# addtt/ladder-vae-pytorch

Hardware: AMD Instinct MI355X
Metric: training images/sec (ELBO step: fwd+bwd+Adamax) (higher is better)
Workload: dtype f32; 1 GPU; CIFAR10-shaped 15-layer LVAE (BASELINE configs[2]): 32x32x3, zdims 32x15, 4 blocks/layer, 64 filters, gated+skip, DMoL-10, dropout 0.2, free bits 1.0; batch_per_gpu=256, global_batch=256, parallelism=dp1, hip_graph=True

## Files before the change

include/lvae_hip.h:

```cpp
#ifndef LVAE_HIP_H
#define LVAE_HIP_H

#include <stddef.h>
#include <stdint.h>

#ifdef __cplusplus
extern "C" {
#endif

#define LVAE_ABI_VERSION 17

#define LVAE_EINVAL (-1)
#define LVAE_EALIGN (-2)
#define LVAE_EWORKSPACE (-3)

enum { LVAE_STATS_BN_FWD = 0, LVAE_STATS_BN_BWD = 1 };
enum { LVAE_PREC_F32 = 0, LVAE_PREC_BF16 = 1 };
enum { LVAE_DT_F32 = 0, LVAE_DT_BF16 = 1 };
enum {
  LVAE_FORM_AUTO = 0,
  LVAE_FORM_F32_MFMA = 1,
  LVAE_FORM_SIX_PRODUCT = 2,
  LVAE_FORM_SIX_PRODUCT_DIRECT = 3
};
enum { LVAE_ACT_NONE = 0, LVAE_ACT_ELU = 1, LVAE_ACT_RELU = 2, LVAE_ACT_LEAKYRELU = 3, LVAE_ACT_SELU = 4 };

enum {
  LVAE_GATHER_CONV = 0,
  LVAE_GATHER_TRANSPOSED = 1
};

int lvae_abi_version(void);
const char* lvae_last_error(void);

typedef struct lvae_bn_fold {
  const float* parts;
  int32_t rows;
  int64_t M;
  const float* gamma;
  const float* beta;
  float eps, momentum;
  float* running_mean;
  float* running_var;
  float* coef_out;
} lvae_bn_fold;

typedef struct lvae_conv_desc {
  const float* x;
  const float* x2;
  int32_t C1, C2;
  const float* w;
  int64_t w_stap, w_sk, w_sn;
  const float* bias;
  const float* in_scale;
  const float* in_shift;
  int32_t in_act;
  const float* out_scale;
  int32_t out_act;
  float* y;
  int32_t N, H, W, OH, OW, Cout;
  int32_t KH, KW, stride, pad;
  int32_t gather;
  int32_t precision;
  void* workspace;
  int64_t workspace_bytes;
  int32_t workspace_ready;
  float* stats_out;
  const float* stats_pivot;
  int32_t stats_mode;
  int32_t stats_act;
  const float* stats_x;
  const struct lvae_bn_fold* in_fold;
  int32_t form;
  uint8_t x_dtype;
  uint8_t y_dtype;
  uint8_t stats_x_dtype;
  uint8_t reserved_;
} lvae_conv_desc;

size_t lvae_conv2d_workspace(const lvae_conv_desc* d);
int lvae_conv2d_f32(const lvae_conv_desc* d, void* stream);
int lvae_conv1x1_dgrad_cat_f32(const lvae_conv_desc* d, float* dx2, int32_t split, void* stream);
int32_t lvae_conv1x1_dgrad_cat_ok(const lvae_conv_desc* d, int32_t split);
enum {
  LVAE_VARIANT_DIRECT = 0,
  LVAE_VARIANT_POS = 2,
  LVAE_VARIANT_WINO_F32 = 3,
  LVAE_VARIANT_WINO_SIX = 4,
  LVAE_VARIANT_BF16_DIRECT = 5,
  LVAE_VARIANT_SIX_DIRECT = 6
};
int32_t lvae_conv2d_variant(const lvae_conv_desc* d);
int32_t lvae_conv2d_position_major(const lvae_conv_desc* d);
int32_t lvae_resblock_bf16_storage(const lvae_conv_desc* d);
int lvae_conv2d_bf16(const lvae_conv_desc* d, void* stream);
int32_t lvae_conv2d_stats_rows(const lvae_conv_desc* d);
int32_t lvae_conv2d_folds_bn_finalize(const lvae_conv_desc* d);
int32_t lvae_conv2d_stats_buffer_rows(const lvae_conv_desc* d);

size_t lvae_conv2d_prepare_entry_bytes(void);
int lvae_conv2d_prepare_entry(const lvae_conv_desc* d, void* entry);
int lvae_conv2d_prepare_weights(const void* entries, int32_t n, int32_t max_cout, void* stream);

int lvae_conv1x1_gate_f32(const lvae_conv_desc* d, const float* res, int32_t act, float* out, void* stream);
int32_t lvae_conv1x1_gate_stats_rows(const lvae_conv_desc* d);
enum {
  LVAE_GATE_PERSISTENT = 1,
  LVAE_GATE_SINGLE_SHOT = 2
};
int32_t lvae_conv1x1_gate_variant(const lvae_conv_desc* d);
int lvae_conv1x1_gate_bwd_f32(const lvae_conv_desc* d, const float* dout, const float* ab, int32_t act, float* dab,
                              void* stream);
int32_t lvae_conv1x1_gate_bwd_ok(const lvae_conv_desc* d);

typedef struct lvae_bn_apply {
  const float* parts;
  int32_t rows;
  int32_t act;
  int64_t M;
  const float* coef;
  const float* dh;
  const float* x;
  const float* add;
  float* dgamma;
  float* dbeta;
  float* out;
  int32_t dh_bf16;
  int32_t reserved_;
  const float* drop;
} lvae_bn_apply;
size_t lvae_conv1x1_gate_bwd_wgrad_workspace(const lvae_conv_desc* d);
int32_t lvae_conv1x1_gate_bwd_wgrad_apply_ok(const lvae_conv_desc* d);
int lvae_conv1x1_gate_bwd_wgrad_f32(const lvae_conv_desc* d, const float* dout, const float* ab, const float* y, int32_t act,
                                    float* dw, int64_t dw_sk, int64_t dw_sn, float* db, void* workspace, size_t workspace_bytes,
                                    const lvae_bn_apply* ap, void* stream);
int32_t lvae_conv1x1_gate_bwd_wgrad_recompute_ok(const lvae_conv_desc* d);
int lvae_conv1x1_gate_bwd_wgrad_recompute_f32(const lvae_conv_desc* d, const float* dout, const float* y, int32_t act, void* gate_ws,
                                              int64_t gate_ws_bytes, int32_t gate_ws_ready, const float* gate_w, int64_t gate_w_sk,
                                              int64_t gate_w_sn, const float* gate_bias, float* dw, int64_t dw_sk, int64_t dw_sn,
                                              float* db, void* workspace, size_t workspace_bytes, const lvae_bn_apply* ap, void* stream);

enum { LVAE_RB_PRO_AFFINE = 0, LVAE_RB_PRO_BN_APPLY = 1, LVAE_RB_PRO_GATE_BWD = 2 };
enum { LVAE_RB_EPI_PLAIN = 0, LVAE_RB_EPI_GATE = 1 };
typedef struct lvae_rb_ext {
  int32_t prologue, epilogue;
  const float* gate_w;
  int64_t gate_w_sk, gate_w_sn;
  void* gate_ws;
  int64_t gate_ws_bytes;
  int32_t gate_ws_ready;
  const float* gate_bias;
  int32_t act;
  const float* res;
  float* ab;
  float* out;
  float* out_stats;
  const float* out_stats_pivot;
  const float* dout;
  const float* ab_in;
  float* dab;
  const float* bwd_parts;
  int32_t bwd_rows;
  int32_t bwd_act;
  int64_t bwd_M;
  const float* bwd_coef;
  const float* bwd_x;
  float* dgamma;
  float* dbeta;
  const float* pro_drop;
  float* xt_out;
  const void* pf_ptr[2];
  int64_t pf_bytes[2];
  const float* ap_parts;
  int32_t ap_rows;
  int32_t ap_act;
  int64_t ap_M;
  const float* ap_coef;
  const float* ap_dh;
  const float* ap_x;
  const float* ap_add;
  float* ap_dgamma;
  float* ap_dbeta;
  float* ap_out;
} lvae_rb_ext;
size_t lvae_resblock_gate_workspace(const lvae_conv_desc* g);
int lvae_resblock_gate_prepare_entry(const lvae_conv_desc* g, void* entry);
int32_t lvae_resblock_conv_rows(const lvae_conv_desc* d);
int32_t lvae_resblock_conv_gate_rows(const lvae_conv_desc* d);
size_t lvae_resblock_conv_workspace(const lvae_conv_desc* d);
int lvae_resblock_conv_prepare_entry(const lvae_conv_desc* d, void* entry);
int lvae_resblock_conv_f32(const lvae_conv_desc* d, const lvae_rb_ext* ext, void* stream);

size_t lvae_conv2d_wgrad_workspace(const lvae_conv_desc* d);
int lvae_conv2d_wgrad_f32(const lvae_conv_desc* d, const float* dy, float* dw, float* db, void* workspace,
                          size_t workspace_bytes, void* stream);
int lvae_conv2d_wgrad_bf16(const lvae_conv_desc* d, const float* dy, float* dw, float* db, void* workspace, size_t workspace_bytes,
                           void* stream);
int32_t lvae_conv2d_wgrad_apply_ok(const lvae_conv_desc* d);
int lvae_conv2d_wgrad_apply_f32(const lvae_conv_desc* d, const lvae_bn_apply* ap, float* dw, float* db, void* workspace,
                                size_t workspace_bytes, void* stream);
int32_t lvae_conv2d_wgrad_pair_ok(const lvae_conv_desc* a, const lvae_conv_desc* b);
size_t lvae_conv2d_wgrad_pair_workspace(const lvae_conv_desc* a, const lvae_conv_desc* b);
int32_t lvae_conv2d_wgrad_pair_schedule(const lvae_conv_desc* a, const lvae_conv_desc* b, int32_t* sched);
int lvae_conv2d_wgrad_pair_f32(const lvae_conv_desc* a, const lvae_bn_apply* ap, const lvae_conv_desc* b, const float* dy_b, float* dw_a,
                               float* db_a, float* dw_b, float* db_b, void* workspace, size_t workspace_bytes, void* stream);
enum {
  LVAE_WGRAD_VARIANT_GENERIC = 0,
  LVAE_WGRAD_VARIANT_IMG = 1,
  LVAE_WGRAD_VARIANT_BF16 = 2,
  LVAE_WGRAD_VARIANT_WINO = 3,
  LVAE_WGRAD_VARIANT_DIRECT_1X1 = 4,
  LVAE_WGRAD_VARIANT_TILE = 5,
  LVAE_WGRAD_VARIANT_THIN = 6
};
int32_t lvae_conv2d_wgrad_variant(const lvae_conv_desc* d);
size_t lvae_conv2d_wgrad_grouped_workspace(const lvae_conv_desc* descs, int32_t n);
int lvae_conv2d_wgrad_grouped_f32(const lvae_conv_desc* descs, const float* const* dy, float* const* dw, float* const* db,
                                  int32_t n, void* workspace, size_t workspace_bytes, void* stream);
int32_t lvae_conv2d_wgrad_grouped_schedule(const lvae_conv_desc* descs, int32_t n, int32_t* launch_of);

size_t lvae_bn_stats_workspace(int64_t M, int32_t C);
int lvae_bn_stats_f32(const float* x, int64_t M, int32_t C, const float* gamma, const float* beta, float eps,
                      float momentum, float* running_mean, float* running_var, float* scale, float* shift,
                      float* mean, float* rstd, void* workspace, size_t workspace_bytes, void* stream);
int lvae_bn_finalize_parts_f32(const float* parts, int32_t rows, int64_t M, int32_t C, const float* pivot, const float* gamma,
                               const float* beta, float eps, float momentum, float* running_mean, float* running_var,
                               float* scale, float* shift, float* mean, float* rstd, void* stream);
int lvae_bn_eval_coeffs_f32(int32_t C, const float* gamma, const float* beta, const float* running_mean,
                            const float* running_var, float eps, float* scale, float* shift, void* stream);

int lvae_affine_act_f32(const float* x, int64_t M, int32_t C, const float* scale, const float* shift, int32_t act,
                        const float* row_scale, int64_t rows_per_n, float* y, void* stream);

int lvae_affine_act_bwd_f32(const float* dh, const float* x, int64_t M, int32_t C, const float* scale,
                            const float* shift, int32_t act, int32_t bn_train, const float* mean, const float* rstd,
                            float* dgamma, float* dbeta, const float* drop, int64_t rows_per_n, const float* add,
                            float* dx, void* workspace, size_t workspace_bytes, void* stream);
int lvae_affine_act_bwd_parts_f32(const float* parts, int32_t rows, const float* dh, const float* x, int64_t M, int32_t C,
                                  const float* scale, const float* shift, int32_t act, const float* mean, const float* rstd,
                                  float* dgamma, float* dbeta, const float* drop, int64_t rows_per_n, const float* add,
                                  float* dx, void* workspace, size_t workspace_bytes, int32_t dtypes, void* stream);

int lvae_gate_fwd_f32(const float* ab, const float* res, int64_t M, int32_t C, int32_t act, float* out, void* stream);
int lvae_gate_bwd_f32(const float* dout, const float* ab, int64_t M, int32_t C, int32_t act, float* dab, void* stream);

int lvae_act_bwd_from_out_f32(const float* dy, const float* y, int64_t n, int32_t act, float* dx, void* stream);
int lvae_add_f32(const float* a, const float* b, int64_t n, float* out, void* stream);
int lvae_add3_f32(const float* a, const float* b, const float* c, int64_t n, float* out, void* stream);
int lvae_sum_of_row_means_f32(const float* x, int32_t L, int32_t N, float* out, void* stream);
int lvae_scale_rows_add_f32(const float* a, const float* row_scale, int64_t rows_per_n, int32_t C, const float* b,
                            int64_t M, float* out, void* stream);
int lvae_colsum_f32(const float* x, int64_t R, int64_t P, float* out, int32_t accumulate, void* stream);

int lvae_normal_stochastic_fwd_f32(const float* p, int32_t p_bcast, const float* q, const float* eps, int32_t N,
                                   int32_t HW, int32_t Z, int32_t mode, int32_t analytical_kl, float* z,
                                   float* logprob_p, float* logprob_q, float* kl_samplewise, float* kl_spatial,
                                   void* stream);
int lvae_normal_stochastic_bwd_f32(const float* p, int32_t p_bcast, const float* q, const float* eps, const float* z,
                                   const float* dz, const float* g_lp, const float* g_lq, const float* g_kl,
                                   const float* g_ks, int32_t N, int32_t HW, int32_t Z, int32_t mode,
                                   int32_t analytical_kl, float* dp, float* dq, void* stream);

typedef struct lvae_stoch_block {
  lvae_conv_desc conv_p, conv_q, conv_out;
  const float* p_given;
  int32_t p_bcast;
  int32_t mode, analytical_kl;
  const float* eps;
  float *logprob_p, *logprob_q, *kl_samplewise, *kl_spatial;
} lvae_stoch_block;
int32_t lvae_stoch_block_ok(const lvae_stoch_block* b);
size_t lvae_stoch_block_workspace(const lvae_conv_desc* d);
int lvae_stoch_block_prepare_entry(const lvae_conv_desc* d, void* entry);
int lvae_stoch_block_fwd_f32(const lvae_stoch_block* b, void* stream);
typedef struct lvae_stoch_block_bwd {
  lvae_conv_desc dgrad_out, dgrad_q, dgrad_p;
  const float* p;
  int32_t p_bcast;
  int32_t mode, analytical_kl;
  const float *q, *z, *eps, *dz, *g_lp, *g_lq, *g_kl, *g_ks;
} lvae_stoch_block_bwd;
int32_t lvae_stoch_block_bwd_ok(const lvae_stoch_block_bwd* b);
int lvae_stoch_block_bwd_f32(const lvae_stoch_block_bwd* b, void* stream);

int lvae_normal_prior_sample_f32(const float* p, int32_t p_bcast, const float* eps, float temperature,
                                 const float* row_temperature, int32_t N, int32_t HW, int32_t Z, float* z, float* logprob_p,
                                 void* stream);

size_t lvae_latent_interp_workspace(int32_t B, int32_t T);
int lvae_latent_interp_f32(const float* za, const float* zb, const float* t, int32_t B, int64_t n, int32_t T, int32_t mode, float* out,
                           void* workspace, size_t workspace_bytes, void* stream);

int lvae_kl_elementwise_fwd_f32(const float* p, int32_t p_bcast, const float* q, int32_t q_bcast, const float* z, int32_t N,
                                int32_t HW, int32_t Z, int32_t analytical_kl, float* out, void* stream);
int lvae_kl_elementwise_bwd_f32(const float* p, int32_t p_bcast, const float* q, int32_t q_bcast, const float* z, const float* g,
                                int32_t N, int32_t HW, int32_t Z, int32_t analytical_kl, float* dp, float* dq, float* dz,
                                void* stream);

int lvae_bernoulli_fwd_f32(const float* logits, const float* x, const float* u, int32_t N, int64_t P, float* mean,
                           float* mode, float* sample, float* ll, float* dll_dlogits, void* stream);
size_t lvae_dmol_workspace(int32_t N, int32_t HW);
int lvae_dmol_ll_fwd_f32(const float* l, const float* x, int32_t N, int32_t HW, int32_t nmix, float* ll, float* dll_dl,
                         void* workspace, size_t workspace_bytes, void* stream);
int lvae_dmol_sample_f32(const float* l, const float* u_mix, const float* u_log, int32_t N, int32_t HW, int32_t nmix,
                         float* sample, void* stream);
int lvae_gaussian_fwd_f32(const float* params, const float* x, const float* eps, int32_t N, int64_t P, int32_t C,
                          float* sample, float* ll, float* dll_dparams, void* stream);
int lvae_discr_logistic_fwd_f32(const float* raw, const float* x, const float* u, int32_t N, int64_t P, int32_t C, float* mean,
                                float* logscale, float* sample, float* ll, float* dll_draw, void* stream);
int lvae_bernoulli_masked_fwd_f32(const float* logits, const float* x, const float* u, int32_t N, int64_t P, int32_t C, float* mean,
                                  float* mode, float* sample, float* ll, float* dll_dlogits, const uint8_t* mask, float* filled,
                                  void* stream);
int lvae_dmol_ll_masked_fwd_f32(const float* l, const float* x, int32_t N, int32_t HW, int32_t nmix, float* ll, float* dll_dl,
                                void* workspace, size_t workspace_bytes, const uint8_t* mask, const float* sample, float* filled,
                                void* stream);
int lvae_gaussian_masked_fwd_f32(const float* params, const float* x, const float* eps, int32_t N, int64_t P, int32_t C, float* sample,
                                 float* ll, float* dll_dparams, const uint8_t* mask, float* filled, void* stream);
int lvae_discr_logistic_masked_fwd_f32(const float* raw, const float* x, const float* u, int32_t N, int64_t P, int32_t C, float* mean,
                                       float* logscale, float* sample, float* ll, float* dll_draw, const uint8_t* mask, float* filled,
                                       void* stream);
int lvae_mask_select_f32(const float* a, const float* b, float b_value, const uint8_t* mask, int32_t N, int32_t C, int64_t HW,
                         int32_t nchw, float* out, void* stream);
int lvae_scale_per_sample_f32(const float* a, const float* g, int32_t N, int64_t P, float* out, void* stream);

int lvae_upsample2x_fwd_f32(const float* x, int32_t N, int32_t H, int32_t W, int32_t C, float* y, void* stream);
int lvae_upsample2x_bwd_f32(const float* dy, int32_t N, int32_t H, int32_t W, int32_t C, float* dx, void* stream);
int lvae_pad_crop_f32(const float* x, int32_t N, int32_t C, int32_t H, int32_t W, int32_t src_nchw, float* y, int32_t OH,
                      int32_t OW, int32_t dst_nchw, void* stream);

int lvae_kl_bookkeeping_fwd_f32(const float* kl, int32_t L, int32_t N, float free_bits, float* kl_sep,
                                float* kl_avg_layerwise, float* scalars, void* stream);
int lvae_kl_bookkeeping_bwd_f32(const float* kl, int32_t L, int32_t N, float free_bits, const float* g_sep,
                                const float* g_avg, const float* g_scalars, float* dkl, void* stream);
int lvae_elbo_loss_fwd_f32(const float* ll, const float* kl_sep, const float* kl_loss, float beta, int32_t N,
                           float* elbo_sep, float* scalars, void* stream);
int lvae_elbo_loss_bwd_f32(const float* g_loss, float beta, int32_t N, float* d_ll, float* d_kl_loss, void* stream);
int lvae_elbo_loss_fwd_anneal_f32(const float* ll, const float* kl_sep, const float* kl_loss, const int64_t* step, int64_t anneal_steps,
                                  int32_t N, float* elbo_sep, float* scalars, void* stream);
int lvae_elbo_loss_bwd_anneal_f32(const float* g_loss, const int64_t* step, int64_t anneal_steps, int32_t N, float* d_ll,
                                  float* d_kl_loss, void* stream);

int lvae_iw_loss_fwd_f32(const float* ll, const float* kl_sep, float beta, int32_t K, int32_t B, float* elbo_sep, float* w, float* bound,
                         float* scalars, void* stream);
int lvae_iw_loss_bwd_f32(const float* g_loss, const float* w, float beta, int32_t K, int32_t B, float* d_ll, float* d_kl_sep,
                         void* stream);
int lvae_iw_loss_fwd_anneal_f32(const float* ll, const float* kl_sep, const int64_t* step, int64_t anneal_steps, int32_t K, int32_t B,
                                float* elbo_sep, float* w, float* bound, float* scalars, void* stream);
int lvae_iw_loss_bwd_anneal_f32(const float* g_loss, const float* w, const int64_t* step, int64_t anneal_steps, int32_t K, int32_t B,
                                float* d_ll, float* d_kl_sep, void* stream);
int lvae_repeat_samples_fwd_f32(const float* in, int64_t n, int32_t K, float* out, void* stream);
int lvae_repeat_samples_bwd_f32(const float* dout, int64_t n, int32_t K, float* din, void* stream);

int lvae_iw_logmeanexp_f32(const float* elbo, int32_t S, int32_t N, float* out, void* stream);
int lvae_iw_online_f32(const float* elbo, float* state, int32_t N, int32_t mode, int32_t S, float* iw, float* mean, void* stream);
int lvae_eval_online_f32(const float* elbo_sep, const float* ll, const float* kl_sep, const float* kl_avg_layerwise, double* state,
                         int32_t N, int32_t L, int32_t mode, void* stream);
int lvae_eval_totals_f64(const double* state, int32_t N, int32_t L, int32_t S, double* totals, void* stream);
size_t lvae_latent_stats_workspace(int32_t N, int32_t HW, int32_t Z);
int lvae_latent_stats_fold_f32(const float* p, int32_t p_bcast, const float* q, int32_t N, int32_t HW, int32_t Z, double* sums,
                               void* workspace, size_t workspace_bytes, void* stream);
int lvae_latent_stats_finalize_f64(const double* sums, int64_t U, int64_t n_images, double kl_threshold, double var_threshold,
                                   double* unit_out, double* layer_out, void* stream);
int lvae_summary_fold_f64(const float* loss, const float* elbo, const float* recons, const float* kl, const float* l2,
                          const float* grad_norm, const float* gscale, const float* kl_layers, int32_t L, double* acc, void* stream);
int lvae_summary_take_f64(double* acc, int32_t n, double* out, void* stream);

int lvae_image_border_count_f32(const float* a, int32_t a_nhwc, const float* b, int32_t b_nhwc, int32_t N, int32_t C, int32_t H,
                                int32_t W, float threshold, int32_t* count, void* stream);
int lvae_image_grid_u8(const float* a, int32_t a_nhwc, const float* b, int32_t b_nhwc, int32_t N, int32_t C, int32_t H, int32_t W,
                       int32_t nrow, const int32_t* border_count, float pad_value, uint8_t* grid, int64_t grid_bytes, void* stream);

#define LVAE_FEED_U8 0
#define LVAE_FEED_F32 1
int lvae_batch_gather_f32(const void* src, int32_t src_kind, int32_t src_hwc, int32_t N, int32_t C, int32_t H, int32_t W,
                          const int32_t* index, const int64_t* cursor, int32_t steps_per_epoch, int32_t B_global, int32_t lo,
                          int64_t base, int32_t n_rows, float* out, void* stream);

size_t lvae_nn_l2_workspace(int32_t Q, int64_t N, int32_t k);
int lvae_nn_l2_f32(const float* queries, int32_t Q, const void* table, int32_t table_kind, int64_t N, int64_t D, const int32_t* exclude,
                   int32_t k, int32_t* index_out, float* dist_out, void* workspace, size_t workspace_bytes, void* stream);

int lvae_adamax_step_f32(float* p, const float* g, float* exp_avg, float* exp_inf, const float* mask, int64_t n,
                         float lr, float beta1, float beta2, float eps, float weight_decay, const float* gscale,
                         const uint64_t* step_count, void* stream);
int lvae_adamax_ema_step_f32(float* p, const float* g, float* exp_avg, float* exp_inf, const float* mask, int64_t n,
                             float lr, float beta1, float beta2, float eps, float weight_decay, const float* gscale,
                             const uint64_t* step_count, float* ema, float decay, void* stream);
enum { LVAE_LR_CONSTANT = 0, LVAE_LR_COSINE = 1, LVAE_LR_LINEAR = 2, LVAE_LR_STEP = 3, LVAE_LR_EXP = 4 };
typedef struct lvae_lr_schedule {
  float base_lr;
  float min_lr;
  float gamma;
  int32_t kind;
  int64_t warmup_steps;
  int64_t decay_steps;
} lvae_lr_schedule;
int lvae_lr_schedule_at(const lvae_lr_schedule* schedule, uint64_t n, float* lr);
int lvae_adamax_sched_step_f32(float* p, const float* g, float* exp_avg, float* exp_inf, const float* mask, int64_t n,
                               const lvae_lr_schedule* schedule, float beta1, float beta2, float eps, float weight_decay,
                               const float* gscale, const uint64_t* step_count, float* ema, float decay, float* lr_out, void* stream);
typedef struct lvae_grad_guard_state {
  float norm;
  float scale;
  int32_t skip;
  int32_t reserved_;
  uint64_t clipped;
  uint64_t skipped;
} lvae_grad_guard_state;
int lvae_grad_guard_f32(const float* g, int64_t n, const float* gscale_in, float max_norm, float skip_threshold,
                        lvae_grad_guard_state* state, void* workspace, size_t workspace_bytes, void* stream);
int lvae_adamax_guarded_step_f32(float* p, const float* g, float* exp_avg, float* exp_inf, const float* mask, int64_t n, float lr,
                                 const lvae_lr_schedule* schedule, float beta1, float beta2, float eps, float weight_decay,
                                 const uint64_t* step_count, float* ema, float decay, float* lr_out,
                                 const lvae_grad_guard_state* guard, void* stream);
int lvae_adam_step_f32(float* p, const float* g, float* exp_avg, float* exp_avg_sq, const float* mask, int64_t n, float lr,
                       const lvae_lr_schedule* schedule , double beta1, double beta2, float eps, float weight_decay,
                       int32_t decoupled, const float* gscale , const uint64_t* step_count, float* ema ,
                       float decay, float* lr_out , const lvae_grad_guard_state* guard , void* stream);
typedef struct lvae_copy_entry {
  float* dst;
  const float* src;
  int64_t n;
} lvae_copy_entry;
int lvae_multi_copy_f32(const lvae_copy_entry* table, int32_t n_entries, const int32_t* flag, int32_t want, void* stream);
int lvae_swap_f32(float* a, float* b, int64_t n, void* stream);
size_t lvae_sumsq_workspace(int64_t n);
int lvae_l2norm_f32(const float* x, int64_t n, float* out, void* workspace, size_t workspace_bytes, void* stream);

int lvae_rng_fill_f32(float* out, int64_t n, int32_t kind, float lo, float hi, uint64_t seed, const uint64_t* offset,
                      uint64_t stream_id, void* stream);
int lvae_counter_advance(uint64_t* counter, uint64_t by, void* stream);
int lvae_counter_advance_unless(uint64_t* counter, uint64_t by, const int32_t* flag, void* stream);
int lvae_fill_f32(float* out, int64_t n, float value, void* stream);

int lvae_allreduce_unique_id(const char* librccl_path, void* id128);
int lvae_allreduce_init(const char* librccl_path, const void* id128, int32_t world, int32_t rank, void** handle);
int lvae_allreduce_enqueue(void* handle, float* buf, int64_t n, float* scratch, void* launch_stream, void* side_stream);
int lvae_allreduce_wait(void* handle, void* launch_stream, void* side_stream);
int lvae_allreduce_destroy(void* handle);

#ifdef __cplusplus
}
#endif
#endif
```

ladder-vae-pytorch_amd/_C.py:

```python
import ctypes as C
import os

import torch

_HERE = os.path.dirname(os.path.abspath(__file__))
LIB_PATH = os.path.join(_HERE, 'liblvae_hip.so')

ACT = {None: 0, 'none': 0, 'elu': 1, 'relu': 2, 'leakyrelu': 3, 'selu': 4}
GATHER_CONV, GATHER_TRANSPOSED = 0, 1
PREC_F32, PREC_BF16 = 0, 1
DT_F32, DT_BF16 = 0, 1
VARIANT_DIRECT, VARIANT_POS, VARIANT_WINO_F32, VARIANT_WINO_SIX, VARIANT_BF16_DIRECT, VARIANT_SIX_DIRECT = 0, 2, 3, 4, 5, 6
GATE_PERSISTENT, GATE_SINGLE_SHOT = 1, 2
WGRAD_VARIANT_GENERIC, WGRAD_VARIANT_IMG, WGRAD_VARIANT_BF16, WGRAD_VARIANT_WINO, WGRAD_VARIANT_DIRECT_1X1, WGRAD_VARIANT_TILE, WGRAD_VARIANT_THIN = range(7)
FEED_U8, FEED_F32 = 0, 1
FORM_AUTO, FORM_F32_MFMA, FORM_SIX_PRODUCT, FORM_SIX_PRODUCT_DIRECT = 0, 1, 2, 3


class LvaeHipError(RuntimeError):
    pass


class ConvDesc(C.Structure):
    _fields_ = [
        ('x', C.c_void_p), ('x2', C.c_void_p), ('C1', C.c_int32), ('C2', C.c_int32),
        ('w', C.c_void_p), ('w_stap', C.c_int64), ('w_sk', C.c_int64), ('w_sn', C.c_int64),
        ('bias', C.c_void_p), ('in_scale', C.c_void_p), ('in_shift', C.c_void_p), ('in_act', C.c_int32),
        ('out_scale', C.c_void_p), ('out_act', C.c_int32), ('y', C.c_void_p),
        ('N', C.c_int32), ('H', C.c_int32), ('W', C.c_int32), ('OH', C.c_int32), ('OW', C.c_int32),
        ('Cout', C.c_int32), ('KH', C.c_int32), ('KW', C.c_int32), ('stride', C.c_int32), ('pad', C.c_int32),
        ('gather', C.c_int32), ('precision', C.c_int32), ('workspace', C.c_void_p), ('workspace_bytes', C.c_int64), ('workspace_ready', C.c_int32), ('stats_out', C.c_void_p), ('stats_pivot', C.c_void_p), ('stats_mode', C.c_int32), ('stats_act', C.c_int32),
        ('stats_x', C.c_void_p),
        ('in_fold', C.c_void_p),
        ('form', C.c_int32), ('x_dtype', C.c_uint8), ('y_dtype', C.c_uint8), ('stats_x_dtype', C.c_uint8), ('reserved_', C.c_uint8),
    ]


class BnFold(C.Structure):
    _fields_ = [('parts', C.c_void_p), ('rows', C.c_int32), ('M', C.c_int64), ('gamma', C.c_void_p), ('beta', C.c_void_p),
                ('eps', C.c_float), ('momentum', C.c_float), ('running_mean', C.c_void_p), ('running_var', C.c_void_p),
                ('coef_out', C.c_void_p)]


class BnApply(C.Structure):
    _fields_ = [('parts', C.c_void_p), ('rows', C.c_int32), ('act', C.c_int32), ('M', C.c_int64), ('coef', C.c_void_p), ('dh', C.c_void_p),
                ('x', C.c_void_p), ('add', C.c_void_p), ('dgamma', C.c_void_p), ('dbeta', C.c_void_p), ('out', C.c_void_p),
                ('dh_bf16', C.c_int32), ('reserved_', C.c_int32), ('drop', C.c_void_p)]


class RbExt(C.Structure):
    _fields_ = [('prologue', C.c_int32), ('epilogue', C.c_int32), ('gate_w', C.c_void_p), ('gate_w_sk', C.c_int64), ('gate_w_sn', C.c_int64),
                ('gate_ws', C.c_void_p), ('gate_ws_bytes', C.c_int64), ('gate_ws_ready', C.c_int32), ('gate_bias', C.c_void_p), ('act', C.c_int32), ('res', C.c_void_p), ('ab', C.c_void_p), ('out', C.c_void_p),
                ('out_stats', C.c_void_p), ('out_stats_pivot', C.c_void_p), ('dout', C.c_void_p), ('ab_in', C.c_void_p), ('dab', C.c_void_p),
                ('bwd_parts', C.c_void_p), ('bwd_rows', C.c_int32), ('bwd_act', C.c_int32), ('bwd_M', C.c_int64), ('bwd_coef', C.c_void_p),
                ('bwd_x', C.c_void_p), ('dgamma', C.c_void_p), ('dbeta', C.c_void_p), ('pro_drop', C.c_void_p), ('xt_out', C.c_void_p),
                ('pf_ptr', C.c_void_p * 2), ('pf_bytes', C.c_int64 * 2),
                ('ap_parts', C.c_void_p), ('ap_rows', C.c_int32), ('ap_act', C.c_int32), ('ap_M', C.c_int64), ('ap_coef', C.c_void_p),
                ('ap_dh', C.c_void_p), ('ap_x', C.c_void_p), ('ap_add', C.c_void_p), ('ap_dgamma', C.c_void_p), ('ap_dbeta', C.c_void_p),
                ('ap_out', C.c_void_p)]


class StochBlock(C.Structure):
    _fields_ = [('conv_p', ConvDesc), ('conv_q', ConvDesc), ('conv_out', ConvDesc), ('p_given', C.c_void_p), ('p_bcast', C.c_int32),
                ('mode', C.c_int32), ('analytical_kl', C.c_int32), ('eps', C.c_void_p), ('logprob_p', C.c_void_p), ('logprob_q', C.c_void_p),
                ('kl_samplewise', C.c_void_p), ('kl_spatial', C.c_void_p)]


class StochBlockBwd(C.Structure):
    _fields_ = [('dgrad_out', ConvDesc), ('dgrad_q', ConvDesc), ('dgrad_p', ConvDesc), ('p', C.c_void_p), ('p_bcast', C.c_int32),
                ('mode', C.c_int32), ('analytical_kl', C.c_int32), ('q', C.c_void_p), ('z', C.c_void_p), ('eps', C.c_void_p), ('dz', C.c_void_p),
                ('g_lp', C.c_void_p), ('g_lq', C.c_void_p), ('g_kl', C.c_void_p), ('g_ks', C.c_void_p)]


class LrScheduleStruct(C.Structure):
    _fields_ = [('base_lr', C.c_float), ('min_lr', C.c_float), ('gamma', C.c_float), ('kind', C.c_int32),
                ('warmup_steps', C.c_int64), ('decay_steps', C.c_int64)]


class GradGuardState(C.Structure):
    _fields_ = [('norm', C.c_float), ('scale', C.c_float), ('skip', C.c_int32), ('reserved_', C.c_int32), ('clipped', C.c_uint64),
                ('skipped', C.c_uint64)]


class CopyEntry(C.Structure):
    _fields_ = [('dst', C.c_void_p), ('src', C.c_void_p), ('n', C.c_int64)]


LR_KINDS = {'constant': 0, 'cosine': 1, 'linear': 2, 'step': 3, 'exp': 4}

RB_PRO_AFFINE, RB_PRO_BN_APPLY, RB_PRO_GATE_BWD = 0, 1, 2
RB_EPI_PLAIN, RB_EPI_GATE = 0, 1

ABI_VERSION = 17

_P, _I, _L, _F, _Z, _U = C.c_void_p, C.c_int32, C.c_int64, C.c_float, C.c_size_t, C.c_uint64

SIGNATURES = {
    'lvae_abi_version': (C.c_int, []),
    'lvae_last_error': (C.c_char_p, []),
    'lvae_conv2d_workspace': (_Z, [C.POINTER(ConvDesc)]),
    'lvae_conv2d_f32': (C.c_int, [C.POINTER(ConvDesc), _P]),
    'lvae_conv2d_bf16': (C.c_int, [C.POINTER(ConvDesc), _P]),
    'lvae_conv1x1_dgrad_cat_f32': (C.c_int, [C.POINTER(ConvDesc), _P, _I, _P]),
    'lvae_conv1x1_dgrad_cat_ok': (_I, [C.POINTER(ConvDesc), _I]),
    'lvae_conv2d_stats_rows': (_I, [C.POINTER(ConvDesc)]),
    'lvae_conv2d_variant': (_I, [C.POINTER(ConvDesc)]),
    'lvae_conv2d_position_major': (_I, [C.POINTER(ConvDesc)]),
    'lvae_resblock_bf16_storage': (_I, [C.POINTER(ConvDesc)]),
    'lvae_conv2d_folds_bn_finalize': (_I, [C.POINTER(ConvDesc)]),
    'lvae_conv2d_stats_buffer_rows': (_I, [C.POINTER(ConvDesc)]),
    'lvae_conv2d_prepare_entry_bytes': (_Z, []),
    'lvae_conv2d_prepare_entry': (C.c_int, [C.POINTER(ConvDesc), _P]),
    'lvae_conv2d_prepare_weights': (C.c_int, [_P, _I, _I, _P]),
    'lvae_conv1x1_gate_f32': (C.c_int, [C.POINTER(ConvDesc), _P, _I, _P, _P]),
    'lvae_conv1x1_gate_stats_rows': (_I, [C.POINTER(ConvDesc)]),
    'lvae_conv1x1_gate_variant': (_I, [C.POINTER(ConvDesc)]),
    'lvae_conv1x1_gate_bwd_f32': (C.c_int, [C.POINTER(ConvDesc), _P, _P, _I, _P, _P]),
    'lvae_conv1x1_gate_bwd_ok': (_I, [C.POINTER(ConvDesc)]),
    'lvae_conv1x1_gate_bwd_wgrad_workspace': (_Z, [C.POINTER(ConvDesc)]),
    'lvae_conv1x1_gate_bwd_wgrad_apply_ok': (_I, [C.POINTER(ConvDesc)]),
    'lvae_conv1x1_gate_bwd_wgrad_f32': (C.c_int, [C.POINTER(ConvDesc), _P, _P, _P, _I, _P, _L, _L, _P, _P, _Z, C.POINTER(BnApply), _P]),
    'lvae_conv1x1_gate_bwd_wgrad_recompute_ok': (_I, [C.POINTER(ConvDesc)]),
    'lvae_conv1x1_gate_bwd_wgrad_recompute_f32': (C.c_int, [C.POINTER(ConvDesc), _P, _P, _I, _P, _L, _I, _P, _L, _L, _P, _P, _L, _L, _P, _P, _Z,
                                                            C.POINTER(BnApply), _P]),
    'lvae_resblock_gate_workspace': (_Z, [C.POINTER(ConvDesc)]),
    'lvae_resblock_gate_prepare_entry': (C.c_int, [C.POINTER(ConvDesc), _P]),
    'lvae_resblock_conv_rows': (_I, [C.POINTER(ConvDesc)]),
    'lvae_resblock_conv_gate_rows': (_I, [C.POINTER(ConvDesc)]),
    'lvae_resblock_conv_workspace': (_Z, [C.POINTER(ConvDesc)]),
    'lvae_resblock_conv_prepare_entry': (C.c_int, [C.POINTER(ConvDesc), _P]),
    'lvae_resblock_conv_f32': (C.c_int, [C.POINTER(ConvDesc), C.POINTER(RbExt), _P]),
    'lvae_conv2d_wgrad_workspace': (_Z, [C.POINTER(ConvDesc)]),
    'lvae_conv2d_wgrad_f32': (C.c_int, [C.POINTER(ConvDesc), _P, _P, _P, _P, _Z, _P]),
    'lvae_conv2d_wgrad_bf16': (C.c_int, [C.POINTER(ConvDesc), _P, _P, _P, _P, _Z, _P]),
    'lvae_conv2d_wgrad_variant': (_I, [C.POINTER(ConvDesc)]),
    'lvae_conv2d_wgrad_apply_ok': (_I, [C.POINTER(ConvDesc)]),
    'lvae_conv2d_wgrad_apply_f32': (C.c_int, [C.POINTER(ConvDesc), C.POINTER(BnApply), _P, _P, _P, _Z, _P]),
    'lvae_conv2d_wgrad_pair_ok': (_I, [C.POINTER(ConvDesc), C.POINTER(ConvDesc)]),
    'lvae_conv2d_wgrad_pair_workspace': (_Z, [C.POINTER(ConvDesc), C.POINTER(ConvDesc)]),
    'lvae_conv2d_wgrad_pair_schedule': (_I, [C.POINTER(ConvDesc), C.POINTER(ConvDesc), C.POINTER(_I)]),
    'lvae_conv2d_wgrad_pair_f32': (C.c_int, [C.POINTER(ConvDesc), C.POINTER(BnApply), C.POINTER(ConvDesc), _P, _P, _P, _P, _P, _P, _Z, _P]),
    'lvae_conv2d_wgrad_grouped_workspace': (_Z, [C.POINTER(ConvDesc), _I]),
    'lvae_conv2d_wgrad_grouped_f32': (C.c_int, [C.POINTER(ConvDesc), _P, _P, _P, _I, _P, _Z, _P]),
    'lvae_conv2d_wgrad_grouped_schedule': (_I, [C.POINTER(ConvDesc), _I, C.POINTER(_I)]),
    'lvae_bn_stats_workspace': (_Z, [_L, _I]),
    'lvae_bn_stats_f32': (C.c_int, [_P, _L, _I, _P, _P, _F, _F, _P, _P, _P, _P, _P, _P, _P, _Z, _P]),
    'lvae_bn_finalize_parts_f32': (C.c_int, [_P, _I, _L, _I, _P, _P, _P, _F, _F, _P, _P, _P, _P, _P, _P, _P]),
    'lvae_bn_eval_coeffs_f32': (C.c_int, [_I, _P, _P, _P, _P, _F, _P, _P, _P]),
    'lvae_affine_act_f32': (C.c_int, [_P, _L, _I, _P, _P, _I, _P, _L, _P, _P]),
    'lvae_affine_act_bwd_f32': (C.c_int, [_P, _P, _L, _I, _P, _P, _I, _I, _P, _P, _P, _P, _P, _L, _P, _P, _P, _Z, _P]),
    'lvae_affine_act_bwd_parts_f32': (C.c_int, [_P, _I, _P, _P, _L, _I, _P, _P, _I, _P, _P, _P, _P, _P, _L, _P, _P, _P, _Z, _I, _P]),
    'lvae_gate_fwd_f32': (C.c_int, [_P, _P, _L, _I, _I, _P, _P]),
    'lvae_gate_bwd_f32': (C.c_int, [_P, _P, _L, _I, _I, _P, _P]),
    'lvae_act_bwd_from_out_f32': (C.c_int, [_P, _P, _L, _I, _P, _P]),
    'lvae_add_f32': (C.c_int, [_P, _P, _L, _P, _P]),
    'lvae_add3_f32': (C.c_int, [_P, _P, _P, _L, _P, _P]),
    'lvae_sum_of_row_means_f32': (C.c_int, [_P, _I, _I, _P, _P]),
    'lvae_scale_rows_add_f32': (C.c_int, [_P, _P, _L, _I, _P, _L, _P, _P]),
    'lvae_colsum_f32': (C.c_int, [_P, _L, _L, _P, _I, _P]),
    'lvae_normal_stochastic_fwd_f32': (C.c_int, [_P, _I, _P, _P, _I, _I, _I, _I, _I, _P, _P, _P, _P, _P, _P]),
    'lvae_normal_stochastic_bwd_f32': (C.c_int, [_P, _I, _P, _P, _P, _P, _P, _P, _P, _P, _I, _I, _I, _I, _I, _P, _P, _P]),
    'lvae_stoch_block_ok': (_I, [C.POINTER(StochBlock)]),
    'lvae_stoch_block_workspace': (_Z, [C.POINTER(ConvDesc)]),
    'lvae_stoch_block_prepare_entry': (C.c_int, [C.POINTER(ConvDesc), _P]),
    'lvae_stoch_block_fwd_f32': (C.c_int, [C.POINTER(StochBlock), _P]),
    'lvae_stoch_block_bwd_ok': (_I, [C.POINTER(StochBlockBwd)]),
    'lvae_stoch_block_bwd_f32': (C.c_int, [C.POINTER(StochBlockBwd), _P]),
    'lvae_normal_prior_sample_f32': (C.c_int, [_P, _I, _P, _F, _P, _I, _I, _I, _P, _P, _P]),
    'lvae_latent_interp_workspace': (_Z, [_I, _I]),
    'lvae_latent_interp_f32': (C.c_int, [_P, _P, _P, _I, _L, _I, _I, _P, _P, _Z, _P]),
    'lvae_kl_elementwise_fwd_f32': (C.c_int, [_P, _I, _P, _I, _P, _I, _I, _I, _I, _P, _P]),
    'lvae_kl_elementwise_bwd_f32': (C.c_int, [_P, _I, _P, _I, _P, _P, _I, _I, _I, _I, _P, _P, _P, _P]),
    'lvae_bernoulli_fwd_f32': (C.c_int, [_P, _P, _P, _I, _L, _P, _P, _P, _P, _P, _P]),
    'lvae_dmol_workspace': (_Z, [_I, _I]),
    'lvae_dmol_ll_fwd_f32': (C.c_int, [_P, _P, _I, _I, _I, _P, _P, _P, _Z, _P]),
    'lvae_dmol_sample_f32': (C.c_int, [_P, _P, _P, _I, _I, _I, _P, _P]),
    'lvae_gaussian_fwd_f32': (C.c_int, [_P, _P, _P, _I, _L, _I, _P, _P, _P, _P]),
    'lvae_discr_logistic_fwd_f32': (C.c_int, [_P, _P, _P, _I, _L, _I, _P, _P, _P, _P, _P, _P]),
    'lvae_bernoulli_masked_fwd_f32': (C.c_int, [_P, _P, _P, _I, _L, _I, _P, _P, _P, _P, _P, _P, _P, _P]),
    'lvae_dmol_ll_masked_fwd_f32': (C.c_int, [_P, _P, _I, _I, _I, _P, _P, _P, _Z, _P, _P, _P, _P]),
    'lvae_gaussian_masked_fwd_f32': (C.c_int, [_P, _P, _P, _I, _L, _I, _P, _P, _P, _P, _P, _P]),
    'lvae_discr_logistic_masked_fwd_f32': (C.c_int, [_P, _P, _P, _I, _L, _I, _P, _P, _P, _P, _P, _P, _P, _P]),
    'lvae_mask_select_f32': (C.c_int, [_P, _P, _F, _P, _I, _I, _L, _I, _P, _P]),
    'lvae_scale_per_sample_f32': (C.c_int, [_P, _P, _I, _L, _P, _P]),
    'lvae_upsample2x_fwd_f32': (C.c_int, [_P, _I, _I, _I, _I, _P, _P]),
    'lvae_upsample2x_bwd_f32': (C.c_int, [_P, _I, _I, _I, _I, _P, _P]),
    'lvae_pad_crop_f32': (C.c_int, [_P, _I, _I, _I, _I, _I, _P, _I, _I, _I, _P]),
    'lvae_kl_bookkeeping_fwd_f32': (C.c_int, [_P, _I, _I, _F, _P, _P, _P, _P]),
    'lvae_kl_bookkeeping_bwd_f32': (C.c_int, [_P, _I, _I, _F, _P, _P, _P, _P, _P]),
    'lvae_elbo_loss_fwd_f32': (C.c_int, [_P, _P, _P, _F, _I, _P, _P, _P]),
    'lvae_elbo_loss_bwd_f32': (C.c_int, [_P, _F, _I, _P, _P, _P]),
    'lvae_elbo_loss_fwd_anneal_f32': (C.c_int, [_P, _P, _P, _P, _L, _I, _P, _P, _P]),
    'lvae_elbo_loss_bwd_anneal_f32': (C.c_int, [_P, _P, _L, _I, _P, _P, _P]),
    'lvae_iw_loss_fwd_f32': (C.c_int, [_P, _P, _F, _I, _I, _P, _P, _P, _P, _P]),
    'lvae_iw_loss_bwd_f32': (C.c_int, [_P, _P, _F, _I, _I, _P, _P, _P]),
    'lvae_iw_loss_fwd_anneal_f32': (C.c_int, [_P, _P, _P, _L, _I, _I, _P, _P, _P, _P, _P]),
    'lvae_iw_loss_bwd_anneal_f32': (C.c_int, [_P, _P, _P, _L, _I, _I, _P, _P, _P]),
    'lvae_repeat_samples_fwd_f32': (C.c_int, [_P, _L, _I, _P, _P]),
    'lvae_repeat_samples_bwd_f32': (C.c_int, [_P, _L, _I, _P, _P]),
    'lvae_iw_online_f32': (C.c_int, [_P, _P, _I, _I, _I, _P, _P, _P]),
    'lvae_eval_online_f32': (C.c_int, [_P, _P, _P, _P, _P, _I, _I, _I, _P]),
    'lvae_eval_totals_f64': (C.c_int, [_P, _I, _I, _I, _P, _P]),
    'lvae_latent_stats_workspace': (_Z, [_I, _I, _I]),
    'lvae_latent_stats_fold_f32': (C.c_int, [_P, _I, _P, _I, _I, _I, _P, _P, _Z, _P]),
    'lvae_latent_stats_finalize_f64': (C.c_int, [_P, _L, _L, C.c_double, C.c_double, _P, _P, _P]),
    'lvae_summary_fold_f64': (C.c_int, [_P, _P, _P, _P, _P, _P, _P, _P, _I, _P, _P]),
    'lvae_summary_take_f64': (C.c_int, [_P, _I, _P, _P]),
    'lvae_image_border_count_f32': (C.c_int, [_P, _I, _P, _I, _I, _I, _I, _I, _F, _P, _P]),
    'lvae_image_grid_u8': (C.c_int, [_P, _I, _P, _I, _I, _I, _I, _I, _I, _P, _F, _P, _L, _P]),
    'lvae_batch_gather_f32': (C.c_int, [_P, _I, _I, _I, _I, _I, _I, _P, _P, _I, _I, _I, _L, _I, _P, _P]),
    'lvae_nn_l2_workspace': (_Z, [_I, _L, _I]),
    'lvae_nn_l2_f32': (C.c_int, [_P, _I, _P, _I, _L, _L, _P, _I, _P, _P, _P, _Z, _P]),
    'lvae_iw_logmeanexp_f32': (C.c_int, [_P, _I, _I, _P, _P]),
    'lvae_adamax_step_f32': (C.c_int, [_P, _P, _P, _P, _P, _L, _F, _F, _F, _F, _F, _P, _P, _P]),
    'lvae_adamax_ema_step_f32': (C.c_int, [_P, _P, _P, _P, _P, _L, _F, _F, _F, _F, _F, _P, _P, _P, _F, _P]),
    'lvae_lr_schedule_at': (C.c_int, [C.POINTER(LrScheduleStruct), _U, C.POINTER(C.c_float)]),
    'lvae_adamax_sched_step_f32': (C.c_int, [_P, _P, _P, _P, _P, _L, C.POINTER(LrScheduleStruct), _F, _F, _F, _F, _P, _P, _P, _F, _P, _P]),
    'lvae_grad_guard_f32': (C.c_int, [_P, _L, _P, _F, _F, _P, _P, _Z, _P]),
    'lvae_adamax_guarded_step_f32': (C.c_int, [_P, _P, _P, _P, _P, _L, _F, C.POINTER(LrScheduleStruct), _F, _F, _F, _F, _P, _P, _F, _P, _P, _P]),
    'lvae_adam_step_f32': (C.c_int, [_P, _P, _P, _P, _P, _L, _F, C.POINTER(LrScheduleStruct), C.c_double, C.c_double, _F, _F, _I, _P, _P, _P,
                                     _F, _P, _P, _P]),
    'lvae_multi_copy_f32': (C.c_int, [_P, _I, _P, _I, _P]),
    'lvae_swap_f32': (C.c_int, [_P, _P, _L, _P]),
    'lvae_sumsq_workspace': (_Z, [_L]),
    'lvae_l2norm_f32': (C.c_int, [_P, _L, _P, _P, _Z, _P]),
    'lvae_rng_fill_f32': (C.c_int, [_P, _L, _I, _F, _F, _U, _P, _U, _P]),
    'lvae_counter_advance': (C.c_int, [_P, _U, _P]),
    'lvae_counter_advance_unless': (C.c_int, [_P, _U, _P, _P]),
    'lvae_fill_f32': (C.c_int, [_P, _L, _F, _P]),
    'lvae_allreduce_unique_id': (C.c_int, [C.c_char_p, _P]),
    'lvae_allreduce_init': (C.c_int, [C.c_char_p, _P, _I, _I, C.POINTER(C.c_void_p)]),
    'lvae_allreduce_enqueue': (C.c_int, [_P, _P, _L, _P, _P, _P]),
    'lvae_allreduce_wait': (C.c_int, [_P, _P, _P]),
    'lvae_allreduce_destroy': (C.c_int, [_P]),
}

_lib = None


def load():
    global _lib
    if _lib is not None:
        return _lib
    if not os.path.exists(LIB_PATH):
        raise LvaeHipError("%s is missing: build it with `python -c 'import __graft_entry__ as g; g.build()'` or "
                           "`make -C ladder-vae-pytorch_amd/csrc`. There is no CPU / PyTorch fallback." % LIB_PATH)
    lib = C.CDLL(LIB_PATH)
    for name, (res, args) in SIGNATURES.items():
        fn = getattr(lib, name)
        fn.restype, fn.argtypes = res, args
    if lib.lvae_abi_version() != ABI_VERSION:
        raise LvaeHipError("liblvae_hip.so ABI version %d, expected %d" % (lib.lvae_abi_version(), ABI_VERSION))
    _lib = lib
    return lib


def stream_ptr():
    return torch.cuda.current_stream().cuda_stream


def ptr(t, dtypes=(torch.float32, torch.int64, torch.uint8)):
    if t is None:
        return None
    if not t.is_cuda:
        raise LvaeHipError("lvae_hip kernels need CUDA/HIP tensors; got a %s tensor (no CPU fallback exists)" % t.device)
    if t.dtype not in dtypes:
        raise LvaeHipError("unexpected dtype %s for this entry point (it has no storage-type argument for this tensor)" % t.dtype)
    return t.data_ptr()


def ptr_dt(t):
    return ptr(t, (torch.float32, torch.bfloat16))


def check(rc, name):
    if rc != 0:
        raise LvaeHipError("%s failed (%d): %s" % (name, rc, load().lvae_last_error().decode()))


def call(name, *args):
    check(getattr(load(), name)(*args), name)
```

ladder-vae-pytorch_amd/csrc/conv3x3_wgrad_wino.hip:

```cpp
#include <stdlib.h>

#include <algorithm>
#include <type_traits>

#include "bn_stats.h"
#include "lvae_host.h"

namespace lvae {

struct WgWinoArgs {
  lvae_conv_desc d;
  const float* dy;
  float* slab_w;
  float* slab_b;
  int nranges, ncog, cpr, total_chunks, cpi;
  uint32_t m_cpi;
};

constexpr int WG_XS = 48;
constexpr int WG_DS = 80;

template <int TPR>
__global__ __launch_bounds__(512, 2) void conv_wgrad_wino_kernel(WgWinoArgs a) {
  kernarg_warmup<sizeof(WgWinoArgs)>();
  const int nwg_ = gridDim.x, bid_ = blockIdx.x;
  constexpr bool AP = false;
  const lvae_bn_apply ap = lvae_bn_apply{};
#include "conv3x3_wgrad_wino_body.inc"
}

struct WgWinoApArgs {
  WgWinoArgs w;
  lvae_bn_apply ap;
};
template <int TPR>
__global__ __launch_bounds__(512, 2) void conv_wgrad_wino_ap_kernel(WgWinoApArgs g) {
  kernarg_warmup<sizeof(WgWinoApArgs)>();
  const WgWinoArgs& a = g.w;
  const lvae_bn_apply& ap = g.ap;
  const int nwg_ = gridDim.x, bid_ = blockIdx.x;
  constexpr bool AP = true;
#include "conv3x3_wgrad_wino_body.inc"
}

struct WgWinoGroup {
  WgWinoArgs p[kWgradWinoGroup];
};
static_assert(sizeof(WgWinoGroup) <= 4096, "kernel argument block");

template <int TPR>
__global__ __launch_bounds__(512, 2) void conv_wgrad_wino_grouped_kernel(WgWinoGroup g) {
  kernarg_warmup<(sizeof(WgWinoGroup) < 1024 ? sizeof(WgWinoGroup) : 1024)>();
  const WgWinoArgs& a = g.p[blockIdx.y];
  const int nwg_ = a.nranges * a.ncog * 2;
  if ((int)blockIdx.x >= nwg_) return;
  const int bid_ = blockIdx.x;
  constexpr bool AP = false;
  const lvae_bn_apply ap = lvae_bn_apply{};
#include "conv3x3_wgrad_wino_body.inc"
}

struct WgWinoPairArgs {
  WgWinoArgs a, b;
  lvae_bn_apply ap;
  int nwg_a, pad_;
};
static_assert(sizeof(WgWinoPairArgs) <= 4096, "kernel argument block");

template <int TPR>
__global__ __launch_bounds__(512, 2) void conv_wgrad_wino_pair_kernel(WgWinoPairArgs g) {
  kernarg_warmup<(sizeof(WgWinoPairArgs) < 1024 ? sizeof(WgWinoPairArgs) : 1024)>();
  if ((int)blockIdx.x < g.nwg_a) {
    const WgWinoArgs& a = g.a;
    const lvae_bn_apply& ap = g.ap;
    const int nwg_ = g.nwg_a, bid_ = blockIdx.x;
    constexpr bool AP = true;
#include "conv3x3_wgrad_wino_body.inc"
  } else {
    const WgWinoArgs& a = g.b;
    const lvae_bn_apply ap = lvae_bn_apply{};
    const int nwg_ = (int)gridDim.x - g.nwg_a, bid_ = (int)blockIdx.x - g.nwg_a;
    constexpr bool AP = false;
#include "conv3x3_wgrad_wino_body.inc"
  }
}

struct WinoReduceArgs {
  const float* slab_w;
  const float* slab_b;
  int nranges, ncog, Cout, pad_;
  int64_t stap, sk, sn;
  float* dw;
  float* db;
};
struct WinoReduceGroup {
  WinoReduceArgs p[kWgradWinoGroup];
};
struct WinoReducePair {
  WinoReduceArgs p[2];
};

template <bool HALF>
__device__ __forceinline__ void wino_reduce_body(const WinoReduceArgs& a, int bx, float* red, float (*red_b)[64]) {
  constexpr int CW = HALF ? 32 : 64;
  const int ncog = a.ncog, nranges = a.nranges;
  const int half = HALF ? (bx & 1) : 0, cc = HALF ? (bx >> 1) : bx, ci = cc / ncog, cog = cc % ncog;
  const int t = threadIdx.x;
  const int q = HALF ? (t & 7) : (t & 15), p = HALF ? ((t >> 3) & 15) : ((t >> 4) & 15), rs = HALF ? (t >> 7) : (t >> 8);
  const float* src = a.slab_w + ((((size_t)(ci >> 5) * ncog + cog) * 32 + (ci & 31)) * 16 + p) * 64 + half * 32 + q * 4;
  const size_t rstride = (size_t)2 * ncog * 32 * 16 * 64;
  f32x4 s = {0.f, 0.f, 0.f, 0.f};
  if ((p & 3) != 3) {
    if (HALF) {
#pragma unroll 8
      for (int r = rs; r < nranges; r += 8) s += *reinterpret_cast<const f32x4*>(src + r * rstride);
      *reinterpret_cast<f32x4*>(red + (rs * 16 + p) * CW + q * 4) = s;
    } else {
      f32x4 s1 = {0.f, 0.f, 0.f, 0.f};
#pragma unroll 4
      for (int r = rs; r < nranges; r += 8) {
        s += *reinterpret_cast<const f32x4*>(src + r * rstride);
        if (r + 4 < nranges) s1 += *reinterpret_cast<const f32x4*>(src + (r + 4) * rstride);
      }
      *reinterpret_cast<f32x4*>(red + (rs * 16 + p) * CW + q * 4) = s;
      *reinterpret_cast<f32x4*>(red + ((rs + 4) * 16 + p) * CW + q * 4) = s1;
    }
  }
  const bool do_b = a.db != nullptr && ci == 0 && half == 0;
  if (do_b) {
    const int co = t & 63, slice = t >> 6;
    float v = 0.f;
#pragma unroll 4
    for (int r = slice; r < nranges; r += 16) v += a.slab_b[(size_t)(r * ncog + cog) * 64 + co];
    red_b[slice][co] = v;
  }
  __syncthreads();
  if (t < 3 * CW && cog * 64 + half * 32 + (t % CW) < a.Cout) {
    const int co = t % CW, ga = t / CW;
    float u[4][3];
#pragma unroll
    for (int i = 0; i < 4; ++i)
#pragma unroll
      for (int b = 0; b < 3; ++b) {
        const float* rp = red + (i * 4 + b) * CW + co;
        u[i][b] = ((rp[0] + rp[16 * CW]) + (rp[32 * CW] + rp[48 * CW])) + ((rp[64 * CW] + rp[80 * CW]) + (rp[96 * CW] + rp[112 * CW]));
      }
    float* o = a.dw + (int64_t)ci * a.sk + (int64_t)(cog * 64 + half * 32 + co) * a.sn + (int64_t)(ga * 3) * a.stap;
#pragma unroll
    for (int b = 0; b < 3; ++b)
      o[b * a.stap] += ga == 0 ? u[0][b] + 0.5f * (u[1][b] + u[2][b]) : (ga == 1 ? 0.5f * (u[1][b] - u[2][b]) : 0.5f * (u[1][b] + u[2][b]) + u[3][b]);
  }
  if (do_b && t >= 256 && t < 320 && cog * 64 + t - 256 < a.Cout) {
    const int co = t - 256;
    float v = 0.f;
#pragma unroll
    for (int k = 0; k < 16; ++k) v += red_b[k][co];
    a.db[cog * 64 + co] += v;
  }
}

__global__ __launch_bounds__(1024) void conv_wgrad_wino_reduce_kernel(WinoReduceArgs a) {
  kernarg_warmup<sizeof(WinoReduceArgs)>();
  __shared__ __attribute__((aligned(16))) float red[8 * 16 * 32];
  __shared__ float red_b[16][64];
  wino_reduce_body<true>(a, blockIdx.x, red, red_b);
}

__global__ __launch_bounds__(1024) void conv_wgrad_wino_reduce_pair_kernel(WinoReducePair g) {
  kernarg_warmup<sizeof(WinoReducePair)>();
  __shared__ __attribute__((aligned(16))) float red[8 * 16 * 32];
  __shared__ float red_b[16][64];
  wino_reduce_body<true>(g.p[blockIdx.y], blockIdx.x, red, red_b);
}

__global__ __launch_bounds__(1024) void conv_wgrad_wino_reduce_grouped_kernel(WinoReduceGroup g) {
  kernarg_warmup<(sizeof(WinoReduceGroup) < 1024 ? sizeof(WinoReduceGroup) : 1024)>();
  const WinoReduceArgs& a = g.p[blockIdx.y];
  if ((int)blockIdx.x >= 64 * a.ncog) return;
  __shared__ __attribute__((aligned(16))) float red[8 * 16 * 64];
  __shared__ float red_b[16][64];
  wino_reduce_body<false>(a, blockIdx.x, red, red_b);
}

static bool wg_wino_plan(const lvae_conv_desc* d, WgWinoArgs& a, int budget = 128) {
  static const bool off = tune("LVAE_DISABLE_WINO_WGRAD", 0) != 0 || tune("LVAE_DISABLE_WINO", 0) != 0;
  if (off) return false;
  if (d->KH != 3 || d->KW != 3 || d->stride != 1 || d->pad != 1 || d->gather != LVAE_GATHER_CONV) return false;
  if (d->C1 != 64 || d->C2 != 0 || d->x2 != nullptr || d->Cout % 4 != 0 || d->Cout > 256) return false;
  if (d->OH != d->H || d->OW != d->W || (d->H & 1)) return false;
  if (d->W != 8 && d->W != 16 && d->W != 32) return false;
  const int tpr = d->W / 2, tr = 16 / tpr;
  if ((d->H / 2) % tr != 0) return false;
  if (!al16_or_null(d->x) || !al16_or_null(d->in_scale) || !al16_or_null(d->in_shift)) return false;
  const int64_t M = (int64_t)d->N * d->H * d->W;
  static const int64_t min_m = tune("LVAE_WINO_WGRAD_MIN_M", 256 * 64);
  if (M < min_m || M * 256 >= ((int64_t)1 << 31)) return false;
  a.ncog = (d->Cout + 63) / 64;
  a.cpi = (d->H / 2) / tr;
  a.total_chunks = d->N * a.cpi;
  int nranges = budget / a.ncog;
  if (nranges < 1) nranges = 1;
  static const int min_cpr = (int)tune("LVAE_WINO_WGRAD_MIN_CPR", 4);
  if (nranges > a.total_chunks / min_cpr) nranges = a.total_chunks / min_cpr;
  if (nranges < 1) nranges = 1;
  a.cpr = (a.total_chunks + nranges - 1) / nranges;
  a.nranges = (a.total_chunks + a.cpr - 1) / a.cpr;
  a.m_cpi = fastdiv_magic(a.cpi);
  return true;
}

bool conv_wgrad_wino_plan(const lvae_conv_desc* d, WgradPlan& p) {
  static const int64_t group_max_m = tune("LVAE_WINO_GROUP_MAX_M", 65536);
  WgWinoArgs a;
  if (!wg_wino_plan(d, a)) return false;
  p.group = (int64_t)d->N * d->H * d->W < group_max_m ? d->W : -1;
  p.set_slabs(a.nranges, (size_t)a.ncog * 2 * 16 * 32 * 64, (size_t)a.ncog * 64);
  p.apply_ok = d->precision == LVAE_PREC_F32 && d->Cout == 64 && (d->W == 16 || d->W == 32) && d->x_dtype == LVAE_DT_F32 && d->y_dtype == LVAE_DT_F32;
  return true;
}

constexpr int kWgWinoPairRangesA = 74;
static int wg_wino_pair_ranges_a() {
  static const int v = (int)std::min<int64_t>(127, std::max<int64_t>(1, tune("LVAE_WINO_PAIR_RANGES_A", kWgWinoPairRangesA)));
  return v;
}

static bool wg_wino_pair_split(const lvae_conv_desc* da, const lvae_conv_desc* db, WgWinoArgs& a, WgWinoArgs& b) {
  if (!wg_wino_plan(da, a, wg_wino_pair_ranges_a()) || a.ncog != 1 || a.nranges >= 128) return false;
  if (!wg_wino_plan(db, b, 128 - a.nranges) || b.ncog != 1) return false;
  return wg_wino_plan(da, a, 128 - b.nranges);
}

bool conv_wgrad_wino_pair_plan(const lvae_conv_desc* da, const lvae_conv_desc* db, WgradPlan& pa, WgradPlan& pb, int32_t* sched) {
  WgWinoArgs a, b;
  if (!wg_wino_pair_split(da, db, a, b)) return false;
  pa.set_slabs(a.nranges, (size_t)2 * 16 * 32 * 64, 64);
  pb.set_slabs(b.nranges, (size_t)2 * 16 * 32 * 64, 64);
  if (sched) {
    const int32_t v[6] = {a.nranges, a.cpr, a.nranges * 2, b.nranges, b.cpr, b.nranges * 2};
    std::copy(v, v + 6, sched);
  }
  return true;
}

template <typename F>
static int with_tpr(int W, F f) {
  if (W == 8) return f(std::integral_constant<int, 4>{});
  if (W == 16) return f(std::integral_constant<int, 8>{});
  return f(std::integral_constant<int, 16>{});
}

static size_t wg_wino_lds(int W) {
  const int tpr = W / 2, hp = (2 * (16 / tpr) + 2) * (W + 2);
  return std::max((size_t)2 * (hp * WG_XS + 64 * WG_DS), (size_t)(4 * 4 * 2 * 16 * 64 + 128)) * sizeof(float);
}

static int wino_fill_planned(const WgradOp& o, WgWinoArgs& a, WinoReduceArgs& r) {
  a.d = *o.d;
  a.dy = o.dy;
  a.slab_w = o.slab_w();
  a.slab_b = o.slab_b();
  r = WinoReduceArgs{a.slab_w, a.slab_b, a.nranges, a.ncog, o.d->Cout, 0, o.d->w_stap, o.d->w_sk, o.d->w_sn, o.dw, o.db};
  return a.nranges * a.ncog * 2;
}
static int wino_fill(const WgradOp& o, WgWinoArgs& a, WinoReduceArgs& r) {
  wg_wino_plan(o.d, a);
  return wino_fill_planned(o, a, r);
}

int conv_wgrad_wino_apply_launch(const WgradOp& o, const lvae_bn_apply* ap, hipStream_t s) {
  WgWinoApArgs g;
  WinoReduceArgs r;
  const int wgs = wino_fill(o, g.w, r);
  g.ap = *ap;
  auto launch = [&](auto tpr) {
    return launch_lds<conv_wgrad_wino_ap_kernel<decltype(tpr)::value>>("conv_wgrad_wino_ap", dim3(wgs), dim3(512), wg_wino_lds(o.d->W),
                                                                       160 * 1024, s, g);
  };
  const int rc = o.d->W == 16 ? launch(std::integral_constant<int, 8>{}) : launch(std::integral_constant<int, 16>{});
  if (rc) return rc;
  hipLaunchKernelGGL(conv_wgrad_wino_reduce_kernel, dim3(128 * r.ncog), dim3(1024), 0, s, r);
  LVAE_LAUNCH_CHECK("conv_wgrad_wino_reduce");
  return 0;
}

int conv_wgrad_wino_pair_launch(const WgradOp& a, const lvae_bn_apply* ap, const WgradOp& b, hipStream_t s) {
  WgWinoPairArgs g;
  WinoReducePair rg;
  wg_wino_pair_split(a.d, b.d, g.a, g.b);
  g.nwg_a = wino_fill_planned(a, g.a, rg.p[0]);
  const int nwg_b = wino_fill_planned(b, g.b, rg.p[1]);
  g.ap = *ap;
  g.pad_ = 0;
  auto launch = [&](auto tpr) {
    return launch_lds<conv_wgrad_wino_pair_kernel<decltype(tpr)::value>>("conv_wgrad_wino_pair", dim3(g.nwg_a + nwg_b), dim3(512), wg_wino_lds(a.d->W),
                                                                         160 * 1024, s, g);
  };
  const int rc = a.d->W == 16 ? launch(std::integral_constant<int, 8>{}) : launch(std::integral_constant<int, 16>{});
  if (rc) return rc;
  hipLaunchKernelGGL(conv_wgrad_wino_reduce_pair_kernel, dim3(128, 2), dim3(1024), 0, s, rg);
  LVAE_LAUNCH_CHECK("conv_wgrad_wino_reduce_pair");
  return 0;
}

int conv_wgrad_wino_launch(const WgradOp* o, int n, hipStream_t s) {
  WgWinoGroup g;
  WinoReduceGroup rg;
  int max_wgs = 0, max_ncog = 0;
  for (int i = 0; i < n; ++i) {
    max_wgs = std::max(max_wgs, wino_fill(o[i], g.p[i], rg.p[i]));
    max_ncog = std::max(max_ncog, g.p[i].ncog);
  }
  for (int i = n; i < kWgradWinoGroup; ++i) {
    g.p[i] = g.p[0];
    rg.p[i] = rg.p[0];
  }
  const size_t lds = wg_wino_lds(o->d->W);
  const int rc = with_tpr(o->d->W, [&](auto tpr) {
    constexpr int T = decltype(tpr)::value;
    if (n == 1) return launch_lds<conv_wgrad_wino_kernel<T>>("conv_wgrad_wino", dim3(max_wgs), dim3(512), lds, 160 * 1024, s, g.p[0]);
    return launch_lds<conv_wgrad_wino_grouped_kernel<T>>("conv_wgrad_wino_grouped", dim3(max_wgs, n), dim3(512), lds, 160 * 1024, s, g);
  });
  if (rc) return rc;
  if (n == 1) hipLaunchKernelGGL(conv_wgrad_wino_reduce_kernel, dim3(128 * max_ncog), dim3(1024), 0, s, rg.p[0]);
  else hipLaunchKernelGGL(conv_wgrad_wino_reduce_grouped_kernel, dim3(64 * max_ncog, n), dim3(1024), 0, s, rg);
  LVAE_LAUNCH_CHECK(n == 1 ? "conv_wgrad_wino_reduce" : "conv_wgrad_wino_reduce_grouped");
  return 0;
}

}
```

ladder-vae-pytorch_amd/csrc/conv3x3_wgrad_wino_body.inc:

```
  extern __shared__ __attribute__((aligned(16))) float smem[];
  constexpr int W = 2 * TPR, HW2 = W + 2, TR = 16 / TPR, HROWS = 2 * TR + 2;
  constexpr int HP = HROWS * HW2;
  constexpr int XSLOTS = (HP * 8 + 511) / 512;
  constexpr int BUF = HP * WG_XS + 64 * WG_DS;
  const lvae_conv_desc& d = a.d;
  const int t = threadIdx.x, lane = t & 63, wave = t >> 6;
  const int li = lane & 31, lh = lane >> 5, pi = wave & 3, kg = wave >> 2;
  int bid = bid_;
  {
    const int nwg = nwg_, xcd = bid & 7, q = nwg >> 3, r = nwg & 7;
    bid = (xcd < r ? xcd * (q + 1) : r * (q + 1) + (xcd - r) * q) + (bid >> 3);
  }
  const int cib = bid & 1, cog = (bid >> 1) % a.ncog, range = (bid >> 1) / a.ncog;
  const int c_begin = range * a.cpr;
  const int c_end = min(a.total_chunks, c_begin + a.cpr);
  const f32x4 zero4 = {0.f, 0.f, 0.f, 0.f};
#ifdef LVAE_WGW_DBG
  constexpr int dbg = LVAE_WGW_DBG;
#else
  constexpr int dbg = 0;
#endif

  const int xc4 = (t & 7) * 4;
  int xrel[AP ? 1 : XSLOTS], xhy[AP ? 1 : XSLOTS];
  bool xcol_ok[AP ? 1 : XSLOTS], xin[AP ? 1 : XSLOTS];
  auto slot = [&](int u, int& hy, bool& col_ok, bool& in, int& rel) {
    const int px = (t >> 3) + 64 * u;
    hy = px / HW2;
    const int hx = px - hy * HW2;
    in = px < HP;
    col_ok = (hx >= 1) & (hx <= W);
    rel = (hy * W + hx) * 64 + cib * 32 + xc4;
  };
  if (!AP) {
#pragma unroll
    for (int u = 0; u < XSLOTS; ++u) slot(u, xhy[u], xcol_ok[u], xin[u], xrel[u]);
  }
  const int dpx = t >> 4, dc4 = (t & 15) * 4;
  const int drel = dpx * d.Cout + cog * 64 + dc4;
  const bool dy_ok = cog * 64 + dc4 < d.Cout;
  f32x4 sc = {1.f, 1.f, 1.f, 1.f}, sh = zero4;
  if (d.in_scale && !AP) {
    sc = *reinterpret_cast<const f32x4*>(d.in_scale + cib * 32 + xc4);
    sh = *reinterpret_cast<const f32x4*>(d.in_shift + cib * 32 + xc4);
  }
  f32x4 xreg[XSLOTS], dreg[2];
  f32x4 yreg[AP ? 2 : 1], dmask = {1.f, 1.f, 1.f, 1.f};
  float* Cf = smem + 2 * BUF;
  if (AP) {
    const int q = t & 31, rg = t >> 5, rows = ap.rows;
    f32x4 accp = zero4;
    for (int r = rg; r < rows; r += 16 * 8) {
      f32x4 v[8];
#pragma unroll
      for (int u = 0; u < 8; ++u) {
        const int rr = r + 16 * u;
        v[u] = *reinterpret_cast<const f32x4*>(ap.parts + (size_t)(rr < rows ? rr : 0) * 128 + q * 4);
      }
#pragma unroll
      for (int u = 0; u < 8; ++u)
        if (r + 16 * u < rows) accp += v[u];
    }
    *reinterpret_cast<f32x4*>(smem + rg * 128 + q * 4) = accp;
    if (t < 256) Cf[t] = ap.coef[t];
    if (t < 64) {
      Cf[384 + t] = d.in_scale ? d.in_scale[t] : 1.f;
      Cf[448 + t] = d.in_scale ? d.in_shift[t] : 0.f;
    }
    __syncthreads();
    if (t < 64) {
      double sa = 0.0, sb = 0.0;
#pragma unroll
      for (int g2 = 0; g2 < 16; ++g2) {
        sa += (double)smem[g2 * 128 + t];
        sb += (double)smem[g2 * 128 + 64 + t];
      }
      const BnBwdChannel r = bn_bwd_finish(sa, sb, ap.M);
      Cf[256 + t] = r.c1;
      Cf[320 + t] = r.c2;
      if (bid_ == 0) {
        if (ap.dbeta) ap.dbeta[t] += r.dbeta;
        if (ap.dgamma) ap.dgamma[t] += r.dgamma;
      }
    }
    __syncthreads();
  }
  const float* dysrc = AP ? ap.dh : a.dy;
  unsigned xok = 0;
  auto load_chunk = [&](int c) {
    const int n = fastdiv(c, a.m_cpi), cr = c - n * a.cpi;
    const int oh0 = cr * (2 * TR);
    const float* xb = d.x + ((int64_t)(n * d.H + oh0 - 1) * W - 1) * 64;
    xok = 0;
#pragma unroll
    for (int u = 0; u < XSLOTS; ++u) {
      int s_hy, s_rel;
      bool s_col, s_in;
      if (AP) slot(u, s_hy, s_col, s_in, s_rel);
      else { s_hy = xhy[u]; s_col = xcol_ok[u]; s_in = xin[u]; s_rel = xrel[u]; }
      const int ih = oh0 - 1 + s_hy;
      const bool ok = s_in & s_col & ((unsigned)ih < (unsigned)d.H);
      const float* p = ok ? xb + s_rel : d.x;
      if (dbg & 1) xreg[u] = zero4;
      else xreg[u] = *reinterpret_cast<const f32x4*>(p);
      xok |= ok ? (1u << u) : 0u;
    }
    const int64_t doff0 = (int64_t)(n * d.H + oh0) * W * d.Cout + drel;
    const float* dyb = dy_ok ? dysrc + doff0 : dysrc;
    if (dbg & 1) {
      dreg[0] = dreg[1] = zero4;
    } else {
      dreg[0] = *reinterpret_cast<const f32x4*>(dyb);
      dreg[1] = *reinterpret_cast<const f32x4*>(dy_ok ? dyb + 32 * d.Cout : dyb);
    }
    if (AP) {
      const float* yb = dy_ok ? ap.x + doff0 : ap.x;
      yreg[0] = *reinterpret_cast<const f32x4*>(yb);
      yreg[AP ? 1 : 0] = *reinterpret_cast<const f32x4*>(dy_ok ? yb + 32 * d.Cout : yb);
      if (ap.drop) dmask = *reinterpret_cast<const f32x4*>(ap.drop + (size_t)n * d.Cout + (dy_ok ? cog * 64 + dc4 : 0));
    }
    if (!dy_ok) dreg[0] = dreg[1] = zero4;
  };
  auto store_chunk = [&](float* buf, int c) {
    if (AP) {
      const int n = fastdiv(c, a.m_cpi), cr = c - n * a.cpi;
      const int64_t doff0 = (int64_t)(n * d.H + cr * (2 * TR)) * W * d.Cout + drel;
      const f32x4 ap_sc = *reinterpret_cast<const f32x4*>(Cf + dc4), ap_sh = *reinterpret_cast<const f32x4*>(Cf + 64 + dc4);
      const f32x4 ap_mu = *reinterpret_cast<const f32x4*>(Cf + 128 + dc4), ap_rs = *reinterpret_cast<const f32x4*>(Cf + 192 + dc4);
      const f32x4 ap_c1 = *reinterpret_cast<const f32x4*>(Cf + 256 + dc4), ap_c2 = *reinterpret_cast<const f32x4*>(Cf + 320 + dc4);
#pragma unroll
      for (int k = 0; k < 2; ++k) {
        const f32x4 xv = yreg[AP ? k : 0];
        const f32x4 gq = dreg[k] * act_grad4(xv * ap_sc + ap_sh, ap.act);
        f32x4 v = bn_bwd_apply(gq, xv, ap_c1, ap_c2, ap_mu, ap_rs, ap_sc) * dmask;
        if (!dy_ok) v = zero4;
        dreg[k] = v;
        if (cib == 0 && dy_ok) store_wt4(ap.out + doff0 + (k ? 32 * d.Cout : 0), v);
      }
    }
    if (AP) {
      sc = *reinterpret_cast<const f32x4*>(Cf + 384 + cib * 32 + xc4);
      sh = *reinterpret_cast<const f32x4*>(Cf + 448 + cib * 32 + xc4);
    }
#pragma unroll
    for (int u = 0; u < XSLOTS; ++u) {
      if (AP ? ((t >> 3) + 64 * u < HP) : xin[u]) {
        f32x4 v = zero4;
        if ((xok >> u) & 1u) {
          v = xreg[u];
          if (d.in_scale && !(dbg & 8)) v = act_fwd4(v * sc + sh, d.in_act);
        }
        *reinterpret_cast<f32x4*>(buf + ((t >> 3) + 64 * u) * WG_XS + xc4) = v;
      }
    }
    *reinterpret_cast<f32x4*>(buf + HP * WG_XS + dpx * WG_DS + dc4) = dreg[0];
    *reinterpret_cast<f32x4*>(buf + HP * WG_XS + (dpx + 32) * WG_DS + dc4) = dreg[1];
  };

  const int ra = pi == 0 ? 0 : (pi == 2 ? 2 : 1);
  const int rb = pi == 0 ? 2 : (pi == 1 ? 2 : (pi == 2 ? 1 : 3));
  const float sgn = pi == 1 ? 1.f : -1.f;
  const float alpha = pi == 3 ? 0.f : 1.f;
  const float beta = pi == 0 ? 0.f : (pi == 1 ? 1.f : -1.f);
  int xbase_px, dbase_px;
  if (TPR == 4) {
    xbase_px = 4 * kg * HW2 + 2 * lh;
    dbase_px = 4 * kg * W + 2 * lh;
  } else if (TPR == 8) {
    xbase_px = 2 * kg * HW2 + 2 * lh;
    dbase_px = 2 * kg * W + 2 * lh;
  } else {
    xbase_px = 16 * kg + 2 * lh;
    dbase_px = 16 * kg + 2 * lh;
  }
  const int xoff_a = (xbase_px + ra * HW2) * WG_XS + li;
  const int xoff_b = (xbase_px + rb * HW2) * WG_XS + li;
  const int doff = HP * WG_XS + dbase_px * WG_DS + li;

  f32x16 acc[4][2];
#pragma unroll
  for (int j = 0; j < 4; ++j)
#pragma unroll
    for (int h = 0; h < 2; ++h)
#pragma unroll
      for (int r = 0; r < 16; ++r) acc[j][h][r] = 0.f;
  float dbacc[2] = {0.f, 0.f};

  if (c_begin < c_end) {
    load_chunk(c_begin);
    store_chunk(smem, c_begin);
    if (c_begin + 1 < c_end) load_chunk(c_begin + 1);
  }
  __syncthreads();
  for (int c = c_begin; c < c_end; ++c) {
    const float* buf = smem + ((c - c_begin) & 1) * BUF;
    const float* pa = buf + xoff_a;
    const float* pb = buf + xoff_b;
    const float* pd = buf + doff;
    float rxa[4], rxb[4], ry[2][4];
    auto read_step = [&](int ss) {
      const int cx = TPR == 4 ? 2 * (ss >> 1) * HW2 + 4 * (ss & 1) : 4 * ss;
      const int cd = TPR == 4 ? 2 * (ss >> 1) * W + 4 * (ss & 1) : 4 * ss;
#pragma unroll
      for (int cc = 0; cc < 4; ++cc) {
        rxa[cc] = pa[(cx + cc) * WG_XS];
        rxb[cc] = pb[(cx + cc) * WG_XS];
      }
#pragma unroll
      for (int h = 0; h < 2; ++h) {
        const float* q = pd + cd * WG_DS + 32 * h;
        ry[h][0] = q[0];
        ry[h][1] = q[WG_DS];
        ry[h][2] = q[W * WG_DS];
        ry[h][3] = q[(W + 1) * WG_DS];
      }
    };
    read_step(0);
#pragma unroll
    for (int ss = 0; ss < 4; ++ss) {
      float tt[4], vv[4];
#pragma unroll
      for (int cc = 0; cc < 4; ++cc) tt[cc] = __builtin_fmaf(sgn, rxb[cc], rxa[cc]);
      vv[0] = tt[0] - tt[2];
      vv[1] = tt[1] + tt[2];
      vv[2] = tt[2] - tt[1];
      vv[3] = tt[1] - tt[3];
      float ww[2][4];
#pragma unroll
      for (int h = 0; h < 2; ++h) {
        const float s0 = __builtin_fmaf(beta, ry[h][2], alpha * ry[h][0]), s1 = __builtin_fmaf(beta, ry[h][3], alpha * ry[h][1]);
        ww[h][0] = s0;
        ww[h][1] = s0 + s1;
        ww[h][2] = s0 - s1;
        ww[h][3] = -s1;
        dbacc[h] += ww[h][1];
      }
      __builtin_amdgcn_sched_barrier(0);
      if (ss + 1 < 4) read_step(ss + 1);
      __builtin_amdgcn_sched_barrier(0);
#pragma unroll
      for (int j = 0; j < 4; ++j)
#pragma unroll
        for (int h = 0; h < 2; ++h) {
          if (dbg & 2) acc[j][h][0] += vv[j] * ww[h][j];
          else acc[j][h] = __builtin_amdgcn_mfma_f32_32x32x2f32(vv[j], ww[h][j], acc[j][h], 0, 0, 0);
        }
      __builtin_amdgcn_sched_barrier(0);
    }
    if (c + 1 < c_end) {
      store_chunk(smem + ((c + 1 - c_begin) & 1) * BUF, c + 1);
      if (c + 2 < c_end) load_chunk(c + 2);
    }
    __syncthreads();
  }

  float* Rs = smem;
  if (dbg & 16) {
    float v = dbacc[0] + dbacc[1];
#pragma unroll
    for (int j = 0; j < 4; ++j)
#pragma unroll
      for (int h = 0; h < 2; ++h)
#pragma unroll
        for (int r = 0; r < 16; ++r) v += acc[j][h][r];
    if (v == 12345.678f) a.slab_w[t] = v;
    return;
  }
  auto hand_over = [&](auto hsel) {
    constexpr int h = decltype(hsel)::value;
#pragma unroll
    for (int j = 0; j < 4; ++j)
#pragma unroll
      for (int r = 0; r < 16; ++r) Rs[(((pi * 4 + j) * 2 + h) * 16 + r) * 64 + lane] = acc[j][h][r];
  };
  if (kg == 0) hand_over(std::integral_constant<int, 1>{});
  else hand_over(std::integral_constant<int, 0>{});
  if (kg == 1 && pi == 1) {
    Rs[4 * 4 * 2 * 16 * 64 + lane] = dbacc[0];
    Rs[4 * 4 * 2 * 16 * 64 + 64 + lane] = dbacc[1];
  }
  __syncthreads();
  float* slab = a.slab_w + (size_t)((range * 2 + cib) * a.ncog + cog) * 32 * 16 * 64 + 4 * pi * 64;
  auto finish = [&](auto hsel) {
    constexpr int h = decltype(hsel)::value;
#pragma unroll
    for (int r = 0; r < 16; ++r) {
      const int ci = (r & 3) + 8 * (r >> 2) + 4 * lh;
      float u[4];
#pragma unroll
      for (int j = 0; j < 4; ++j) u[j] = acc[j][h][r] + Rs[(((pi * 4 + j) * 2 + h) * 16 + r) * 64 + lane];
      const float g[3] = {u[0] + 0.5f * (u[1] + u[2]), 0.5f * (u[1] - u[2]), 0.5f * (u[1] + u[2]) + u[3]};
#pragma unroll
      for (int b = 0; b < 3; ++b)
        if (!(dbg & 4) || g[b] == 12345.678f) slab[((size_t)ci * 16 + b) * 64 + 32 * h + li] = g[b];
    }
  };
  if (kg == 0) finish(std::integral_constant<int, 0>{});
  else finish(std::integral_constant<int, 1>{});
  if (kg == 0) {
    if (pi == 1 && cib == 0 && a.slab_b) {
#pragma unroll
      for (int h = 0; h < 2; ++h) {
        float v = dbacc[h] + Rs[4 * 4 * 2 * 16 * 64 + 64 * h + lane];
        v += __shfl_xor(v, 32, 64);
        if (lh == 0) a.slab_b[(size_t)(range * a.ncog + cog) * 64 + 32 * h + li] = v;
      }
    }
  }
```

ladder-vae-pytorch_amd/csrc/conv_wgrad.hip:

```cpp
#include <stdlib.h>

#include <algorithm>
#include <map>
#include <vector>

#include "lvae_host.h"

namespace lvae {

constexpr int KP = 32;
constexpr int CT = 64;

struct WgradArgs {
  lvae_conv_desc d;
  const float* dy;
  float* slab_w;
  float* slab_b;
  int M, ohw, Cin, ntaps, ncit, ncot, ksplit, px_per_split;
};

__device__ __forceinline__ bool tap_coord_w(int o, int k, int stride, int pad, int limit, int gather, int& i) {
  if (gather == LVAE_GATHER_CONV) {
    i = o * stride - pad + k;
    return i >= 0 && i < limit;
// ... 332 lines not shown
  for (int i = 0; i < n; ++i) {
    g.p[i] = r[i];
    const int tot = r[i].ntaps * r[i].Cin * r[i].Cout + (r[i].db ? r[i].Cout : 0);
    if (tot > max_tot) max_tot = tot;
  }
  for (int i = n; i < kMaxReduceGroup; ++i) g.p[i] = g.p[0];
  hipLaunchKernelGGL(wgrad_reduce_grouped_kernel, dim3((max_tot / 4 + 15) / 16, n), dim3(256), 0, s, g);
}

struct ThinWgradArgs {
  lvae_conv_desc d;
  const float* dy;
  float* slab_w;
  float* slab_b;
  int K, PH, PW;
};

__global__ __launch_bounds__(256) void conv_wgrad_thin_kernel(ThinWgradArgs a) {
  kernarg_warmup<(sizeof(ThinWgradArgs) < 1024 ? sizeof(ThinWgradArgs) : 1024)>();
  extern __shared__ __attribute__((aligned(16))) float smem[];
  const lvae_conv_desc& d = a.d;
  const int t = threadIdx.x, n = blockIdx.x;
  const int Cin = d.C1, npx = d.OH * d.OW;
  float* xs = smem;
  float* ys = smem + ((a.PH * a.PW * Cin + 3) & ~3);
  for (int i = t; i < a.PH * a.PW * Cin; i += 256) {
    const int ci = i % Cin, r = i / Cin, pw = r % a.PW, ph = r / a.PW;
    const int ih = ph - d.pad, iw = pw - d.pad;
    xs[i] = ((unsigned)ih < (unsigned)d.H && (unsigned)iw < (unsigned)d.W) ? d.x[((size_t)(n * d.H + ih) * d.W + iw) * Cin + ci] : 0.f;
  }
  for (int i = t; i < npx * 64; i += 256) {
    const int co = i & 63, px = i >> 6;
    ys[i] = co < d.Cout ? a.dy[((size_t)n * npx + px) * d.Cout + co] : 0.f;
  }
  __syncthreads();
  const int co = t & 63, kg = t >> 6;
  int koff[19];
#pragma unroll
  for (int kk = 0; kk < 19; ++kk) {
    int k = kg * 19 + kk;
    if (k >= a.K) k = 0;
    const int ci = k % Cin, tap = k / Cin, kw = tap % d.KW, kh = tap / d.KW;
    koff[kk] = (kh * a.PW + kw) * Cin + ci;
  }
  float acc[19];
#pragma unroll
  for (int kk = 0; kk < 19; ++kk) acc[kk] = 0.f;
  float bsum = 0.f;
  for (int oh = 0; oh < d.OH; ++oh) {
    for (int ow = 0; ow < d.OW; ++ow) {
      const float g = ys[(oh * d.OW + ow) * 64 + co];
      const float* xb = xs + ((oh * d.stride) * a.PW + ow * d.stride) * Cin;
      bsum += g;
#pragma unroll
      for (int kk = 0; kk < 19; ++kk) acc[kk] += xb[koff[kk]] * g;
    }
  }
  if (co < d.Cout) {
    float* slab = a.slab_w + (size_t)n * a.K * d.Cout;
#pragma unroll
    for (int kk = 0; kk < 19; ++kk) {
      const int k = kg * 19 + kk;
      if (k < a.K) slab[(size_t)k * d.Cout + co] = acc[kk];
    }
    if (a.slab_b && kg == 0) a.slab_b[(size_t)n * d.Cout + co] = bsum;
  }
}

static size_t thin_lds(const lvae_conv_desc* d) {
  return ((size_t)((d->H + 2 * d->pad) * (d->W + 2 * d->pad) * d->C1 + 3) / 4 * 4 + (size_t)d->OH * d->OW * 64) * sizeof(float);
}

static bool thin_wgrad_plan(const lvae_conv_desc* d, WgradPlan& p) {
  const int K = d->KH * d->KW * d->C1;
  if (d->gather != LVAE_GATHER_CONV || d->x2 != nullptr || d->C2 != 0 || d->in_scale != nullptr) return false;
  if (K > 76 || d->Cout > 64 || d->OH * d->OW > 1024 || d->N < 32 || d->N > 65535) return false;
  if (thin_lds(d) > 160 * 1024) return false;
  p.set_slabs(d->N, (size_t)K * d->Cout, d->Cout);
  return true;
}

static int thin_wgrad_launch(const WgradOp& o, hipStream_t s) {
  const lvae_conv_desc* d = o.d;
  ThinWgradArgs ta;
  ta.d = *d;
  ta.dy = o.dy;
  ta.K = d->KH * d->KW * d->C1;
  ta.PH = d->H + 2 * d->pad;
  ta.PW = d->W + 2 * d->pad;
  ta.slab_w = o.slab_w();
  ta.slab_b = o.slab_b();
  const int rc = launch_lds<conv_wgrad_thin_kernel>("conv_wgrad_thin", dim3(d->N), dim3(256), thin_lds(d), 160 * 1024, s, ta);
  return rc ? rc : wgrad_op_reduce(o, s);
}

static void wgrad_plan(const lvae_conv_desc* d, int& ksplit, int& px_per_split, int& ncit, int& ncot) {
  const int Cin = d->C1 + d->C2, M = d->N * d->OH * d->OW, ntaps = d->KH * d->KW;
  ncit = (Cin + CT - 1) / CT;
  ncot = (d->Cout + CT - 1) / CT;
  const int tiles = ntaps * ncit * ncot;
  int want = (512 + tiles - 1) / tiles;
  if (want > 64) want = 64;
  int maxsplit = (M + 255) / 256;
  ksplit = want < 1 ? 1 : want;
  if (ksplit > maxsplit) ksplit = maxsplit;
  if (ksplit < 1) ksplit = 1;
  px_per_split = (M + ksplit - 1) / ksplit;
  px_per_split = (px_per_split + KP - 1) / KP * KP;
  ksplit = (M + px_per_split - 1) / px_per_split;
}

static bool generic_wgrad_plan(const lvae_conv_desc* d, WgradPlan& p) {
  int ksplit, pps, ncit, ncot;
  wgrad_plan(d, ksplit, pps, ncit, ncot);
  p.set_slabs(ksplit, (size_t)d->KH * d->KW * (d->C1 + d->C2) * d->Cout, d->Cout);
  return true;
}

static int generic_wgrad_launch(const WgradOp& o, hipStream_t s) {
  const lvae_conv_desc* d = o.d;
  WgradArgs a;
  a.d = *d;
  a.dy = o.dy;
  a.M = d->N * d->OH * d->OW;
  a.ohw = d->OH * d->OW;
  a.Cin = d->C1 + d->C2;
  a.ntaps = d->KH * d->KW;
  wgrad_plan(d, a.ksplit, a.px_per_split, a.ncit, a.ncot);
  a.slab_w = o.slab_w();
  a.slab_b = o.slab_b();
  const bool xv = (d->C1 % 4 == 0) && (d->C2 % 4 == 0) && al16(d->x) && (!d->x2 || al16(d->x2)) &&
                  (!d->in_scale || (al16(d->in_scale) && al16(d->in_shift)));
  const bool yv = (d->Cout % 4 == 0) && al16(o.dy);
  const int grid = a.ksplit * a.ncot * a.ncit * a.ntaps;
  if (xv && yv) hipLaunchKernelGGL((conv_wgrad_kernel<true, true>), dim3(grid), dim3(256), 0, s, a);
  else if (xv) hipLaunchKernelGGL((conv_wgrad_kernel<true, false>), dim3(grid), dim3(256), 0, s, a);
  else if (yv) hipLaunchKernelGGL((conv_wgrad_kernel<false, true>), dim3(grid), dim3(256), 0, s, a);
  else hipLaunchKernelGGL((conv_wgrad_kernel<false, false>), dim3(grid), dim3(256), 0, s, a);
  LVAE_LAUNCH_CHECK("conv2d_wgrad");
  return wgrad_op_reduce(o, s);
}

struct WgradFamily {
  int32_t variant;
  bool (*plan)(const lvae_conv_desc*, WgradPlan&);
  bool dy16, ws16;
};
static const WgradFamily kWgradFamilies[] = {
    {LVAE_WGRAD_VARIANT_IMG, [](auto d, auto& p) { return conv_wgrad_img_plan(d, p); }, true, true},
    {LVAE_WGRAD_VARIANT_BF16, [](auto d, auto& p) { return conv3x3_wgrad_bf16_plan(d, p); }, true, true},
    {LVAE_WGRAD_VARIANT_WINO, [](auto d, auto& p) { return conv_wgrad_wino_plan(d, p); }, true, true},
    {LVAE_WGRAD_VARIANT_DIRECT_1X1, [](auto d, auto& p) { return conv1x1_wgrad_plan(d, p); }, false, false},
    {LVAE_WGRAD_VARIANT_TILE, [](auto d, auto& p) { return conv_wgrad_tile_plan(d, p); }, true, false},
    {LVAE_WGRAD_VARIANT_THIN, thin_wgrad_plan, false, false},
    {LVAE_WGRAD_VARIANT_GENERIC, generic_wgrad_plan, false, false},
};

static WgradPlan wgrad_route(const lvae_conv_desc* d, bool dy16, bool ws16) {
  static const bool halo_off = tune("LVAE_DISABLE_HALO", 0) != 0;
  for (const WgradFamily& f : kWgradFamilies) {
    WgradPlan p;
    p.variant = f.variant;
    if ((f.dy16 && !dy16) || (f.ws16 && !ws16) || (halo_off && f.variant != LVAE_WGRAD_VARIANT_GENERIC)) continue;
    if (f.plan(d, p)) return p;
  }
  return WgradPlan{};
}

static int wgrad_launch(const WgradOp* o, int n, hipStream_t s) {
  switch (o->plan.variant) {
    case LVAE_WGRAD_VARIANT_IMG: return conv_wgrad_img_grouped(o, n, s);
    case LVAE_WGRAD_VARIANT_BF16: return conv3x3_wgrad_bf16_launch(*o, s);
    case LVAE_WGRAD_VARIANT_WINO: return conv_wgrad_wino_launch(o, n, s);
    case LVAE_WGRAD_VARIANT_DIRECT_1X1: return conv1x1_wgrad_launch(*o, s);
    case LVAE_WGRAD_VARIANT_TILE: return conv_wgrad_tile_launch(o, n, s);
    case LVAE_WGRAD_VARIANT_THIN: return thin_wgrad_launch(*o, s);
    default: return generic_wgrad_launch(*o, s);
  }
}

static const std::pair<int32_t, int> kWgradGroupings[] = {
    {LVAE_WGRAD_VARIANT_TILE, kWgradTileGroup}, {LVAE_WGRAD_VARIANT_WINO, kWgradWinoGroup}, {LVAE_WGRAD_VARIANT_IMG, kWgradImgGroup}};
constexpr int kWgradMaxGroup = std::max({kWgradTileGroup, kWgradWinoGroup, kWgradImgGroup});

static std::vector<std::vector<int>> wgrad_schedule(const WgradOp* ops, int n) {
  std::vector<std::vector<int>> launches;
  std::vector<char> grouped(n, 0);
  for (const auto& [variant, cap] : kWgradGroupings) {
    std::map<int32_t, std::vector<int>> members;
    for (int i = 0; i < n; ++i)
      if (ops[i].plan.variant == variant && ops[i].plan.group >= 0) members[ops[i].plan.group].push_back(i);
    for (const auto& km : members)
      for (size_t m0 = 0; m0 < km.second.size(); m0 += cap) {
        const size_t m1 = std::min(km.second.size(), m0 + cap);
        if (m1 - m0 == 1 && variant != LVAE_WGRAD_VARIANT_IMG) continue;
        launches.emplace_back(km.second.begin() + m0, km.second.begin() + m1);
        for (const int i : launches.back()) grouped[i] = 1;
      }
  }
  for (int i = 0; i < n; ++i)
    if (!grouped[i]) launches.push_back({i});
  return launches;
}

static int wgrad_op_check(const WgradOp& o, size_t have, const char* who) {
  LVAE_REQUIRE(have >= o.plan.workspace, LVAE_EWORKSPACE,
               "%s: workspace %zu < %zu (the kernel taken for this dy / workspace alignment; lvae_conv2d_wgrad_workspace assumes 16-byte "
               "aligned ones)", who, have, o.plan.workspace);
  LVAE_REQUIRE((o.d->x_dtype == LVAE_DT_F32 && o.d->y_dtype == LVAE_DT_F32) || o.plan.takes_bf16_storage, LVAE_EINVAL,
               "%s: bf16-stored x / dy need the bf16 weight-gradient kernel, which does not take this shape (lvae_resblock_bf16_storage(d) == 0)", who);
  return 0;
}

}

using namespace lvae;

extern "C" size_t lvae_conv2d_wgrad_workspace(const lvae_conv_desc* d) { return d ? wgrad_route(d, true, true).workspace : 0; }

extern "C" int32_t lvae_conv2d_wgrad_variant(const lvae_conv_desc* d) {
  return d ? wgrad_route(d, true, true).variant : LVAE_WGRAD_VARIANT_GENERIC;
}

extern "C" int32_t lvae_conv2d_wgrad_apply_ok(const lvae_conv_desc* d) { return d && wgrad_route(d, true, true).apply_ok ? 1 : 0; }

extern "C" int lvae_conv2d_wgrad_f32(const lvae_conv_desc* d, const float* dy, float* dw, float* db, void* workspace,
                                     size_t workspace_bytes, void* stream) {
  int rc = conv_desc_check(d, "lvae_conv2d_wgrad_f32");
  if (rc) return rc;
  LVAE_REQUIRE(dy && dw && workspace, LVAE_EINVAL, "lvae_conv2d_wgrad_f32: null dy/dw/workspace");
  const WgradOp o{d, wgrad_route(d, al16(dy), al16(workspace)), dy, dw, db, workspace};
  rc = wgrad_op_check(o, workspace_bytes, "lvae_conv2d_wgrad_f32");
  return rc ? rc : wgrad_launch(&o, 1, (hipStream_t)stream);
}

extern "C" int lvae_conv2d_wgrad_apply_f32(const lvae_conv_desc* d, const lvae_bn_apply* ap, float* dw, float* db, void* workspace,
                                           size_t workspace_bytes, void* stream) {
  const char* who = "lvae_conv2d_wgrad_apply_f32";
  int rc = conv_desc_check(d, who);
  if (rc) return rc;
  const WgradOp o{d, wgrad_route(d, true, true), nullptr, dw, db, workspace};
  LVAE_REQUIRE(o.plan.apply_ok, LVAE_EINVAL,
               "%s: shape not supported (the Winograd-domain fp32 weight gradient of a 64 -> 64 layer, W = 16 or 32): "
               "use lvae_affine_act_bwd_parts_f32 + lvae_conv2d_wgrad_f32", who);
  LVAE_REQUIRE(ap && ap->parts && ap->rows > 0 && ap->M == (int64_t)d->N * d->H * d->W && ap->coef && ap->dh && ap->x && ap->out && ap->add == nullptr &&
                   ap->dh_bf16 == 0 && dw && workspace,
               LVAE_EINVAL, "%s: needs parts / rows, M = N*H*W, the coefficient block, fp32 dh, x and out, no add", who);
  LVAE_REQUIRE(workspace_bytes >= o.plan.workspace, LVAE_EWORKSPACE, "%s: workspace %zu < %zu", who, workspace_bytes, o.plan.workspace);
  const void* const operand[] = {workspace, ap->parts, ap->coef, ap->dh, ap->x, ap->out, ap->drop};
  const char* const name[] = {"workspace", "ap->parts", "ap->coef", "ap->dh", "ap->x", "ap->out", "ap->drop"};
  for (int i = 0; i < 7; ++i) LVAE_REQUIRE(al16_or_null(operand[i]), LVAE_EALIGN, "%s: %s must be 16-byte aligned", who, name[i]);
  return conv_wgrad_wino_apply_launch(o, ap, (hipStream_t)stream);
}

static bool wgrad_pair_route(const lvae_conv_desc* a, const lvae_conv_desc* b, WgradPlan& pa, WgradPlan& pb, int32_t* sched) {
  if (!a || !b) return false;
  pa = wgrad_route(a, true, true);
  pb = wgrad_route(b, true, true);
  if (pa.variant != LVAE_WGRAD_VARIANT_WINO || pb.variant != LVAE_WGRAD_VARIANT_WINO || !pa.apply_ok) return false;
  const bool same = a->N == b->N && a->H == b->H && a->W == b->W && a->OH == b->OH && a->OW == b->OW && a->C1 == b->C1 && a->C2 == b->C2 &&
                    a->KH == b->KH && a->KW == b->KW && a->stride == b->stride && a->pad == b->pad && a->gather == b->gather;
  const auto f32 = [](const lvae_conv_desc* d) { return d->precision == LVAE_PREC_F32 && d->x_dtype == LVAE_DT_F32 && d->y_dtype == LVAE_DT_F32; };
  if (!same || a->Cout != 64 || b->Cout != 64 || !f32(a) || !f32(b)) return false;
  return conv_wgrad_wino_pair_plan(a, b, pa, pb, sched);
}
static size_t wgrad_piece(const WgradPlan& aligned) { return (aligned.workspace + 255) / 256 * 256; }

extern "C" int32_t lvae_conv2d_wgrad_pair_ok(const lvae_conv_desc* a, const lvae_conv_desc* b) {
  WgradPlan pa, pb;
  return wgrad_pair_route(a, b, pa, pb, nullptr) ? 1 : 0;
}

extern "C" size_t lvae_conv2d_wgrad_pair_workspace(const lvae_conv_desc* a, const lvae_conv_desc* b) {
  WgradPlan pa, pb;
  return wgrad_pair_route(a, b, pa, pb, nullptr) ? wgrad_piece(pa) + wgrad_piece(pb) : 0;
}

extern "C" int32_t lvae_conv2d_wgrad_pair_schedule(const lvae_conv_desc* a, const lvae_conv_desc* b, int32_t* sched) {
  WgradPlan pa, pb;
  return sched && wgrad_pair_route(a, b, pa, pb, sched) ? 1 : 0;
}

extern "C" int lvae_conv2d_wgrad_pair_f32(const lvae_conv_desc* a, const lvae_bn_apply* ap, const lvae_conv_desc* b, const float* dy_b,
                                          float* dw_a, float* db_a, float* dw_b, float* db_b, void* workspace, size_t workspace_bytes,
                                          void* stream) {
  const char* who = "lvae_conv2d_wgrad_pair_f32";
  int rc = conv_desc_check(a, who);
  if (!rc) rc = conv_desc_check(b, who);
  if (rc) return rc;
  WgradPlan pa, pb;
  LVAE_REQUIRE(wgrad_pair_route(a, b, pa, pb, nullptr), LVAE_EINVAL,
               "%s: not a pair (two Winograd-domain fp32 weight gradients of 64 -> 64 layers of one geometry, W = 16 or 32, fp32 storage; "
               "lvae_conv2d_wgrad_pair_ok): use lvae_conv2d_wgrad_apply_f32 + lvae_conv2d_wgrad_f32", who);
  LVAE_REQUIRE(ap && ap->parts && ap->rows > 0 && ap->M == (int64_t)a->N * a->H * a->W && ap->coef && ap->dh && ap->x && ap->out && ap->add == nullptr &&
                   ap->dh_bf16 == 0 && dy_b && dw_a && dw_b && workspace,
               LVAE_EINVAL, "%s: needs parts / rows, M = N*H*W, the coefficient block, fp32 dh, x and out, no add; dy of B, both dw, workspace", who);
  const size_t piece_a = wgrad_piece(pa), need = piece_a + wgrad_piece(pb);
  LVAE_REQUIRE(workspace_bytes >= need, LVAE_EWORKSPACE, "%s: workspace %zu < %zu", who, workspace_bytes, need);
  const void* const operand[] = {workspace, ap->parts, ap->coef, ap->dh, ap->x, ap->out, ap->drop, dy_b};
  const char* const name[] = {"workspace", "ap->parts", "ap->coef", "ap->dh", "ap->x", "ap->out", "ap->drop", "dy_b"};
  for (int i = 0; i < 8; ++i) LVAE_REQUIRE(al16_or_null(operand[i]), LVAE_EALIGN, "%s: %s must be 16-byte aligned", who, name[i]);
  const WgradOp oa{a, pa, nullptr, dw_a, db_a, workspace}, ob{b, pb, dy_b, dw_b, db_b, static_cast<char*>(workspace) + piece_a};
  return conv_wgrad_wino_pair_launch(oa, ap, ob, (hipStream_t)stream);
}

extern "C" int lvae_conv2d_wgrad_bf16(const lvae_conv_desc* d, const float* dy, float* dw, float* db, void* workspace,
                                      size_t workspace_bytes, void* stream) {
  LVAE_REQUIRE(d != nullptr, LVAE_EINVAL, "lvae_conv2d_wgrad_bf16: null descriptor");
  lvae_conv_desc dd = *d;
  dd.precision = LVAE_PREC_BF16;
  return lvae_conv2d_wgrad_f32(&dd, dy, dw, db, workspace, workspace_bytes, stream);
}


extern "C" size_t lvae_conv2d_wgrad_grouped_workspace(const lvae_conv_desc* descs, int32_t n) {
  size_t tot = 0;
  for (int i = 0; descs && i < n; ++i) tot += wgrad_piece(wgrad_route(&descs[i], true, true));
  return tot;
}

extern "C" int32_t lvae_conv2d_wgrad_grouped_schedule(const lvae_conv_desc* descs, int32_t n, int32_t* launch_of) {
  if (!descs || !launch_of || n <= 0) return 0;
  std::vector<WgradOp> ops(n);
  for (int i = 0; i < n; ++i) ops[i].plan = wgrad_route(&descs[i], true, true);
  const std::vector<std::vector<int>> launches = wgrad_schedule(ops.data(), n);
  for (size_t l = 0; l < launches.size(); ++l)
    for (const int i : launches[l]) launch_of[i] = (int32_t)l;
  return (int32_t)launches.size();
}

extern "C" int lvae_conv2d_wgrad_grouped_f32(const lvae_conv_desc* descs, const float* const* dy, float* const* dw,
                                             float* const* db, int32_t n, void* workspace, size_t workspace_bytes,
                                             void* stream) {
  const char* who = "lvae_conv2d_wgrad_grouped_f32";
  LVAE_REQUIRE(descs && dy && dw && db && n > 0 && n <= 4096 && workspace, LVAE_EINVAL, "%s: bad arguments", who);
  std::vector<WgradOp> ops(n);
  char* ws = static_cast<char*>(workspace);
  for (int i = 0; i < n; ++i) {
    const lvae_conv_desc* d = &descs[i];
    int rc = conv_desc_check(d, who);
    if (rc) return rc;
    LVAE_REQUIRE(dy[i] && dw[i], LVAE_EINVAL, "%s: null dy/dw at %d", who, i);
    WgradPlan p = wgrad_route(d, true, true);
    const size_t piece = wgrad_piece(p);
    LVAE_REQUIRE((size_t)(ws - static_cast<char*>(workspace)) + piece <= workspace_bytes, LVAE_EWORKSPACE, "%s: workspace %zu < %zu", who,
                 workspace_bytes, lvae_conv2d_wgrad_grouped_workspace(descs, n));
    if (!al16(dy[i]) || !al16(ws)) p = wgrad_route(d, al16(dy[i]), al16(ws));
    ops[i] = WgradOp{d, p, dy[i], dw[i], db[i], ws};
    char entry[64];
    snprintf(entry, sizeof entry, "%s: entry %d", who, i);
    rc = wgrad_op_check(ops[i], piece, entry);
    if (rc) return rc;
    ws += piece;
  }
  WgradOp group[kWgradMaxGroup];
  for (const std::vector<int>& l : wgrad_schedule(ops.data(), n)) {
    for (size_t j = 0; j < l.size(); ++j) group[j] = ops[l[j]];
    const int rc = wgrad_launch(group, (int)l.size(), (hipStream_t)stream);
    if (rc) return rc;
  }
  return 0;
}
```

ladder-vae-pytorch_amd/csrc/lvae_host.h:

```cpp
#pragma once
#include "lvae_common.h"

namespace lvae {

struct ConvPlan {
  int32_t variant = LVAE_VARIANT_DIRECT;
  int32_t rows = 0;
  bool folds = false;
  size_t workspace = 0;
};

struct ReduceArgs {
  const float* slab_w;
  const float* slab_b;
  int ksplit, ntaps, Cin, Cout;
  int64_t stap, sk, sn;
  float* dw;
  float* db;
};
constexpr int kMaxReduceGroup = 12;

struct WgradPlan {
  int32_t variant = LVAE_WGRAD_VARIANT_GENERIC;
  int32_t group = -1;
  int32_t slabs = 0;
  size_t w_floats = 0, b_floats = 0;
  size_t workspace = 0;
  bool takes_bf16_storage = false, apply_ok = false;
  void set_slabs(int n, size_t w, size_t b) { slabs = n, w_floats = w, b_floats = b, workspace = (size_t)n * (w + b) * sizeof(float); }
};

struct WgradOp {
  const lvae_conv_desc* d;
  WgradPlan plan;
  const float* dy;
  float *dw, *db;
  void* workspace;
  float* slab_w() const { return static_cast<float*>(workspace); }
  float* slab_b() const { return db ? slab_w() + (size_t)plan.slabs * plan.w_floats : nullptr; }
};
constexpr int kWgradTileGroup = 12, kWgradWinoGroup = 12, kWgradImgGroup = 32;

int conv_desc_check(const lvae_conv_desc* d, const char* who);

bool conv3x3_halo_plan(const lvae_conv_desc* d, ConvPlan& p);
int conv3x3_halo_launch(const lvae_conv_desc* d, hipStream_t s);

bool conv3x3_pos_plan(const lvae_conv_desc* d, ConvPlan& p);
int conv3x3_pos_launch(const lvae_conv_desc* d, hipStream_t s);

bool conv3x3_resample_plan(const lvae_conv_desc* d, ConvPlan& p);
int conv3x3_resample_launch(const lvae_conv_desc* d, hipStream_t s);

bool conv3x3_wino_plan(const lvae_conv_desc* d, bool assume_ws, ConvPlan& p);
int conv3x3_wino_launch(const lvae_conv_desc* d, hipStream_t s);
int conv3x3_wino2_gate_rows(const lvae_conv_desc* d);
int conv3x3_wino2_gate_launch(const lvae_conv_desc* d, const lvae_rb_ext* gate, hipStream_t s);

int conv3x3_bf16_form(const lvae_conv_desc* d);
bool conv3x3_bf16_plan(const lvae_conv_desc* d, bool assume_ws, ConvPlan& p);
int conv3x3_bf16_launch(const lvae_conv_desc* d, const ConvPlan& p, hipStream_t s);
size_t conv3x3_bf16_workspace(const lvae_conv_desc* d, int split);
void conv3x3_bf16_prep_entry(const lvae_conv_desc* d, int split, void* entry);
int conv3x3_bf16_prepare_single(const lvae_conv_desc* d, int split, hipStream_t s);
int conv3x3_bf16_prepare_batched(const void* entries, int n, int npad, hipStream_t s);
size_t resblock_gate_ws_bytes(const lvae_conv_desc* d, int planes);
void resblock_gate_prep_entry(const lvae_conv_desc* d, int planes, void* entry);
int resblock_gate_prepare_single(const lvae_conv_desc* d, int planes, hipStream_t s);
bool conv3x3_wgrad_bf16_plan(const lvae_conv_desc* d, WgradPlan& p);
int conv3x3_wgrad_bf16_launch(const WgradOp& o, hipStream_t s);

enum { PW_PLAIN, PW_GATE_FWD, PW_GATE_BWD, PW_DGRAD_CAT };
struct PwForm {
  int kind = PW_PLAIN;
  int act = 0;
  const float* res = nullptr;
  float* out = nullptr;
  const float* dout = nullptr;
  const float* ab = nullptr;
  float* dab = nullptr;
  float* y2 = nullptr;
  int split = 0;
};
bool conv1x1_plan(const lvae_conv_desc* d, const PwForm& f, ConvPlan& p);
int conv1x1_launch(const lvae_conv_desc* d, const PwForm& f, hipStream_t s);

bool conv1x1_gate_fwd_plan(const lvae_conv_desc* d, ConvPlan& p);
int conv1x1_gate_fwd_launch(const lvae_conv_desc* d, const ConvPlan& p, const float* res, float* out, int act, hipStream_t s);

bool conv1x1_gate_bwd_fused_plan(const lvae_conv_desc* d, bool with_apply, ConvPlan& p);

void wgrad_reduce_launch(const float* slab_w, const float* slab_b, int ksplit, int ntaps, int Cin, int Cout, int64_t stap,
                         int64_t sk, int64_t sn, float* dw, float* db, hipStream_t s);
void wgrad_reduce_grouped_launch(const ReduceArgs* r, int n, hipStream_t s);
int wgrad_op_reduce(const WgradOp& o, hipStream_t s);

bool conv_wgrad_img_plan(const lvae_conv_desc* d, WgradPlan& p);
int conv_wgrad_img_grouped(const WgradOp* o, int n, hipStream_t s);

bool conv_wgrad_tile_plan(const lvae_conv_desc* d, WgradPlan& p);
int conv_wgrad_tile_launch(const WgradOp* o, int n, hipStream_t s);

bool conv_wgrad_wino_plan(const lvae_conv_desc* d, WgradPlan& p);
int conv_wgrad_wino_launch(const WgradOp* o, int n, hipStream_t s);
int conv_wgrad_wino_apply_launch(const WgradOp& o, const lvae_bn_apply* ap, hipStream_t s);
bool conv_wgrad_wino_pair_plan(const lvae_conv_desc* da, const lvae_conv_desc* db, WgradPlan& pa, WgradPlan& pb, int32_t* sched);
int conv_wgrad_wino_pair_launch(const WgradOp& a, const lvae_bn_apply* ap, const WgradOp& b, hipStream_t s);

bool conv1x1_wgrad_plan(const lvae_conv_desc* d, WgradPlan& p);
int conv1x1_wgrad_launch(const WgradOp& o, hipStream_t s);

template <auto Kern, typename Args>
int launch_lds(const char* name, dim3 grid, dim3 block, size_t lds, int max_lds, hipStream_t s, const Args& a) {
  static std::atomic<bool> attr_set{false};
  if (!attr_set) {
    hipError_t e = hipFuncSetAttribute(reinterpret_cast<const void*>(Kern), hipFuncAttributeMaxDynamicSharedMemorySize, max_lds);
    if (e != hipSuccess) {
      set_error("%s: hipFuncSetAttribute failed: %s", name, hipGetErrorString(e));
      return (int)e;
    }
    attr_set = true;
  }
  hipLaunchKernelGGL(Kern, grid, block, lds, s, a);
  LVAE_LAUNCH_CHECK(name);
  return 0;
}

}
```

ladder-vae-pytorch_amd/kernels.py:

```python
import ctypes as C
import weakref

import torch

from . import _C
from ._C import ACT, BnFold, ConvDesc, RbExt, GATHER_CONV, GATHER_TRANSPOSED, PREC_BF16, PREC_F32, call, ptr, ptr_dt, stream_ptr

_ws_cache = {}

precision = PREC_F32


form = _C.FORM_AUTO


class use_form:
    def __init__(self, f):
        self.f = f

    def __enter__(self):
        global form
        self.prev, form = form, self.f

    def __exit__(self, *exc):
# ... 392 lines not shown
    return int(_C.load().lvae_resblock_conv_rows(C.byref(d))) if d is not None else 0


def _rb_query_desc(x, weight, g):
    if _ddi is not None or x.dtype != torch.float32 or x.dim() != 4 or g.transposed or g.KH != 3 or g.stride != 1 or g.pad != 1:
        return None
    N, H, W, _ = x.shape
    return _desc(g, weight, x, None, N, H, W, H, W, g.Cout, g.s_ci, g.s_co, GATHER_CONV)


def _in_bn(d, in_bn, x, can_fold=True, coef=None):
    if in_bn is None:
        d.in_scale, d.in_shift = ptr(coef[0]), ptr(coef[1])
        return coef, None
    sp, pivot, bn = in_bn
    N, H, W, C1 = x.shape
    M = N * H * W
    if sp.has_pivot and can_fold:
        coef = torch.empty((4, C1), dtype=torch.float32, device=x.device)
        fold = BnFold(ptr(sp.buf), sp.rows, M, ptr(bn.weight), ptr(bn.bias), bn.eps, bn.momentum, ptr(bn.running_mean),
                      ptr(bn.running_var), ptr(coef))
        d.in_fold = C.addressof(fold)
        return (coef[0], coef[1], coef[2], coef[3]), fold
    coef = bn_finalize_parts(sp.rows_view(), M, pivot, bn.weight, bn.bias, bn.running_mean, bn.running_var, bn.eps, bn.momentum)
    d.in_scale, d.in_shift = ptr(coef[0]), ptr(coef[1])
    return coef, None


def rb_weight_ranges(x_like, weight, g, dgrad, gate=None, gate_bwd=False):
    d, need = _rb_desc(x_like, weight, g, dgrad)
    out = [(int(d.workspace), int(need), d._ws_tensor)] if need else []
    if gate is not None:
        e = RbExt()
        _rb_gate_ws(e, gate[0], gate[1], x_like.device, gate_bwd)
        out.append((int(e.gate_ws), int(e.gate_ws_bytes), e._ws_tensor))
    return out


def _rb_prefetch(e, prefetch):
    for i, rng in enumerate((prefetch or [])[:2]):
        e.pf_ptr[i], e.pf_bytes[i] = rng[0], rng[1]


def rb_conv(x, weight, g, bias, in_act, out_scale, in_bn=None, coef=None, stats_pivot=None, prefetch=None):
    N, H, W, _ = x.shape
    y = torch.empty((N, H, W, g.Cout), dtype=torch.float32, device=x.device)
    d, _ = _rb_desc(x, weight, g, False, y, bias, None, None, in_act, out_scale)
    coef, keep = _in_bn(d, in_bn, x, coef=coef)
    parts = None
    if stats_pivot is not None:
        rows = _C.load().lvae_resblock_conv_rows(C.byref(d))
        buf = torch.empty((rows + 1, 2, g.Cout), dtype=torch.float32, device=x.device)
        parts = StatParts(buf, rows, True)
        d.stats_out, d.stats_pivot = ptr(buf), ptr(stats_pivot)
    e = RbExt()
    e.prologue, e.epilogue = _C.RB_PRO_AFFINE, _C.RB_EPI_PLAIN
    _rb_prefetch(e, prefetch)
    call('lvae_resblock_conv_f32', C.byref(d), C.byref(e), stream_ptr())
    del keep
    return y, parts, coef


def rb_gate_rows(x, weight, g, whole_image=True):
    d = _rb_query_desc(x, weight, g)
    if d is None:
        return 0
    rows = int(_C.load().lvae_resblock_conv_rows(C.byref(d)))
    if rows > 0:
        return rows if whole_image else 0
    _conv_ws(d, weight, x.device)
    return int(_C.load().lvae_resblock_conv_gate_rows(C.byref(d)))


def rb_conv_gate(x, weight, g, bias, in_act, out_scale, gate_w, gate_g, gate_bias, res, act, in_bn=None, coef=None, stats_pivot=None,
                 prefetch=None, want_ab=True):
    N, H, W, _ = x.shape
    dev = x.device
    y = torch.empty((N, H, W, g.Cout), dtype=torch.float32, device=dev)
    out = torch.empty((N, H, W, gate_g.Cout // 2), dtype=torch.float32, device=dev)
    d, need = _rb_desc(x, weight, g, False, y, bias, None, None, in_act, out_scale)
    if need and not want_ab:
        raise _C.LvaeHipError("rb_conv_gate: the whole-image kernels always store ab")
    ab = torch.empty((N, H, W, gate_g.Cout), dtype=torch.float32, device=dev) if want_ab else None
    can_fold = True
    if not need:
        _conv_ws(d, weight, dev)
        can_fold = bool(_C.load().lvae_conv2d_folds_bn_finalize(C.byref(d)))
    coef, keep = _in_bn(d, in_bn, x, can_fold, coef)
    e = RbExt()
    e.prologue, e.epilogue = _C.RB_PRO_AFFINE, _C.RB_EPI_GATE
    _rb_gate_ws(e, gate_w, gate_g, dev, False)
    e.gate_bias, e.act = ptr(gate_bias), ACT[act]
    e.res, e.ab, e.out = ptr(res), ptr(ab), ptr(out)
    parts = None
    if stats_pivot is not None:
        rows = _C.load().lvae_resblock_conv_gate_rows(C.byref(d))
        buf = torch.empty((rows + 1, 2, g.Cout), dtype=torch.float32, device=dev)
        parts = StatParts(buf, rows, True)
        e.out_stats, e.out_stats_pivot = ptr(buf), ptr(stats_pivot)
    _rb_prefetch(e, prefetch)
    call('lvae_resblock_conv_f32', C.byref(d), C.byref(e), stream_ptr())
    del keep
    return y, ab, out, parts, coef


def _rb_bn_bwd(d, bn_bwd, dx):
    xb, coef0, act = bn_bwd
    rows = _C.load().lvae_resblock_conv_rows(C.byref(d))
    parts = torch.empty((rows, 2, dx.shape[3]), dtype=torch.float32, device=dx.device)
    d.stats_out, d.stats_pivot, d.stats_x = ptr(parts), ptr(coef0), ptr(xb)
    d.stats_mode, d.stats_act = 1, ACT[act]
    return parts


class PendingApply:
    __slots__ = ('parts', 'dh', 'x', 'coef0', 'act', 'dgamma', 'dbeta', 'add', 'out')

    def __init__(self, parts, dh, x, coef0, act, dgamma, dbeta, add, out):
        self.parts, self.dh, self.x, self.coef0, self.act, self.dgamma, self.dbeta, self.add, self.out = parts, dh, x, coef0, act, dgamma, dbeta, add, out


def rb_gate_dgrad(dout, ab, gate_w, gate_g, act, drop, weight, g, bn_bwd, prefetch=None, apply=None):
    N, H, W, Cn = dout.shape
    dev = dout.device
    dab = torch.empty_like(ab)
    dy2 = torch.empty((N, H, W, Cn), dtype=torch.float32, device=dev)
    dh = torch.empty((N, H, W, g.Cin), dtype=torch.float32, device=dev)
    d, _ = _rb_desc(dout, weight, g, True, dh)
    e = RbExt()
    e.prologue, e.epilogue = _C.RB_PRO_GATE_BWD, _C.RB_EPI_PLAIN
    _rb_gate_ws(e, gate_w, gate_g, dev, True)
    e.act = ACT[act]
    e.dout, e.ab_in, e.dab, e.pro_drop, e.xt_out = ptr(dout), ptr(ab), ptr(dab), ptr(drop), ptr(dy2)
    if apply is not None:
        e.ap_parts, e.ap_rows, e.ap_act, e.ap_M = ptr(apply.parts), apply.parts.shape[0], ACT[apply.act], N * H * W
        e.ap_coef, e.ap_dh, e.ap_x, e.ap_add = ptr(apply.coef0), ptr(apply.dh), ptr(apply.x), ptr(apply.add)
        e.ap_dgamma, e.ap_dbeta, e.ap_out = ptr(apply.dgamma), ptr(apply.dbeta), ptr(apply.out)
    parts = _rb_bn_bwd(d, bn_bwd, dh)
    _rb_prefetch(e, prefetch)
    call('lvae_resblock_conv_f32', C.byref(d), C.byref(e), stream_ptr())
    return dab, dy2, dh, parts


def rb_apply_dgrad(parts_in, dh_in, x_bn, coef0, act, dgamma, dbeta, drop, weight, g, bn_bwd, prefetch=None):
    N, H, W, Cn = dh_in.shape
    dev = dh_in.device
    dy1 = torch.empty((N, H, W, Cn), dtype=torch.float32, device=dev)
    dh = torch.empty((N, H, W, g.Cin), dtype=torch.float32, device=dev)
    d, _ = _rb_desc(dh_in, weight, g, True, dh)
    e = RbExt()
    e.prologue, e.epilogue = _C.RB_PRO_BN_APPLY, _C.RB_EPI_PLAIN
    e.bwd_parts, e.bwd_rows, e.bwd_act, e.bwd_M = ptr(parts_in), parts_in.shape[0], ACT[act], N * H * W
    e.bwd_coef, e.bwd_x, e.dgamma, e.dbeta, e.pro_drop, e.xt_out = ptr(coef0), ptr(x_bn), ptr(dgamma), ptr(dbeta), ptr(drop), ptr(dy1)
    parts = _rb_bn_bwd(d, bn_bwd, dh)
    _rb_prefetch(e, prefetch)
    call('lvae_resblock_conv_f32', C.byref(d), C.byref(e), stream_ptr())
    return dy1, dh, parts


def bn_coef_block(scale, shift, mean, rstd):
    if scale is None or shift is None or mean is None or rstd is None:
        return False
    n = 4 * scale.numel()
    p0 = scale.data_ptr()
    return shift.data_ptr() == p0 + n and mean.data_ptr() == p0 + 2 * n and rstd.data_ptr() == p0 + 3 * n


def affine_act_bwd_parts(parts, dh, x, scale, shift, act, mean, rstd, dgamma, dbeta, drop=None, add=None, out_bf16=False, out=None):
    Cn = x.shape[-1]
    M = x.numel() // Cn
    dx = out if out is not None else torch.empty(x.shape, dtype=torch.bfloat16 if out_bf16 else torch.float32, device=x.device)
    ws = workspace(8 * Cn, x.device)
    rows_per_n = M // x.shape[0]
    dtypes = _dt(dh) | (_dt(x) << 1) | (_dt(dx) << 2)
    call('lvae_affine_act_bwd_parts_f32', ptr(parts), parts.shape[0], ptr_dt(dh), ptr_dt(x), M, Cn, ptr(scale), ptr(shift), ACT[act],
         ptr(mean), ptr(rstd), ptr(dgamma), ptr(dbeta), ptr(drop), rows_per_n, ptr(add), ptr_dt(dx), ws.data_ptr(), ws.numel(),
         dtypes, stream_ptr())
    return dx


def conv2d_dgrad(dy, weight, g, in_hw, out_scale=None, ci_range=None, bn_bwd=None, out_bf16=False):
    _chk_nhwc(dy, 'dy')
    N, OH, OW, Co = dy.shape
    H, W = in_hw
    a, b = ci_range if ci_range is not None else (0, g.Cin)
    dx = torch.empty((N, H, W, b - a), dtype=torch.bfloat16 if out_bf16 else torch.float32, device=dy.device)
    d = _desc(g, weight, dy, None, N, OH, OW, H, W, b - a, g.s_co, g.s_ci,
              GATHER_CONV if g.transposed else GATHER_TRANSPOSED, out_scale=out_scale, y=dx)
    d.w = ptr(weight) + 4 * a * g.s_ci
    _conv_ws(d, weight, dy.device)
    if bn_bwd is None:
        call('lvae_conv2d_f32', C.byref(d), stream_ptr())
        return dx
    xb, coef, act = bn_bwd
    parts = None
    rows = _C.load().lvae_conv2d_stats_rows(C.byref(d))
    if rows > 0 and out_scale is None and ci_range is None and tuple(xb.shape) == tuple(dx.shape):
        parts = torch.empty((rows, 2, b - a), dtype=torch.float32, device=dy.device)
        d.stats_out, d.stats_pivot, d.stats_x = ptr(parts), ptr(coef), ptr_dt(xb)
        d.stats_mode, d.stats_act, d.stats_x_dtype = 1, ACT[act], _dt(xb)
    call('lvae_conv2d_f32', C.byref(d), stream_ptr())
    return dx, parts


def conv2d_wgrad_apply_ok(x, weight, g):
    if precision != PREC_F32 or x.dtype != torch.float32 or x.dim() != 4 or g.transposed or _ddi is not None:
        return False
    N, H, W, _ = x.shape
    d = _desc(g, weight, x, None, N, H, W, H, W, g.Cout, g.s_ci, g.s_co, GATHER_CONV)
    return bool(_C.load().lvae_conv2d_wgrad_apply_ok(C.byref(d)))


def conv2d_wgrad_apply(x, weight, g, dweight, dbias, parts, dh, xbn, coef0, act, dgamma, dbeta, drop=None, in_scale=None, in_shift=None, in_act=None):
    _chk_nhwc(x, 'x')
    N, H, W, _ = x.shape
    if tuple(dweight.stride()) != tuple(weight.stride()):
        raise _C.LvaeHipError("conv2d_wgrad_apply: gradient strides differ from weight strides")
    d = _desc(g, weight, x, None, N, H, W, H, W, g.Cout, g.s_ci, g.s_co, GATHER_CONV, None, in_scale, in_shift, in_act)
    need = _C.load().lvae_conv2d_wgrad_workspace(C.byref(d))
    ws = workspace(need, x.device)
    dy = torch.empty((N, H, W, g.Cout), dtype=torch.float32, device=x.device)
    ap = _C.BnApply(ptr(parts), parts.shape[0], ACT[act], N * H * W, ptr(coef0), ptr(dh), ptr(xbn), None, ptr(dgamma), ptr(dbeta), ptr(dy), 0, 0, ptr(drop))
    call('lvae_conv2d_wgrad_apply_f32', C.byref(d), C.byref(ap), ptr(dweight), ptr(dbias), ws.data_ptr(), ws.numel(), stream_ptr())
    return dy


def _wgrad_pair_descs(x_a, w_a, g_a, x_b, w_b, g_b, in_a=(None, None, None), in_b=(None, None, None)):
    if precision != PREC_F32 or _ddi is not None or g_a.transposed or g_b.transposed:
        return None
    if x_a.dim() != 4 or x_b.dim() != 4:
        return None
    N, H, W, _ = x_a.shape
    d_a = _desc(g_a, w_a, x_a, None, N, H, W, H, W, g_a.Cout, g_a.s_ci, g_a.s_co, GATHER_CONV, None, *in_a)
    N, H, W, _ = x_b.shape
    d_b = _desc(g_b, w_b, x_b, None, N, H, W, H, W, g_b.Cout, g_b.s_ci, g_b.s_co, GATHER_CONV, None, *in_b)
    return d_a, d_b


def conv2d_wgrad_pair_ok(x_a, w_a, g_a, x_b, w_b, g_b):
    ds = _wgrad_pair_descs(x_a, w_a, g_a, x_b, w_b, g_b)
    return ds is not None and bool(_C.load().lvae_conv2d_wgrad_pair_ok(C.byref(ds[0]), C.byref(ds[1])))


def conv2d_wgrad_pair_schedule(x_a, w_a, g_a, x_b, w_b, g_b):
    ds = _wgrad_pair_descs(x_a, w_a, g_a, x_b, w_b, g_b)
    out = (C.c_int32 * 6)()
    if ds is None or not _C.load().lvae_conv2d_wgrad_pair_schedule(C.byref(ds[0]), C.byref(ds[1]), out):
        return None
    return tuple(out[:3]), tuple(out[3:])


def conv2d_wgrad_pair(x, weight, g, dweight, dbias, parts, dh, xbn, coef0, act, dgamma, dbeta, dy_b, weight_b, g_b, dweight_b, dbias_b,
                      drop=None, in_scale=None, in_shift=None, in_act=None, in_scale_b=None, in_shift_b=None, in_act_b=None, out=None):
    _chk_nhwc(x, 'x')
    _chk_nhwc(xbn, 'xbn')
    _chk_nhwc(dy_b, 'dy_b')
    N, H, W, _ = x.shape
    if tuple(dweight.stride()) != tuple(weight.stride()) or tuple(dweight_b.stride()) != tuple(weight_b.stride()):
        raise _C.LvaeHipError("conv2d_wgrad_pair: gradient strides differ from weight strides")
    ds = _wgrad_pair_descs(x, weight, g, xbn, weight_b, g_b, (in_scale, in_shift, in_act), (in_scale_b, in_shift_b, in_act_b))
    if ds is None:
        raise _C.LvaeHipError("conv2d_wgrad_pair: not a pair (fp32 precision, plain convolutions)")
    d_a, d_b = ds
    d_b.y_dtype = _dt(dy_b)
    need = _C.load().lvae_conv2d_wgrad_pair_workspace(C.byref(d_a), C.byref(d_b))
    ws = workspace(need, x.device)
    dy = out if out is not None else torch.empty((N, H, W, g.Cout), dtype=torch.float32, device=x.device)
    ap = _C.BnApply(ptr(parts), parts.shape[0], ACT[act], N * H * W, ptr(coef0), ptr(dh), ptr(xbn), None, ptr(dgamma), ptr(dbeta), ptr(dy), 0, 0, ptr(drop))
    call('lvae_conv2d_wgrad_pair_f32', C.byref(d_a), C.byref(ap), C.byref(d_b), ptr_dt(dy_b), ptr(dweight), ptr(dbias), ptr(dweight_b), ptr(dbias_b),
         ws.data_ptr(), ws.numel(), stream_ptr())
    return dy


def conv1x1_dgrad_cat(dy, weight, g, C1):
    _chk_nhwc(dy, 'dy')
    N, H, W, _ = dy.shape
    if not 0 < C1 < g.Cin:
        return None
    dx = torch.empty((N, H, W, C1), dtype=torch.float32, device=dy.device)
    dx2 = torch.empty((N, H, W, g.Cin - C1), dtype=torch.float32, device=dy.device)
    d = _desc(g, weight, dy, None, N, H, W, H, W, g.Cin, g.s_co, g.s_ci, GATHER_TRANSPOSED, y=dx)
    if not _C.load().lvae_conv1x1_dgrad_cat_ok(C.byref(d), C1):
        return None
    call('lvae_conv1x1_dgrad_cat_f32', C.byref(d), ptr(dx2), C1, stream_ptr())
    return dx, dx2


def conv2d_wgrad(x, dy, weight, g, dweight, dbias=None, x2=None, in_scale=None, in_shift=None, in_act=None):
    _chk_nhwc(x, 'x')
    _chk_nhwc(dy, 'dy')
    N, H, W, _ = x.shape
    OH, OW = dy.shape[1], dy.shape[2]
    if tuple(dweight.stride()) != tuple(weight.stride()):
        raise _C.LvaeHipError("conv2d_wgrad: gradient strides %s differ from weight strides %s" %
                              (tuple(dweight.stride()), tuple(weight.stride())))
    d = _desc(g, weight, x, x2, N, H, W, OH, OW, g.Cout, g.s_ci, g.s_co,
              GATHER_TRANSPOSED if g.transposed else GATHER_CONV, None, in_scale, in_shift, in_act)
    d.y_dtype = _dt(dy)
    need = _C.load().lvae_conv2d_wgrad_workspace(C.byref(d))
    ws = workspace(need, x.device)
    call('lvae_conv2d_wgrad_f32', C.byref(d), ptr_dt(dy), ptr(dweight), ptr(dbias), ws.data_ptr(), ws.numel(), stream_ptr())


def conv2d_wgrad_grouped(items):
    n = len(items)
    descs = (ConvDesc * n)()
    dys, dws, dbs = (C.c_void_p * n)(), (C.c_void_p * n)(), (C.c_void_p * n)()
    for i, (x, dy, weight, g, dweight, dbias, kw) in enumerate(items):
        _chk_nhwc(x, 'x')
        _chk_nhwc(dy, 'dy')
        if tuple(dweight.stride()) != tuple(weight.stride()):
            raise _C.LvaeHipError("conv2d_wgrad_grouped: gradient strides %s differ from weight strides %s" %
                                  (tuple(dweight.stride()), tuple(weight.stride())))
        N, H, W, _ = x.shape
        d = _desc(g, weight, x, kw.get('x2'), N, H, W, dy.shape[1], dy.shape[2], g.Cout, g.s_ci, g.s_co,
                  GATHER_TRANSPOSED if g.transposed else GATHER_CONV, None, kw.get('in_scale'), kw.get('in_shift'), kw.get('in_act'))
        d.y_dtype = _dt(dy)
        C.memmove(C.byref(descs, i * C.sizeof(ConvDesc)), C.byref(d), C.sizeof(ConvDesc))
        dys[i], dws[i], dbs[i] = ptr_dt(dy), ptr(dweight), ptr(dbias)
    need = _C.load().lvae_conv2d_wgrad_grouped_workspace(descs, n)
    ws = workspace(need, items[0][0].device)
    call('lvae_conv2d_wgrad_grouped_f32', descs, C.cast(dys, C.c_void_p), C.cast(dws, C.c_void_p), C.cast(dbs, C.c_void_p), n,
         ws.data_ptr(), ws.numel(), stream_ptr())


def bn_stats(x, gamma, beta, running_mean, running_var, eps=1e-5, momentum=0.1):
    Cn = x.shape[-1]
    M = x.numel() // Cn
    out = torch.empty((4, Cn), dtype=torch.float32, device=x.device)
    need = _C.load().lvae_bn_stats_workspace(M, Cn)
    ws = workspace(need, x.device)
    call('lvae_bn_stats_f32', ptr(x), M, Cn, ptr(gamma), ptr(beta), eps, momentum, ptr(running_mean), ptr(running_var),
         ptr(out[0]), ptr(out[1]), ptr(out[2]), ptr(out[3]), ws.data_ptr(), ws.numel(), stream_ptr())
    return out[0], out[1], out[2], out[3]


def bn_finalize_parts(parts, M, pivot, gamma, beta, running_mean, running_var, eps=1e-5, momentum=0.1):
    rows, _, Cn = parts.shape
    out = torch.empty((4, Cn), dtype=torch.float32, device=parts.device)
    call('lvae_bn_finalize_parts_f32', ptr(parts), rows, M, Cn, ptr(pivot), ptr(gamma), ptr(beta), eps, momentum,
         ptr(running_mean), ptr(running_var), ptr(out[0]), ptr(out[1]), ptr(out[2]), ptr(out[3]), stream_ptr())
    return out[0], out[1], out[2], out[3]


def bn_eval_coeffs(gamma, beta, running_mean, running_var, eps=1e-5):
    Cn = running_mean.numel()
    out = torch.empty((2, Cn), dtype=torch.float32, device=running_mean.device)
    call('lvae_bn_eval_coeffs_f32', Cn, ptr(gamma), ptr(beta), ptr(running_mean), ptr(running_var), eps, ptr(out[0]),
         ptr(out[1]), stream_ptr())
    return out[0], out[1]


def affine_act(x, scale, shift, act, row_scale=None):
    Cn = x.shape[-1]
    M = x.numel() // Cn
    y = torch.empty_like(x)
    rows_per_n = M // x.shape[0]
    call('lvae_affine_act_f32', ptr(x), M, Cn, ptr(scale), ptr(shift), ACT[act], ptr(row_scale), rows_per_n, ptr(y),
         stream_ptr())
    return y


def affine_act_bwd(dh, x, scale, shift, act, bn_train, mean=None, rstd=None, dgamma=None, dbeta=None, drop=None, add=None):
    Cn = x.shape[-1]
    M = x.numel() // Cn
    dx = torch.empty_like(x)
    need = _C.load().lvae_bn_stats_workspace(M, Cn)
    ws = workspace(need, x.device)
    rows_per_n = M // x.shape[0]
    call('lvae_affine_act_bwd_f32', ptr(dh), ptr(x), M, Cn, ptr(scale), ptr(shift), ACT[act], int(bool(bn_train)),
         ptr(mean), ptr(rstd), ptr(dgamma), ptr(dbeta), ptr(drop), rows_per_n, ptr(add), ptr(dx), ws.data_ptr(),
         ws.numel(), stream_ptr())
    return dx


def gate_fwd(ab, res, act):
    Cn = ab.shape[-1] // 2
    M = ab.numel() // (2 * Cn)
    out = torch.empty(ab.shape[:-1] + (Cn,), dtype=torch.float32, device=ab.device)
    call('lvae_gate_fwd_f32', ptr(ab), ptr(res), M, Cn, ACT[act], ptr(out), stream_ptr())
    return out


def gate_bwd(dout, ab, act):
    Cn = ab.shape[-1] // 2
    M = ab.numel() // (2 * Cn)
    dab = torch.empty_like(ab)
    call('lvae_gate_bwd_f32', ptr(dout), ptr(ab), M, Cn, ACT[act], ptr(dab), stream_ptr())
    return dab


def act_bwd_from_out(dy, y, act):
    dx = torch.empty_like(y)
    call('lvae_act_bwd_from_out_f32', ptr(dy), ptr(y), y.numel(), ACT[act], ptr(dx), stream_ptr())
    return dx


def add(a, b):
    out = torch.empty_like(a)
    call('lvae_add_f32', ptr(a), ptr(b), a.numel(), ptr(out), stream_ptr())
    return out


def fill(t, value=0.0):
    call('lvae_fill_f32', ptr(t), t.numel(), float(value), stream_ptr())
    return t


def fill_zero(t):
    z = _zeros_like_cached(t)
    call('lvae_scale_rows_add_f32', ptr(z), None, 1, 1, None, t.numel(), ptr(t), stream_ptr())
    return t


_zero_cache = {}


def _zeros_like_cached(t):
    key = (t.device, t.numel())
    if key not in _zero_cache:
        _zero_cache[key] = torch.zeros(t.numel(), dtype=torch.float32, device=t.device)
    return _zero_cache[key]


def add3(a, b, c):
    out = torch.empty_like(a)
    call('lvae_add3_f32', ptr(a), ptr(b), ptr(c), a.numel(), ptr(out), stream_ptr())
    return out


def sum_of_row_means(x_ln):
    L, N = x_ln.shape
    out = torch.empty((1,), dtype=torch.float32, device=x_ln.device)
    call('lvae_sum_of_row_means_f32', ptr(x_ln), L, N, ptr(out), stream_ptr())
    return out


def scale_rows_add(a, row_scale, b, out=None):
    Cn = a.shape[-1]
    M = a.numel() // Cn
    if out is None:
        out = torch.empty_like(a)
    call('lvae_scale_rows_add_f32', ptr(a), ptr(row_scale), M // a.shape[0], Cn, ptr(b), M, ptr(out), stream_ptr())
    return out


def colsum(x2d, out, accumulate):
    R, P = x2d.shape
    call('lvae_colsum_f32', ptr(x2d), R, P, ptr(out), int(bool(accumulate)), stream_ptr())


def normal_stochastic_fwd(p, q, eps_or_z, mode, analytical_kl, Z, N, rows=None):
    p_bcast = int(p.shape[0] == 1 and N > 1)
    _, H, W, _ = p.shape
    dev = p.device
    z = torch.empty((N, H, W, Z), dtype=torch.float32, device=dev)
    small = torch.empty((3, N), dtype=torch.float32, device=dev)
    if rows is not None:
        small = [rows[0], small[1], rows[1]]
    ks = torch.empty((N, H, W), dtype=torch.float32, device=dev) if q is not None else None
    call('lvae_normal_stochastic_fwd_f32', ptr(p), p_bcast, ptr(q), ptr(eps_or_z), N, H * W, Z, mode, int(bool(analytical_kl)),
         ptr(z), ptr(small[0]), ptr(small[1]) if q is not None else None, ptr(small[2]) if q is not None else None, ptr(ks),
         stream_ptr())
    if q is None:
        return z, small[0], None, None, None
    return z, small[0], small[1], small[2], ks


def _stoch_block_desc(x_p, cv_p, p_given, x_q, cv_q, cv_out, eps_or_z, mode, analytical_kl, N, attach=True):
    if _ddi is not None or x_q is None or x_q.dim() != 4 or x_q.dtype != torch.float32 or not x_q.is_contiguous():
        return None
    _, H, W, _ = x_q.shape
    b = _C.StochBlock()
    keep = []
    for name, cv, x, cin in (('conv_p', cv_p, x_p, None), ('conv_q', cv_q, x_q, None), ('conv_out', cv_out, None, cv_out[1].Cin)):
        if cv is None:
            continue
        w, g, bias = cv
        if g.transposed or (x is not None and (x.dim() != 4 or x.dtype != torch.float32 or not x.is_contiguous() or tuple(x.shape[:3]) != (N, H, W))):
            return None
        d = ConvDesc()
        d.x = ptr(x)
        d.C1 = x.shape[3] if x is not None else cin
        d.w, d.w_stap, d.w_sk, d.w_sn, d.bias = ptr(w), g.s_tap, g.s_ci, g.s_co, ptr(bias)
        d.N, d.H, d.W, d.OH, d.OW, d.Cout = N, H, W, H, W, g.Cout
        d.KH, d.KW, d.stride, d.pad, d.gather, d.precision = g.KH, g.KW, g.stride, g.pad, GATHER_CONV, precision
        if d.C1 != g.Cin:
            return None
        if attach:
            need = _C.load().lvae_stoch_block_workspace(C.byref(d))
            if not need:
                return None
            prepared.attach(d, w, x_q.device, need, 'lvae_stoch_block_prepare_entry')
            keep.append(d._ws_tensor)
        setattr(b, name, d)
    if cv_p is None:
        if p_given is None or p_given.dim() != 4 or p_given.dtype != torch.float32 or not p_given.is_contiguous() or tuple(p_given.shape[1:3]) != (H, W):
            return None
        b.p_given, b.p_bcast = ptr(p_given), int(p_given.shape[0] == 1 and N > 1)
        if p_given.shape[0] not in (1, N) or p_given.shape[3] != cv_q[1].Cout:
            return None
    b.mode, b.analytical_kl, b.eps = mode, int(bool(analytical_kl)), ptr(eps_or_z)
    b._keep = keep
    return b


def stoch_block_ok(x_p, cv_p, p_given, x_q, cv_q, cv_out, mode, N):
    b = _stoch_block_desc(x_p, cv_p, p_given, x_q, cv_q, cv_out, None, mode, False, N, attach=False)
    return b is not None and bool(_C.load().lvae_stoch_block_ok(C.byref(b)))


def stoch_block_fwd(x_p, cv_p, p_given, x_q, cv_q, cv_out, eps_or_z, mode, analytical_kl, N, rows=None):
    b = _stoch_block_desc(x_p, cv_p, p_given, x_q, cv_q, cv_out, eps_or_z, mode, analytical_kl, N)
    if b is None:
        raise _C.LvaeHipError("stoch_block_fwd: not a call of the fused stochastic block (ask stoch_block_ok first)")
    _, H, W, _ = x_q.shape
    dev, Z = x_q.device, cv_out[1].Cin
    q_params = torch.empty((N, H, W, cv_q[1].Cout), dtype=torch.float32, device=dev)
    p_params = torch.empty_like(q_params) if cv_p is not None else p_given
    z = torch.empty((N, H, W, Z), dtype=torch.float32, device=dev)
    out = torch.empty((N, H, W, cv_out[1].Cout), dtype=torch.float32, device=dev)
    small = torch.empty((3, N), dtype=torch.float32, device=dev)
    if rows is not None:
        small = [rows[0], small[1], rows[1]]
    ks = torch.empty((N, H, W), dtype=torch.float32, device=dev)
    if cv_p is not None:
        b.conv_p.y = ptr(p_params)
    b.conv_q.y, b.conv_out.x, b.conv_out.y = ptr(q_params), ptr(z), ptr(out)
    b.logprob_p, b.logprob_q, b.kl_samplewise, b.kl_spatial = ptr(small[0]), ptr(small[1]), ptr(small[2]), ptr(ks)
    call('lvae_stoch_block_fwd_f32', C.byref(b), stream_ptr())
    return out, z, p_params, q_params, small[0], small[1], small[2], ks


def stoch_block_bwd(d_out, cv_p, cv_q, cv_out, p, q, z, eps, dz, g_lp, g_lq, g_kl, g_ks, mode, analytical_kl):
    if _ddi is not None or any(t is None or t.dtype != torch.float32 or not t.is_contiguous() for t in (d_out, p, q, z)):
        return None
    N, H, W, _ = z.shape
    dev = z.device
    b = _C.StochBlockBwd()
    keep = []
    dq = torch.empty_like(q)
    dp = torch.empty_like(q)
    dxq = torch.empty((N, H, W, cv_q[1].Cin), dtype=torch.float32, device=dev)
    dxp = torch.empty((N, H, W, cv_p[1].Cin), dtype=torch.float32, device=dev) if cv_p is not None else None
    for name, cv, x, y in (('dgrad_out', cv_out, d_out, None), ('dgrad_q', cv_q, dq, dxq), ('dgrad_p', cv_p, dp, dxp)):
        d = ConvDesc()
        d.x, d.y = ptr(x), ptr(y)
        if cv is not None:
            w, g, _ = cv
            if g.transposed or tuple(x.shape) != (N, H, W, g.Cout):
                return None
            d.C1, d.Cout = g.Cout, g.Cin
            d.w, d.w_stap, d.w_sk, d.w_sn = ptr(w), g.s_tap, g.s_co, g.s_ci
            d.N, d.H, d.W, d.OH, d.OW = N, H, W, H, W
            d.KH, d.KW, d.stride, d.pad, d.gather, d.precision = g.KH, g.KW, g.stride, g.pad, GATHER_TRANSPOSED, precision
            need = _C.load().lvae_stoch_block_workspace(C.byref(d))
            if not need:
                return None
            prepared.attach(d, w, dev, need, 'lvae_stoch_block_prepare_entry')
            keep.append(d._ws_tensor)
        setattr(b, name, d)
    b.p, b.p_bcast, b.q, b.z, b.eps, b.dz = ptr(p), int(p.shape[0] == 1 and N > 1), ptr(q), ptr(z), ptr(eps), ptr(dz)
    b.g_lp, b.g_lq, b.g_kl, b.g_ks = ptr(g_lp), ptr(g_lq), ptr(g_kl), ptr(g_ks)
    b.mode, b.analytical_kl = mode, int(bool(analytical_kl))
    if not _C.load().lvae_stoch_block_bwd_ok(C.byref(b)):
        return None
    call('lvae_stoch_block_bwd_f32', C.byref(b), stream_ptr())
    del keep
    return dp, dq, dxp, dxq


def normal_prior_sample(p, eps, Z, N, temperature, row_temperature=None, rows=None):
    p_bcast = int(p.shape[0] == 1 and N > 1)
    _, H, W, _ = p.shape
    if row_temperature is not None and (row_temperature.dtype != torch.float32 or tuple(row_temperature.shape) != (N,)):
        raise ValueError("row_temperature must be a float32 tensor of shape (%d,), got %s %s"
                         % (N, row_temperature.dtype, tuple(row_temperature.shape)))
    z = torch.empty((N, H, W, Z), dtype=torch.float32, device=p.device)
    lp = rows[0] if rows is not None else torch.empty((N,), dtype=torch.float32, device=p.device)
    call('lvae_normal_prior_sample_f32', ptr(p), p_bcast, ptr(eps), float(temperature),
         ptr(None if row_temperature is None else row_temperature.contiguous()), N, H * W, Z, ptr(z), ptr(lp), stream_ptr())
    return z, lp


INTERP_MODES = {'lerp': 0, 'slerp': 1}


def latent_interp(za, zb, t, mode='slerp'):
    if mode not in INTERP_MODES:
        raise ValueError("mode must be 'slerp' or 'lerp', got %r" % (mode,))
    if tuple(za.shape) != tuple(zb.shape) or za.dim() < 1:
        raise ValueError("za and zb must have one shape (B, ...), got %s and %s" % (tuple(za.shape), tuple(zb.shape)))
    if t.dim() != 1:
        raise ValueError("t must have shape (T,), got %s" % (tuple(t.shape),))
    pa, pb, pt = ptr(za, (torch.float32,)), ptr(zb, (torch.float32,)), ptr(t, (torch.float32,))
    if not (za.is_contiguous() and zb.is_contiguous() and t.is_contiguous()):
        raise _C.LvaeHipError("latent_interp: za, zb and t must be contiguous, got strides %s, %s, %s" % (za.stride(), zb.stride(), t.stride()))
    B, T = int(za.shape[0]), int(t.shape[0])
    n = za.numel() // B if B > 0 else 0
    out = torch.empty((T * B,) + tuple(za.shape[1:]), dtype=torch.float32, device=za.device)
    ws = workspace(_C.load().lvae_latent_interp_workspace(B, T), za.device)
    call('lvae_latent_interp_f32', pa, pb, pt, B, n, T, INTERP_MODES[mode], ptr(out), ws.data_ptr(), ws.numel(), stream_ptr())
    return out


def normal_stochastic_bwd(p, q, eps, z, dz, g_lp, g_lq, g_kl, g_ks, mode, analytical_kl, Z):
    N, H, W, _ = z.shape
    p_bcast = int(p.shape[0] == 1 and N > 1)
    dp = torch.empty((N, H, W, 2 * Z), dtype=torch.float32, device=z.device)
    dq = torch.empty_like(dp) if q is not None else None
    call('lvae_normal_stochastic_bwd_f32', ptr(p), p_bcast, ptr(q), ptr(eps), ptr(z), ptr(dz), ptr(g_lp), ptr(g_lq),
         ptr(g_kl), ptr(g_ks), N, H * W, Z, mode, int(bool(analytical_kl)), ptr(dp), ptr(dq), stream_ptr())
    return dp, dq


def kl_elementwise_fwd(p, q, z, analytical_kl):
    N, H, W, Z = z.shape
    out = torch.empty_like(z)
    call('lvae_kl_elementwise_fwd_f32', ptr(p), int(p.shape[0] == 1 and N > 1), ptr(q), int(q.shape[0] == 1 and N > 1), ptr(z),
         N, H * W, Z, int(bool(analytical_kl)), ptr(out), stream_ptr())
    return out

# ... 549 lines not shown
```

ladder-vae-pytorch_amd/lib/stochastic.py:

```python
import torch
from torch import nn

from .. import kernels as K
from .. import ops
from .. import resblock as RB
from .nn import Conv2dParams


class NormalStochasticBlock2d(nn.Module):

    def __init__(self, c_in, c_vars, c_out, kernel=3, transform_p_params=True):
        super().__init__()
        assert kernel % 2 == 1
        pad = kernel // 2
        self.transform_p_params = transform_p_params
        self.c_in, self.c_out, self.c_vars = c_in, c_out, c_vars
        if transform_p_params:
            self.conv_in_p = Conv2dParams(c_in, 2 * c_vars, kernel, padding=pad)
        self.conv_in_q = Conv2dParams(c_in, 2 * c_vars, kernel, padding=pad)
        self.conv_out = Conv2dParams(c_vars, c_out, kernel, padding=pad)

    def forward(self, p_params, q_params=None, forced_latent=None, use_mode=False, force_constant_output=False,
                analytical_kl=False, noise=None, n_img=None, need_kl_elementwise=True, rows=None, stats=None, temperature=None):
        assert (forced_latent is None) or (not use_mode)
        tempered = temperature is not None and (torch.is_tensor(temperature) or float(temperature) != 1.0)
        if tempered and (q_params is not None or forced_latent is not None or use_mode):
            raise ValueError("temperature applies to a draw from the prior: it cannot be combined with q_params, forced_latent or use_mode")
        if not self.transform_p_params:
            assert p_params.size(3) == 2 * self.c_vars
        if q_params is not None and not tempered and not need_kl_elementwise and not force_constant_output and RB.switches.stoch_block:
            fused = self._fused(p_params, q_params, forced_latent, use_mode, analytical_kl, noise, n_img, rows, stats)
            if fused is not None:
                return fused
        if self.transform_p_params:
            p_params = self.conv_in_p(p_params)
        if q_params is not None:
            q_params = self.conv_in_q(q_params)
        ref = q_params if q_params is not None else p_params
        N = ref.shape[0] if n_img is None else n_img
        H, W = ref.shape[1], ref.shape[2]
        dev = ref.device
        if tempered:
            return self._tempered(p_params, temperature, force_constant_output, noise, N, H, W, rows)
        if forced_latent is not None:
            mode, src = 2, forced_latent.contiguous()
        elif use_mode:
            mode, src = 1, None
        else:
            mode, src = 0, noise.normal((N, H, W, self.c_vars), dev)
        outs = ops.NormalStochFn.apply(p_params, q_params, src, mode, bool(analytical_kl), self.c_vars, N, rows)
        if stats is not None and q_params is not None:
            with torch.no_grad():
                K.latent_stats_fold(p_params.detach(), q_params.detach(), stats, N)
        z = outs[0]
        if force_constant_output:
            if torch.is_grad_enabled() and z.requires_grad:
                raise RuntimeError("force_constant_output is a sampling-time option; run it under torch.no_grad()")
            z = z[0:1].expand_as(z).contiguous()
            p_params = p_params[0:1].expand(N, -1, -1, -1).contiguous()
        out = self.conv_out(z)
        data = {'z': z, 'p_params': p_params, 'q_params': q_params, 'logprob_p': outs[1], 'logprob_q': None,
                'kl_elementwise': None, 'kl_samplewise': None, 'kl_spatial': None}
        if q_params is not None:
            data['logprob_q'], data['kl_samplewise'], data['kl_spatial'] = outs[2], outs[3], outs[4]
            if need_kl_elementwise:
                data['kl_elementwise'] = ops.KlElementwiseFn.apply(z, p_params, q_params, bool(analytical_kl))
        return out, data

    def _fused(self, p_in, q_in, forced_latent, use_mode, analytical_kl, noise, n_img, rows, stats):
        has_p = self.transform_p_params
        N = q_in.shape[0] if n_img is None else n_img
        cv = lambda m: (m.weight, m.geom(), m.bias)
        mode = 2 if forced_latent is not None else 1 if use_mode else 0
        if not K.stoch_block_ok(p_in if has_p else None, cv(self.conv_in_p) if has_p else None, None if has_p else p_in, q_in,
                                cv(self.conv_in_q), cv(self.conv_out), mode, N):
            return None
        H, W = q_in.shape[1], q_in.shape[2]
        src = forced_latent.contiguous() if mode == 2 else None if mode == 1 else noise.normal((N, H, W, self.c_vars), q_in.device)
        params = [t for m in ((self.conv_in_p,) if has_p else ()) + (self.conv_in_q, self.conv_out) for t in (m.weight, m.bias)]
        outs = ops.StochBlockFn.apply(p_in if has_p else None, None if has_p else p_in, q_in, src, self, mode, bool(analytical_kl), N, rows, *params)
        out, z, q_params, lp, lq, kl, ks = outs[:7]
        p_params = outs[7] if has_p else p_in
        if stats is not None:
            with torch.no_grad():
                K.latent_stats_fold(p_params.detach(), q_params.detach(), stats, N)
        return out, {'z': z, 'p_params': p_params, 'q_params': q_params, 'logprob_p': lp, 'logprob_q': lq, 'kl_elementwise': None,
                     'kl_samplewise': kl, 'kl_spatial': ks}

    def _tempered(self, p_params, temperature, force_constant_output, noise, N, H, W, rows):
        if torch.is_grad_enabled() and p_params.requires_grad:
            raise RuntimeError("a tempered prior draw has no backward; run it under torch.no_grad()")
        p_params = p_params.detach()
        if torch.is_tensor(temperature):
            scalar, row_t = 1.0, temperature
        else:
            scalar, row_t = float(temperature), None
            if not (0.0 <= scalar < float('inf')):
                raise ValueError("temperature must be a finite number >= 0, got %r" % (temperature,))
        eps = None if row_t is None and scalar == 0.0 else noise.normal((N, H, W, self.c_vars), p_params.device)
        z, logprob_p = K.normal_prior_sample(p_params, eps, self.c_vars, N, scalar, row_t, rows=rows)
        if force_constant_output:
            z = z[0:1].expand_as(z).contiguous()
            p_params = p_params[0:1].expand(N, -1, -1, -1).contiguous()
        out = self.conv_out(z)
        return out, {'z': z, 'p_params': p_params, 'q_params': None, 'logprob_p': logprob_p, 'logprob_q': None,
                     'kl_elementwise': None, 'kl_samplewise': None, 'kl_spatial': None}


def kl_normal_mc(z, p_mulv, q_mulv):
    return ops.KlElementwiseFn.apply(z.contiguous(), p_mulv.contiguous(), q_mulv.contiguous(), False)
```

ladder-vae-pytorch_amd/ops.py:

```python
from types import SimpleNamespace

import torch
from torch.autograd import Function

from . import kernels as K
from . import resblock as RB

_const_cache = {}


def _ones_zeros(C, device):
    key = (C, device)
    if key not in _const_cache:
        _const_cache[key] = (torch.ones(C, device=device), torch.zeros(C, device=device))
    return _const_cache[key]


def grad_buf(p):
    if not p.requires_grad:
        return None
    if p.grad is None:
        p.grad = torch.zeros_like(p)
    return p.grad


def _c(t):
    return t if t.is_contiguous() else t.contiguous()


_side = {'stream': None}


def set_wgrad_stream(streams):
    if streams is None:
        _side['stream'] = None
    else:
        _side['stream'] = list(streams) if isinstance(streams, (list, tuple)) else [streams]


def join_wgrad_stream():
    sts = _side['stream']
    if sts is not None:
        for st in sts:
            torch.cuda.current_stream().wait_stream(st)


def set_wgrad_grouping(max_rows, flush_at=None):
    flush_wgrad_group()
    _side['group_rows'] = max_rows
    _side['group_at'] = RB.switches.wgrad_flush if flush_at is None else flush_at


def flush_wgrad_group():
    q, _side['group_q'] = _side.get('group_q') or [], []
    if len(q) == 1:
        x, dy, w, g, dw, db, kw = q[0]
        K.conv2d_wgrad(x, dy, w, g, dw, db, **kw)
    elif q:
        K.conv2d_wgrad_grouped(q)


def drop_wgrad_group():
    _side['group_q'] = []


def wgrad(x, dy, w, g, dw, db, **kw):
    rows = _side.get('group_rows')
    if rows is not None and x.shape[0] * x.shape[1] * x.shape[2] <= rows:
        q = _side.setdefault('group_q', [])
        if any(e[4].data_ptr() == dw.data_ptr() for e in q):
            flush_wgrad_group()
            q = _side['group_q']
        q.append((x, dy, w, g, dw, db, kw))
        if len(q) >= _side.get('group_at', 1024):
            flush_wgrad_group()
        return
    sts = _side['stream']
    if sts is None:
        return K.conv2d_wgrad(x, dy, w, g, dw, db, **kw)
    st = sts[(dw.data_ptr() >> 8) % len(sts)]
    st.wait_stream(torch.cuda.current_stream())
    with torch.cuda.stream(st):
        K.conv2d_wgrad(x, dy, w, g, dw, db, **kw)
    for t in (x, dy, kw.get('x2'), kw.get('in_scale'), kw.get('in_shift')):
        if t is not None:
            t.record_stream(st)


class ConvFn(Function):

    @staticmethod
    def forward(ctx, x, x2, mod, out_act, weight, bias):
        g = mod.geom()
        y = K.conv2d(x, weight, g, bias=bias, x2=x2, out_act=out_act)
        ctx.mod, ctx.out_act, ctx.g = mod, out_act, g
        ctx.has_x2 = x2 is not None
        ctx.save_for_backward(x, x2, y if out_act else None)
        return y

    @staticmethod
    def backward(ctx, dy):
        x, x2, y = ctx.saved_tensors
        mod, g = ctx.mod, ctx.g
        dy = _c(dy)
        if ctx.out_act:
            dy = K.act_bwd_from_out(dy, y, ctx.out_act)
        w = mod.weight
        if w.requires_grad:
            wgrad(x, dy, w, g, grad_buf(w), grad_buf(mod.bias) if mod.bias is not None else None, x2=x2)
        dx = dx2 = None
        hw = (x.shape[1], x.shape[2])
        if x2 is None:
            if ctx.needs_input_grad[0]:
                dx = K.conv2d_dgrad(dy, w, g, hw)
        else:
            C1 = x.shape[3]
            both = K.conv1x1_dgrad_cat(dy, w, g, C1) if (RB.switches.dgrad_cat and ctx.needs_input_grad[0] and ctx.needs_input_grad[1]) else None
            if both is not None:
                dx, dx2 = both
            else:
                if ctx.needs_input_grad[0]:
                    dx = K.conv2d_dgrad(dy, w, g, hw, ci_range=(0, C1))
                if ctx.needs_input_grad[1]:
                    dx2 = K.conv2d_dgrad(dy, w, g, hw, ci_range=(C1, g.Cin))
        return dx, dx2, None, None, None, None


def conv(x, mod, x2=None, out_act=None):
    return ConvFn.apply(x, x2, mod, out_act, mod.weight, mod.bias)


def _bn_of_half(h, bn, training, parts, pivot):
    if bn is None:
        return None, _ones_zeros(h.shape[3], h.device) + (None, None)
    if not training:
        return None, K.bn_eval_coeffs(bn.weight, bn.bias, bn.running_mean, bn.running_var, bn.eps) + (None, None)
    if parts is not None:
        return (parts, pivot, bn), None
    return None, K.bn_stats(h, bn.weight, bn.bias, bn.running_mean, bn.running_var, bn.eps, bn.momentum)


def _conv_half(h, bn, cv, act, m, training, parts, pivot, stats_pivot, s16):
    in_bn, coef = _bn_of_half(h, bn, training, parts, pivot)
    if in_bn is not None:
        return K.conv2d(h, cv.weight, cv.geom(), bias=cv.bias, in_act=act, out_scale=m, in_bn=in_bn, stats_pivot=stats_pivot, out_bf16=s16)
    r = K.conv2d(h, cv.weight, cv.geom(), bias=cv.bias, in_scale=coef[0], in_shift=coef[1], in_act=act, out_scale=m, stats_pivot=stats_pivot,
                 out_bf16=s16)
    return (r if stats_pivot is not None else (r, None)) + (coef,)


def _fwd_fused_gate(call, x, blk, m1, m2, training):
    act, st, bn2, cv1, cv2, gate = blk.act, blk.sched, blk.bn2, blk.conv1, blk.conv2, blk.gate
    whole = call.plan.forward == 'whole-image'
    if whole:
        in_bn, coef1 = _bn_of_half(x, blk.bn1, True, call.parts, call.pivot)
        st.link('fwd', K.rb_weight_ranges(x, cv1.weight, cv1.geom(), False))
        y1, parts2, coef1 = K.rb_conv(x, cv1.weight, cv1.geom(), cv1.bias, act, m1, in_bn=in_bn, coef=coef1, stats_pivot=bn2.running_mean,
                                      prefetch=K.rb_weight_ranges(x, cv2.weight, cv2.geom(), False, gate=(gate.weight, gate.geom())))
    else:
        y1, parts2, coef1 = _conv_half(x, blk.bn1, cv1, act, m1, True, call.parts, call.pivot, bn2.running_mean, False)
    in_bn, coef2 = _bn_of_half(y1, bn2, True, parts2, bn2.running_mean)
    call.out_pivot = coef1[2].detach() if call.plan.gate_stats else None
    y2, ab, out, call.out_parts, coef2 = K.rb_conv_gate(y1, cv2.weight, cv2.geom(), cv2.bias, act, m2, gate.weight, gate.geom(), gate.bias, x, act,
                                                        in_bn=in_bn, coef=coef2, stats_pivot=call.out_pivot,
                                                        prefetch=st.next_ranges('fwd') if whole else None,
                                                        want_ab=not call.plan.recompute_ab)
    return y1, y2, ab, out, coef1, coef2


def _fwd_per_op(call, x, blk, m1, m2, training):
    act, bn2, gate, s16 = blk.act, blk.bn2, blk.gate, call.plan.bf16_internals
    want_stats = training and bn2 is not None and bn2.running_mean is not None
    y1, parts2, coef1 = _conv_half(x, blk.bn1, blk.conv1, act, m1, training, call.parts, call.pivot, bn2.running_mean if want_stats else None, s16)
    y2, _, coef2 = _conv_half(y1, bn2, blk.conv2, act, m2, training, parts2, bn2.running_mean if bn2 is not None else None, None, s16)
    if gate is None:
        return y1, y2, None, K.add(y2, x), coef1, coef2
    call.out_pivot = coef1[2].detach() if call.plan.gate_stats else None
    r = K.conv1x1_gate(y2, gate.weight, gate.geom(), gate.bias, x, act, stats_pivot=call.out_pivot)
    ab, out, call.out_parts = r if call.out_pivot is not None else r + (None,)
    return y1, y2, ab, out, coef1, coef2


class ResBlockFn(Function):

    @staticmethod
    def forward(ctx, x, blk, m1, m2, training, call, *params):
        plan, fwd = call.plan, _fwd_fused_gate if call.plan.forward in ('whole-image', 'wino-gate') else _fwd_per_op
        y1, y2, ab, out, coef1, coef2 = fwd(call, x, blk, m1, m2, training)
        if plan.backward == 'whole-image' and not (K.bn_coef_block(*coef1) and K.bn_coef_block(*coef2)):
            call.plan = plan = plan._replace(backward='composed', accepts=None)
        ctx.blk, ctx.plan, ctx.training, ctx.defer = blk, plan, training, call.defer
        ctx.save_for_backward(x, y1, y2, ab, *coef1, *coef2, m1, m2)
        return out

    @staticmethod
    def backward(ctx, dout):
        blk, plan, act = ctx.blk, ctx.plan, ctx.blk.act
        x, y1, y2, ab, sc1, sh1, mean1, rstd1, sc2, sh2, mean2, rstd2, m1, m2 = ctx.saved_tensors
        coef1, coef2 = (sc1, sh1, mean1, rstd1), (sc2, sh2, mean2, rstd2)
        dout = _c(dout)
        if plan.backward == 'whole-image':
            dh1, parts1 = _bwd_whole_image(blk, dout, x, y1, y2, ab, coef1, coef2, m1, m2)
        else:
            dy2 = _bwd_gate(blk, plan, dout, y2, ab, m2)
            cv1, bn2 = blk.conv1, blk.bn2
            cv2 = blk.conv2
            paired = (plan.wgrad_pair and _side['stream'] is None and dy2.dtype == torch.float32 and bn2 is not None and ctx.training and
                      K.bn_coef_block(*coef2))
            dh2, parts2 = _bwd_half(ctx, cv2, bn2, y1, dy2, coef2, wgrad_done=paired)
            absorbed = (plan.wgrad_absorbs_apply and parts2 is not None and _side['stream'] is None and dh2.dtype == torch.float32)
            if paired and absorbed:
                dy1 = K.conv2d_wgrad_pair(x, cv1.weight, cv1.geom(), grad_buf(cv1.weight), grad_buf(cv1.bias), parts2, dh2, y1, sc2, act,
                                          grad_buf(bn2.weight), grad_buf(bn2.bias), dy2, cv2.weight, cv2.geom(), grad_buf(cv2.weight),
                                          grad_buf(cv2.bias), drop=m1, in_scale=sc1, in_shift=sh1, in_act=act, in_scale_b=sc2, in_shift_b=sh2,
                                          in_act_b=act)
            elif absorbed:
                dy1 = K.conv2d_wgrad_apply(x, cv1.weight, cv1.geom(), grad_buf(cv1.weight), grad_buf(cv1.bias), parts2, dh2, y1, sc2, act,
                                           grad_buf(bn2.weight), grad_buf(bn2.bias), drop=m1, in_scale=sc1, in_shift=sh1, in_act=act)
            else:
                if paired:
                    wgrad(y1, dy2, cv2.weight, cv2.geom(), grad_buf(cv2.weight), grad_buf(cv2.bias), in_scale=sc2, in_shift=sh2, in_act=act)
                dy1 = _bwd_apply(ctx, bn2, parts2, dh2, y1, coef2, drop=m1, out_bf16=plan.bf16_internals)
            dh1, parts1 = _bwd_half(ctx, cv1, blk.bn1, x, dy1, coef1, wgrad_done=absorbed)
        if parts1 is not None and ctx.defer is not None and (dh1.dtype == torch.float32 or ctx.defer[1] == 'any-dh') and K.bn_coef_block(*coef1):
            dx = torch.empty_like(x)
            ctx.defer[0].pending = K.PendingApply(parts1, dh1, x, sc1, act, grad_buf(blk.bn1.weight), grad_buf(blk.bn1.bias), dout, dx)
        else:
            dx = _bwd_apply(ctx, blk.bn1, parts1, dh1, x, coef1, add=dout)
        return (dx, None, None, None, None, None) + (None,) * (len(ctx.needs_input_grad) - 6)


def _bwd_whole_image(blk, dout, x, y1, y2, ab, coef1, coef2, m1, m2):
    act, st, gate, cv2, cv1, bn2 = blk.act, blk.sched, blk.gate, blk.conv2, blk.conv1, blk.bn2
    gw, w2, w1 = gate.weight, cv2.weight, cv1.weight
    st.link('bwd', K.rb_weight_ranges(dout, w2, cv2.geom(), True, gate=(gw, gate.geom()), gate_bwd=True))
    dab, dy2, dh2, parts2 = K.rb_gate_dgrad(dout, ab, gw, gate.geom(), act, m2, w2, cv2.geom(), bn_bwd=(y1, coef2[0], act),
                                            prefetch=K.rb_weight_ranges(dout, w1, cv1.geom(), True), apply=st.take_pending(dout))
    if gw.requires_grad:
        wgrad(y2, dab, gw, gate.geom(), grad_buf(gw), grad_buf(gate.bias))
    wgrad(y1, dy2, w2, cv2.geom(), grad_buf(w2), grad_buf(cv2.bias), in_scale=coef2[0], in_shift=coef2[1], in_act=act)
    dy1, dh1, parts1 = K.rb_apply_dgrad(parts2, dh2, y1, coef2[0], act, grad_buf(bn2.weight), grad_buf(bn2.bias), m1, w1, cv1.geom(),
                                        bn_bwd=(x, coef1[0], act), prefetch=st.next_ranges('bwd'))
    wgrad(x, dy1, w1, cv1.geom(), grad_buf(w1), grad_buf(cv1.bias), in_scale=coef1[0], in_shift=coef1[1], in_act=act)
    return dh1, parts1


def _bwd_gate(blk, plan, dout, y2, ab, m2):
    gate, act, s16 = blk.gate, blk.act, plan.bf16_internals
    if gate is None:
        return K.scale_rows_add(dout, m2, None) if m2 is not None else dout
    gw = gate.weight
    if plan.backward == 'persistent-gate':
        if plan.recompute_ab:
            dy2 = K.conv1x1_gate_bwd_wgrad_recompute(dout, y2, gw, gate.geom(), gate.bias, act, grad_buf(gw), grad_buf(gate.bias), out_scale=m2,
                                                     apply=blk.sched.take_pending(dout))
        else:
            dy2 = K.conv1x1_gate_bwd_wgrad(dout, ab, y2, gw, gate.geom(), act, grad_buf(gw), grad_buf(gate.bias), out_scale=m2, out_bf16=s16,
                                           apply=blk.sched.take_pending(dout))
        if dy2 is None:
            raise K._C.LvaeHipError("residual block: the persistent gate backward the block was planned with did not take this shape")
        return dy2
    if s16:
        raise K._C.LvaeHipError("bf16-stored residual block: the fused gate backward did not take this shape")
    dab, dy2 = K.conv1x1_gate_bwd(dout, ab, gw, gate.geom(), act, out_scale=m2)
    wgrad(y2, dab, gw, gate.geom(), grad_buf(gw), grad_buf(gate.bias))
    return dy2


def _bwd_half(ctx, cv, bn, h, dy, coef, wgrad_done=False):
    w, g, act = cv.weight, cv.geom(), ctx.blk.act
    if not wgrad_done:
        wgrad(h, dy, w, g, grad_buf(w), grad_buf(cv.bias), in_scale=coef[0], in_shift=coef[1], in_act=act)
    if bn is not None and ctx.training and K.bn_coef_block(*coef):
        return K.conv2d_dgrad(dy, w, g, h.shape[1:3], bn_bwd=(h, coef[0], act), out_bf16=ctx.plan.bf16_internals)
    return K.conv2d_dgrad(dy, w, g, h.shape[1:3]), None


def _bwd_apply(ctx, bn, parts, dh, h, coef, drop=None, add=None, out_bf16=False):
    sc, sh, mean, rstd = coef
    train = bn is not None and ctx.training
    dgamma, dbeta = (grad_buf(bn.weight), grad_buf(bn.bias)) if train else (None, None)
    if parts is not None:
        return K.affine_act_bwd_parts(parts, dh, h, sc, sh, ctx.blk.act, mean, rstd, dgamma, dbeta, drop=drop, add=add, out_bf16=out_bf16)
    return K.affine_act_bwd(dh, h, sc, sh, ctx.blk.act, train, mean, rstd, dgamma, dbeta, drop=drop, add=add)


def residual_block(x, blk, m1, m2):
    training = blk.training
    blk.sched.pending = None
    parts, pivot, defer = RB.received(x, training)
    call = SimpleNamespace(plan=RB.plan_block(blk, x, training), parts=parts, pivot=pivot, defer=defer, out_parts=None, out_pivot=None)
    out = ResBlockFn.apply(x, blk, m1, m2, training, call, *blk.parameters())
    return RB.tagged(out, blk, call.plan, call.out_parts, call.out_pivot)


class BnDropFn(Function):

    @staticmethod
    def forward(ctx, x, bn, mask, training, *params):
        _, (sc, sh, mean, rstd) = _bn_of_half(x, bn, training, None, None)
        y = K.affine_act(x, sc, sh, None, row_scale=mask)
        ctx.bn, ctx.training = bn, training
        ctx.save_for_backward(x, sc, sh, mean, rstd, mask)
        return y

    @staticmethod
    def backward(ctx, dy):
        x, sc, sh, mean, rstd, mask = ctx.saved_tensors
        dy = _c(dy)
        if mask is not None:
            dy = K.scale_rows_add(dy, mask, None)
        bn = ctx.bn
        train = bn is not None and ctx.training
        dx = K.affine_act_bwd(dy, x, sc, sh, None, train, mean, rstd, grad_buf(bn.weight) if train else None,
                              grad_buf(bn.bias) if train else None)
        return (dx, None, None, None) + (None,) * (len(ctx.needs_input_grad) - 4)


class GateFn(Function):

    @staticmethod
    def forward(ctx, ab, res, act):
        ctx.act = act
        ctx.has_res = res is not None
        ctx.save_for_backward(ab)
        return K.gate_fwd(ab, res, act)

    @staticmethod
    def backward(ctx, dout):
        (ab,) = ctx.saved_tensors
        dout = _c(dout)
        return K.gate_bwd(dout, ab, ctx.act), (dout if ctx.has_res else None), None


class AddFn(Function):
    @staticmethod
    def forward(ctx, a, b):
        return K.add(a, b)

    @staticmethod
    def backward(ctx, d):
        return d, d


class NormalStochFn(Function):

    @staticmethod
    def forward(ctx, p, q, noise, mode, analytical, Z, N, rows=None):
        z, lp, lq, kl, ks = K.normal_stochastic_fwd(p, q, noise, mode, analytical, Z, N, rows=rows)
        ctx.set_materialize_grads(False)
        ctx.mode, ctx.analytical, ctx.Z = mode, analytical, Z
        ctx.has_q = q is not None
        ctx.p_bcast = p.shape[0] == 1 and N > 1
        ctx.save_for_backward(p, q, noise if mode == 0 else None, z)
        if q is None:
            return z, lp
        return z, lp, lq, kl, ks

    @staticmethod
    def backward(ctx, dz, g_lp, g_lq=None, g_kl=None, g_ks=None):
        p, q, eps, z = ctx.saved_tensors
        cc = lambda t: None if t is None else _c(t)
        if dz is None and g_lp is None and g_lq is None and g_kl is None and g_ks is None:
            return None, None, None, None, None, None, None, None
        dp, dq = K.normal_stochastic_bwd(p, q, eps, z, cc(dz), cc(g_lp), cc(g_lq), cc(g_kl), cc(g_ks), ctx.mode,
                                         ctx.analytical, ctx.Z)
        if ctx.p_bcast:
            red = torch.empty_like(p)
            K.colsum(dp.view(dp.shape[0], -1), red.view(-1), False)
            dp = red
        return dp, dq, None, None, None, None, None, None


class StochBlockFn(Function):

    @staticmethod
    def forward(ctx, x_p, p_given, x_q, noise, blk, mode, analytical, N, rows, *params):
        cv = lambda m: (m.weight, m.geom(), m.bias)
        has_p = x_p is not None
        out, z, p, q, lp, lq, kl, ks = K.stoch_block_fwd(x_p, cv(blk.conv_in_p) if has_p else None, p_given, x_q, cv(blk.conv_in_q), cv(blk.conv_out),
                                                         noise, mode, analytical, N, rows=rows)
        ctx.set_materialize_grads(False)
        ctx.blk, ctx.mode, ctx.analytical, ctx.has_p = blk, mode, analytical, has_p
        ctx.p_bcast = p.shape[0] == 1 and N > 1
        ctx.save_for_backward(x_p, p, x_q, q, noise if mode == 0 else None, z)
        return (out, z, q, lp, lq, kl, ks) + ((p,) if has_p else ())

    @staticmethod
    def backward(ctx, d_out, dz, dq_out, g_lp, g_lq, g_kl, g_ks, dp_out=None):
        x_p, p, x_q, q, eps, z = ctx.saved_tensors
        none = (None,) * len(ctx.needs_input_grad)
        if all(g is None for g in (d_out, dz, dq_out, g_lp, g_lq, g_kl, g_ks, dp_out)):
            return none
        cc = lambda t: None if t is None else _c(t)
        cv = lambda m: None if m is None else (m.weight, m.geom(), m.bias)
        co, cq, cp = ctx.blk.conv_out, ctx.blk.conv_in_q, ctx.blk.conv_in_p if ctx.has_p else None
        hw = (z.shape[1], z.shape[2])
        d_out, dz, g = cc(d_out), cc(dz), (cc(g_lp), cc(g_lq), cc(g_kl), cc(g_ks))
        one = None
        if d_out is not None and dq_out is None and dp_out is None and RB.switches.stoch_block_bwd:
            one = K.stoch_block_bwd(d_out, cv(cp), cv(cq), cv(co), p, q, z, eps, dz, *g, ctx.mode, ctx.analytical)
        if one is not None:
            dp, dq, dx_p, dx_q = one
        else:
            if d_out is not None:
                dzc = K.conv2d_dgrad(d_out, co.weight, co.geom(), hw)
                dz = dzc if dz is None else K.add(dzc, dz)
            dp, dq = K.normal_stochastic_bwd(p, q, eps, z, dz, *g, ctx.mode, ctx.analytical, z.shape[3])
            if dq_out is not None:
                dq = K.add(dq, _c(dq_out))
            if dp_out is not None:
                dp = K.add(dp, _c(dp_out))
            dx_q = K.conv2d_dgrad(dq, cq.weight, cq.geom(), hw) if ctx.needs_input_grad[2] else None
            dx_p = K.conv2d_dgrad(dp, cp.weight, cp.geom(), hw) if cp is not None and ctx.needs_input_grad[0] else None
        for m, x, dy in ((co, z, d_out), (cq, x_q, dq), (cp, x_p, dp)):
            if m is not None and dy is not None and m.weight.requires_grad:
                wgrad(x, dy, m.weight, m.geom(), grad_buf(m.weight), grad_buf(m.bias))
        dpg = None
        if cp is None and ctx.needs_input_grad[1]:
            dpg = dp
            if ctx.p_bcast:
                dpg = torch.empty_like(p)
                K.colsum(dp.view(dp.shape[0], -1), dpg.view(-1), False)
        return (dx_p, dpg, dx_q) + none[3:]


class KlElementwiseFn(Function):

    @staticmethod
    def forward(ctx, z, p, q, analytical):
        ctx.analytical = analytical
        ctx.save_for_backward(z, p, q)
# ... 343 lines not shown
```

ladder-vae-pytorch_amd/resblock.py:

```python
import os
import weakref
from typing import NamedTuple, Optional

import torch

from . import kernels as K


class Switches:

    def __init__(self, env):
        on = lambda name: env.get(name, '1') != '0'
        self.wgrad_flush = int(env.get('LVAE_WGRAD_FLUSH', '1024'))
        self.dgrad_cat = on('LVAE_DGRAD_CAT')
        self.wgrad_apply = on('LVAE_WGRAD_APPLY')
        self.wgrad_apply_maxw = int(env.get('LVAE_WGRAD_APPLY_MAXW', '16'))
        self.wgrad_pair = on('LVAE_WGRAD_PAIR')
        self.wgrad_pair_maxw = int(env.get('LVAE_WGRAD_PAIR_MAXW', '16'))
        self.gate_stats = env.get('LVAE_NO_GATE_STATS') is None
        self.defer_apply = on('LVAE_DEFER_APPLY')
        self.defer_apply_large = on('LVAE_DEFER_APPLY_LARGE')
        self.rb_fwd_min_hw, self.rb_bwd_min_hw = int(env.get('LVAE_RB_FWD_MIN_HW', '16')), int(env.get('LVAE_RB_BWD_MIN_HW', '1'))
        self.rb_gate_large = on('LVAE_RB_GATE_LARGE')
        self.stoch_block = on('LVAE_STOCH_BLOCK')
        self.stoch_block_bwd = on('LVAE_STOCH_BLOCK_BWD')
        self.gate_recompute = on('LVAE_GATE_RECOMPUTE')
        self.gate_recompute_maxw = int(env.get('LVAE_GATE_RECOMPUTE_MAXW', '16'))


switches = Switches(os.environ)


class BlockPlan(NamedTuple):
    forward: str
    bf16_internals: bool
    gate_stats: bool
    backward: Optional[str]
    wgrad_absorbs_apply: bool
    wgrad_pair: bool
    accepts: Optional[str]
    recompute_ab: bool = False


def plan_block(blk, x, training):
    sw, grad = switches, torch.is_grad_enabled()
    cv1, cv2, gate, bn1, bn2 = blk.conv1, blk.conv2, blk.gate, blk.bn1, blk.bn2
    gated_bn = gate is not None and bn1 is not None and bn2 is not None and gate.bias is not None
    full = (training and gated_bn and cv1.bias is not None and cv2.bias is not None and bn1.running_mean is not None and
            bn2.running_mean is not None and x.dtype == torch.float32)
    hw = x.shape[1] * x.shape[2]
    whole = full and K.rb_rows(x, cv1.weight, cv1.geom()) > 0
    whole_fwd, whole_bwd = whole and 0 < sw.rb_fwd_min_hw <= hw, whole and 0 < sw.rb_bwd_min_hw <= hw
    s16 = bool(not whole_fwd and not whole_bwd and gated_bn and K.resblock_bf16_storage(x, cv1.weight, cv1.geom()))
    if whole_fwd:
        forward = 'whole-image'
    elif full and not s16 and sw.rb_gate_large and K.rb_gate_rows(x, cv2.weight, cv2.geom(), whole_image=False) > 0:
        forward = 'wino-gate'
    else:
        forward = 'per-op' if gate is not None else 'ungated'
    gate_stats = gate is not None and training and bn1 is not None and bn1.running_mean is not None and sw.gate_stats
    backward, accepts, absorbs, pair = None, None, False, False
    if grad and whole_bwd:
        backward, accepts = 'whole-image', 'f32-dh'
    elif grad:
        backward = 'composed'
        if gate is not None and gate.bias is not None and gate.weight.requires_grad and \
                K.gate_bwd_fused_ws(x, gate.weight, gate.geom(), gate.weight.grad) > 0:
            backward = 'persistent-gate'
            if training and not whole_fwd and sw.defer_apply_large and K.gate_bwd_apply_ok(x, gate.weight, gate.geom(), gate.weight.grad):
                accepts = 'any-dh'
        absorbs = bool(training and bn2 is not None and sw.wgrad_apply and not s16 and cv1.weight.requires_grad and
                       x.shape[2] <= sw.wgrad_apply_maxw and K.conv2d_wgrad_apply_ok(x, cv1.weight, cv1.geom()))
        pair = bool(absorbs and sw.wgrad_pair and cv2.weight.requires_grad and x.shape[2] <= sw.wgrad_pair_maxw and
                    K.conv2d_wgrad_pair_ok(x, cv1.weight, cv1.geom(), x, cv2.weight, cv2.geom()))
    recompute = bool(forward == 'wino-gate' and backward == 'persistent-gate' and not s16 and sw.gate_recompute and
                     x.shape[2] <= sw.gate_recompute_maxw and K.gate_bwd_recompute_ok(x, gate.weight, gate.geom(), gate.weight.grad))
    return BlockPlan(forward, s16, gate_stats, backward, absorbs, pair, accepts, recompute)


class Handover(NamedTuple):
    parts: object
    pivot: object
    producer: object = None
    accepts: Optional[str] = None


def passed_on(src, aliases):
    h = getattr(src, '_lvae_handover', None)
    if h is not None and h.parts is not None:
        for a in aliases:
            a._lvae_handover = Handover(h.parts, h.pivot)


def received(x, training):
    h = getattr(x, '_lvae_handover', None) or Handover(None, None)
    defer = None
    if h.producer is not None:
        x._lvae_handover = h._replace(producer=None)
        if training and torch.is_grad_enabled() and switches.defer_apply and x.dtype == torch.float32:
            defer = (h.producer, h.accepts)
    return (h.parts, h.pivot, defer) if training else (None, None, defer)


def tagged(out, blk, plan, parts, pivot):
    producer = blk.sched if (plan.accepts and blk.training and torch.is_grad_enabled()) else None
    if parts is not None or producer is not None:
        out._lvae_handover = Handover(parts, pivot, producer, plan.accepts)
    return out


class BlockState:
    __slots__ = ('pending', 'first', 'next', '__weakref__')

    def __init__(self):
        self.pending, self.first, self.next = None, {}, weakref.WeakValueDictionary()

    def __reduce__(self):
        return BlockState, ()

    def take_pending(self, dout):
        pend, self.pending = self.pending, None
        if pend is not None and pend.out.data_ptr() != dout.data_ptr():
            raise K._C.LvaeHipError("deferred BatchNorm-backward apply: the gradient that reached the consuming block is not the tensor the "
                                    "producer left unwritten (the block output has another consumer?)")
        return pend

    _last = weakref.WeakValueDictionary()

    def link(self, direction, first_ranges):
        self.first[direction] = first_ranges
        prev = BlockState._last.get(direction)
        if prev is not None and prev is not self:
            prev.next[direction] = self
        BlockState._last[direction] = self

    def next_ranges(self, direction):
        nb = self.next.get(direction)
        return nb.first.get(direction) if nb is not None else None
```

Before: 9386 images/s.

## Batch stochastic-layer conv weight gradients into one shared Winograd launch

Adds a shared Winograd weight-gradient kernel that computes up to three 3x3 conv weight gradients (conv_in_p, conv_in_q, conv_out of a stochastic layer) in one launch. Workgroups are partitioned across the gradients by a prefix table, and a single reduce launch follows. The Winograd wgrad path is also generalised to 32-channel inputs (ncib parameter) so the 32-channel latent conv can use it. This is meant to cut launch count and fill the GPU better for small per-layer gradients, at the cost of deferring wgrad until all three backward gradients have arrived and adding bookkeeping in autograd.

```diff
diff --git a/include/lvae_hip.h b/include/lvae_hip.h
--- a/include/lvae_hip.h
+++ b/include/lvae_hip.h
@@ -204,6 +204,11 @@
 int32_t lvae_conv2d_wgrad_pair_schedule(const lvae_conv_desc* a, const lvae_conv_desc* b, int32_t* sched);
 int lvae_conv2d_wgrad_pair_f32(const lvae_conv_desc* a, const lvae_bn_apply* ap, const lvae_conv_desc* b, const float* dy_b, float* dw_a,
                                float* db_a, float* dw_b, float* db_b, void* workspace, size_t workspace_bytes, void* stream);
+int32_t lvae_conv2d_wgrad_shared_ok(const lvae_conv_desc* descs, const lvae_bn_apply* const* aps, int32_t n);
+size_t lvae_conv2d_wgrad_shared_workspace(const lvae_conv_desc* descs, int32_t n);
+int32_t lvae_conv2d_wgrad_shared_schedule(const lvae_conv_desc* descs, const lvae_bn_apply* const* aps, int32_t n, int32_t* sched);
+int lvae_conv2d_wgrad_shared_f32(const lvae_conv_desc* descs, const float* const* dy, float* const* dw, float* const* db, int32_t n,
+                                 void* workspace, size_t workspace_bytes, void* stream);
 enum {
   LVAE_WGRAD_VARIANT_GENERIC = 0,
   LVAE_WGRAD_VARIANT_IMG = 1,
diff --git a/ladder-vae-pytorch_amd/_C.py b/ladder-vae-pytorch_amd/_C.py
--- a/ladder-vae-pytorch_amd/_C.py
+++ b/ladder-vae-pytorch_amd/_C.py
@@ -140,6 +140,10 @@
     'lvae_conv2d_wgrad_pair_workspace': (_Z, [C.POINTER(ConvDesc), C.POINTER(ConvDesc)]),
     'lvae_conv2d_wgrad_pair_schedule': (_I, [C.POINTER(ConvDesc), C.POINTER(ConvDesc), C.POINTER(_I)]),
     'lvae_conv2d_wgrad_pair_f32': (C.c_int, [C.POINTER(ConvDesc), C.POINTER(BnApply), C.POINTER(ConvDesc), _P, _P, _P, _P, _P, _P, _Z, _P]),
+    'lvae_conv2d_wgrad_shared_ok': (_I, [C.POINTER(ConvDesc), _P, _I]),
+    'lvae_conv2d_wgrad_shared_workspace': (_Z, [C.POINTER(ConvDesc), _I]),
+    'lvae_conv2d_wgrad_shared_schedule': (_I, [C.POINTER(ConvDesc), _P, _I, C.POINTER(_I)]),
+    'lvae_conv2d_wgrad_shared_f32': (C.c_int, [C.POINTER(ConvDesc), _P, _P, _P, _I, _P, _Z, _P]),
     'lvae_conv2d_wgrad_grouped_workspace': (_Z, [C.POINTER(ConvDesc), _I]),
     'lvae_conv2d_wgrad_grouped_f32': (C.c_int, [C.POINTER(ConvDesc), _P, _P, _P, _I, _P, _Z, _P]),
     'lvae_conv2d_wgrad_grouped_schedule': (_I, [C.POINTER(ConvDesc), _I, C.POINTER(_I)]),
diff --git a/ladder-vae-pytorch_amd/csrc/conv3x3_wgrad_wino.hip b/ladder-vae-pytorch_amd/csrc/conv3x3_wgrad_wino.hip
--- a/ladder-vae-pytorch_amd/csrc/conv3x3_wgrad_wino.hip
+++ b/ladder-vae-pytorch_amd/csrc/conv3x3_wgrad_wino.hip
@@ -15,6 +15,7 @@
   float* slab_b;
   int nranges, ncog, cpr, total_chunks, cpi;
   uint32_t m_cpi;
+  int ncib, pad_;
 };
 
 constexpr int WG_XS = 48;
@@ -52,7 +53,7 @@
 __global__ __launch_bounds__(512, 2) void conv_wgrad_wino_grouped_kernel(WgWinoGroup g) {
   kernarg_warmup<(sizeof(WgWinoGroup) < 1024 ? sizeof(WgWinoGroup) : 1024)>();
   const WgWinoArgs& a = g.p[blockIdx.y];
-  const int nwg_ = a.nranges * a.ncog * 2;
+  const int nwg_ = a.nranges * a.ncog * a.ncib;
   if ((int)blockIdx.x >= nwg_) return;
   const int bid_ = blockIdx.x;
   constexpr bool AP = false;
@@ -85,10 +86,28 @@
   }
 }
 
+constexpr int kWgWinoShared = kWgradWinoShared;
+struct WgWinoSharedArgs {
+  WgWinoArgs p[kWgWinoShared];
+  int first[kWgWinoShared + 1];
+};
+static_assert(sizeof(WgWinoSharedArgs) <= 4096, "kernel argument block");
+
+template <int TPR>
+__global__ __launch_bounds__(512, 2) void conv_wgrad_wino_shared_kernel(WgWinoSharedArgs g) {
+  kernarg_warmup<(sizeof(WgWinoSharedArgs) < 1024 ? sizeof(WgWinoSharedArgs) : 1024)>();
+  const int sel = (int)blockIdx.x < g.first[1] ? 0 : ((int)blockIdx.x < g.first[2] ? 1 : 2);
+  const WgWinoArgs& a = g.p[sel];
+  const int nwg_ = g.first[sel + 1] - g.first[sel], bid_ = (int)blockIdx.x - g.first[sel];
+  constexpr bool AP = false;
+  const lvae_bn_apply ap = lvae_bn_apply{};
+#include "conv3x3_wgrad_wino_body.inc"
+}
+
 struct WinoReduceArgs {
   const float* slab_w;
   const float* slab_b;
-  int nranges, ncog, Cout, pad_;
+  int nranges, ncog, Cout, ncib;
   int64_t stap, sk, sn;
   float* dw;
   float* db;
@@ -98,6 +117,9 @@
 };
 struct WinoReducePair {
   WinoReduceArgs p[2];
+};
+struct WinoReduceShared {
+  WinoReduceArgs p[kWgWinoShared];
 };
 
 template <bool HALF>
@@ -108,7 +130,7 @@
   const int t = threadIdx.x;
   const int q = HALF ? (t & 7) : (t & 15), p = HALF ? ((t >> 3) & 15) : ((t >> 4) & 15), rs = HALF ? (t >> 7) : (t >> 8);
   const float* src = a.slab_w + ((((size_t)(ci >> 5) * ncog + cog) * 32 + (ci & 31)) * 16 + p) * 64 + half * 32 + q * 4;
-  const size_t rstride = (size_t)2 * ncog * 32 * 16 * 64;
+  const size_t rstride = (size_t)a.ncib * ncog * 32 * 16 * 64;
   f32x4 s = {0.f, 0.f, 0.f, 0.f};
   if ((p & 3) != 3) {
     if (HALF) {
@@ -173,20 +195,34 @@
   wino_reduce_body<true>(g.p[blockIdx.y], blockIdx.x, red, red_b);
 }
 
+__global__ __launch_bounds__(1024) void conv_wgrad_wino_reduce_shared_kernel(WinoReduceShared g) {
+  kernarg_warmup<sizeof(WinoReduceShared)>();
+  const WinoReduceArgs& a = g.p[blockIdx.y];
+  if ((int)blockIdx.x >= 64 * a.ncib * a.ncog) return;
+  __shared__ __attribute__((aligned(16))) float red[8 * 16 * 32];
+  __shared__ float red_b[16][64];
+  wino_reduce_body<true>(a, blockIdx.x, red, red_b);
+}
+
 __global__ __launch_bounds__(1024) void conv_wgrad_wino_reduce_grouped_kernel(WinoReduceGroup g) {
   kernarg_warmup<(sizeof(WinoReduceGroup) < 1024 ? sizeof(WinoReduceGroup) : 1024)>();
   const WinoReduceArgs& a = g.p[blockIdx.y];
-  if ((int)blockIdx.x >= 64 * a.ncog) return;
+  if ((int)blockIdx.x >= 32 * a.ncib * a.ncog) return;
   __shared__ __attribute__((aligned(16))) float red[8 * 16 * 64];
   __shared__ float red_b[16][64];
   wino_reduce_body<false>(a, blockIdx.x, red, red_b);
+}
+
+static int wg_wino_min_cpr() {
+  static const int v = (int)std::max<int64_t>(1, tune("LVAE_WINO_WGRAD_MIN_CPR", 4));
+  return v;
 }
 
 static bool wg_wino_plan(const lvae_conv_desc* d, WgWinoArgs& a, int budget = 128) {
   static const bool off = tune("LVAE_DISABLE_WINO_WGRAD", 0) != 0 || tune("LVAE_DISABLE_WINO", 0) != 0;
   if (off) return false;
   if (d->KH != 3 || d->KW != 3 || d->stride != 1 || d->pad != 1 || d->gather != LVAE_GATHER_CONV) return false;
-  if (d->C1 != 64 || d->C2 != 0 || d->x2 != nullptr || d->Cout % 4 != 0 || d->Cout > 256) return false;
+  if ((d->C1 != 64 && d->C1 != 32) || d->C2 != 0 || d->x2 != nullptr || d->Cout % 4 != 0 || d->Cout > 256) return false;
   if (d->OH != d->H || d->OW != d->W || (d->H & 1)) return false;
   if (d->W != 8 && d->W != 16 && d->W != 32) return false;
   const int tpr = d->W / 2, tr = 16 / tpr;
@@ -196,11 +232,13 @@
   static const int64_t min_m = tune("LVAE_WINO_WGRAD_MIN_M", 256 * 64);
   if (M < min_m || M * 256 >= ((int64_t)1 << 31)) return false;
   a.ncog = (d->Cout + 63) / 64;
+  a.ncib = d->C1 / 32;
+  a.pad_ = 0;
   a.cpi = (d->H / 2) / tr;
   a.total_chunks = d->N * a.cpi;
-  int nranges = budget / a.ncog;
+  int nranges = 2 * budget / (a.ncog * a.ncib);
   if (nranges < 1) nranges = 1;
-  static const int min_cpr = (int)tune("LVAE_WINO_WGRAD_MIN_CPR", 4);
+  const int min_cpr = wg_wino_min_cpr();
   if (nranges > a.total_chunks / min_cpr) nranges = a.total_chunks / min_cpr;
   if (nranges < 1) nranges = 1;
   a.cpr = (a.total_chunks + nranges - 1) / nranges;
@@ -212,10 +250,10 @@
 bool conv_wgrad_wino_plan(const lvae_conv_desc* d, WgradPlan& p) {
   static const int64_t group_max_m = tune("LVAE_WINO_GROUP_MAX_M", 65536);
   WgWinoArgs a;
-  if (!wg_wino_plan(d, a)) return false;
+  if (d->C1 != 64 || !wg_wino_plan(d, a)) return false;
   p.group = (int64_t)d->N * d->H * d->W < group_max_m ? d->W : -1;
-  p.set_slabs(a.nranges, (size_t)a.ncog * 2 * 16 * 32 * 64, (size_t)a.ncog * 64);
-  p.apply_ok = d->precision == LVAE_PREC_F32 && d->Cout == 64 && (d->W == 16 || d->W == 32) && d->x_dtype == LVAE_DT_F32 && d->y_dtype == LVAE_DT_F32;
+  p.set_slabs(a.nranges, (size_t)a.ncog * a.ncib * 16 * 32 * 64, (size_t)a.ncog * 64);
+  p.apply_ok = d->precision == LVAE_PREC_F32 && d->C1 == 64 && d->Cout == 64 && (d->W == 16 || d->W == 32) && d->x_dtype == LVAE_DT_F32 && d->y_dtype == LVAE_DT_F32;
   return true;
 }
 
@@ -226,6 +264,7 @@
 }
 
 static bool wg_wino_pair_split(const lvae_conv_desc* da, const lvae_conv_desc* db, WgWinoArgs& a, WgWinoArgs& b) {
+  if (da->C1 != 64 || db->C1 != 64) return false;
   if (!wg_wino_plan(da, a, wg_wino_pair_ranges_a()) || a.ncog != 1 || a.nranges >= 128) return false;
   if (!wg_wino_plan(db, b, 128 - a.nranges) || b.ncog != 1) return false;
   return wg_wino_plan(da, a, 128 - b.nranges);
@@ -243,6 +282,40 @@
   return true;
 }
 
+static bool wg_wino_shared_split(const lvae_conv_desc* const* d, int n, WgWinoArgs* a) {
+  if (n < 1 || n > kWgWinoShared) return false;
+  int max_chunks = 1;
+  for (int i = 0; i < n; ++i) {
+    if (!wg_wino_plan(d[i], a[i]) || a[i].ncog != 1 || d[i]->W != d[0]->W) return false;
+    max_chunks = std::max(max_chunks, a[i].total_chunks);
+  }
+  for (int c = wg_wino_min_cpr(); c <= max_chunks; ++c) {
+    int wgs = 0;
+    for (int i = 0; i < n; ++i) wgs += a[i].ncib * ((a[i].total_chunks + c - 1) / c);
+    if (wgs > 256) continue;
+    for (int i = 0; i < n; ++i) {
+      a[i].cpr = std::min(c, a[i].total_chunks);
+      a[i].nranges = (a[i].total_chunks + a[i].cpr - 1) / a[i].cpr;
+    }
+    return true;
+  }
+  return false;
+}
+
+bool conv_wgrad_wino_shared_plan(const lvae_conv_desc* const* d, int n, WgradPlan* p, int32_t* sched) {
+  WgWinoArgs a[kWgWinoShared];
+  if (!wg_wino_shared_split(d, n, a)) return false;
+  for (int i = 0; i < n; ++i) {
+    p[i].set_slabs(a[i].nranges, (size_t)a[i].ncib * 16 * 32 * 64, 64);
+    if (sched) {
+      sched[3 * i] = a[i].nranges;
+      sched[3 * i + 1] = a[i].cpr;
+      sched[3 * i + 2] = a[i].nranges * a[i].ncib;
+    }
+  }
+  return true;
+}
+
 template <typename F>
 static int with_tpr(int W, F f) {
   if (W == 8) return f(std::integral_constant<int, 4>{});
@@ -260,8 +333,8 @@
   a.dy = o.dy;
   a.slab_w = o.slab_w();
   a.slab_b = o.slab_b();
-  r = WinoReduceArgs{a.slab_w, a.slab_b, a.nranges, a.ncog, o.d->Cout, 0, o.d->w_stap, o.d->w_sk, o.d->w_sn, o.dw, o.db};
-  return a.nranges * a.ncog * 2;
+  r = WinoReduceArgs{a.slab_w, a.slab_b, a.nranges, a.ncog, o.d->Cout, a.ncib, o.d->w_stap, o.d->w_sk, o.d->w_sn, o.dw, o.db};
+  return a.nranges * a.ncog * a.ncib;
 }
 static int wino_fill(const WgradOp& o, WgWinoArgs& a, WinoReduceArgs& r) {
   wg_wino_plan(o.d, a);
@@ -303,6 +376,31 @@
   return 0;
 }
 
+int conv_wgrad_wino_shared_launch(const WgradOp* o, int n, hipStream_t s) {
+  WgWinoSharedArgs g;
+  WinoReduceShared rg;
+  const lvae_conv_desc* d[kWgWinoShared];
+  for (int i = 0; i < n; ++i) d[i] = o[i].d;
+  if (!wg_wino_shared_split(d, n, g.p)) return LVAE_EINVAL;
+  g.first[0] = 0;
+  for (int i = 0; i < kWgWinoShared; ++i) {
+    if (i < n) {
+      g.first[i + 1] = g.first[i] + wino_fill_planned(o[i], g.p[i], rg.p[i]);
+    } else {
+      g.p[i] = g.p[0];
+      g.first[i + 1] = g.first[i];
+    }
+  }
+  const size_t lds = wg_wino_lds(o->d->W);
+  const int rc = with_tpr(o->d->W, [&](auto tpr) {
+    return launch_lds<conv_wgrad_wino_shared_kernel<decltype(tpr)::value>>("conv_wgrad_wino_shared", dim3(g.first[n]), dim3(512), lds, 160 * 1024, s, g);
+  });
+  if (rc) return rc;
+  hipLaunchKernelGGL(conv_wgrad_wino_reduce_shared_kernel, dim3(128, n), dim3(1024), 0, s, rg);
+  LVAE_LAUNCH_CHECK("conv_wgrad_wino_reduce_shared");
+  return 0;
+}
+
 int conv_wgrad_wino_launch(const WgradOp* o, int n, hipStream_t s) {
   WgWinoGroup g;
   WinoReduceGroup rg;
@@ -322,7 +420,7 @@
     return launch_lds<conv_wgrad_wino_grouped_kernel<T>>("conv_wgrad_wino_grouped", dim3(max_wgs, n), dim3(512), lds, 160 * 1024, s, g);
   });
   if (rc) return rc;
-  if (n == 1) hipLaunchKernelGGL(conv_wgrad_wino_reduce_kernel, dim3(128 * max_ncog), dim3(1024), 0, s, rg.p[0]);
+  if (n == 1) hipLaunchKernelGGL(conv_wgrad_wino_reduce_kernel, dim3(64 * g.p[0].ncib * max_ncog), dim3(1024), 0, s, rg.p[0]);
   else hipLaunchKernelGGL(conv_wgrad_wino_reduce_grouped_kernel, dim3(64 * max_ncog, n), dim3(1024), 0, s, rg);
   LVAE_LAUNCH_CHECK(n == 1 ? "conv_wgrad_wino_reduce" : "conv_wgrad_wino_reduce_grouped");
   return 0;
diff --git a/ladder-vae-pytorch_amd/csrc/conv3x3_wgrad_wino_body.inc b/ladder-vae-pytorch_amd/csrc/conv3x3_wgrad_wino_body.inc
--- a/ladder-vae-pytorch_amd/csrc/conv3x3_wgrad_wino_body.inc
+++ b/ladder-vae-pytorch_amd/csrc/conv3x3_wgrad_wino_body.inc
@@ -11,7 +11,8 @@
     const int nwg = nwg_, xcd = bid & 7, q = nwg >> 3, r = nwg & 7;
     bid = (xcd < r ? xcd * (q + 1) : r * (q + 1) + (xcd - r) * q) + (bid >> 3);
   }
-  const int cib = bid & 1, cog = (bid >> 1) % a.ncog, range = (bid >> 1) / a.ncog;
+  const int ncib = AP ? 2 : a.ncib, xcs = 32 * ncib;
+  const int cib = bid & (ncib - 1), cog = (bid >> (ncib - 1)) % a.ncog, range = (bid >> (ncib - 1)) / a.ncog;
   const int c_begin = range * a.cpr;
   const int c_end = min(a.total_chunks, c_begin + a.cpr);
   const f32x4 zero4 = {0.f, 0.f, 0.f, 0.f};
@@ -30,7 +31,7 @@
     const int hx = px - hy * HW2;
     in = px < HP;
     col_ok = (hx >= 1) & (hx <= W);
-    rel = (hy * W + hx) * 64 + cib * 32 + xc4;
+    rel = (hy * W + hx) * xcs + cib * 32 + xc4;
   };
   if (!AP) {
 #pragma unroll
@@ -90,7 +91,7 @@
   auto load_chunk = [&](int c) {
     const int n = fastdiv(c, a.m_cpi), cr = c - n * a.cpi;
     const int oh0 = cr * (2 * TR);
-    const float* xb = d.x + ((int64_t)(n * d.H + oh0 - 1) * W - 1) * 64;
+    const float* xb = d.x + ((int64_t)(n * d.H + oh0 - 1) * W - 1) * xcs;
     xok = 0;
 #pragma unroll
     for (int u = 0; u < XSLOTS; ++u) {
@@ -280,7 +281,7 @@
     Rs[4 * 4 * 2 * 16 * 64 + 64 + lane] = dbacc[1];
   }
   __syncthreads();
-  float* slab = a.slab_w + (size_t)((range * 2 + cib) * a.ncog + cog) * 32 * 16 * 64 + 4 * pi * 64;
+  float* slab = a.slab_w + (size_t)((range * ncib + cib) * a.ncog + cog) * 32 * 16 * 64 + 4 * pi * 64;
   auto finish = [&](auto hsel) {
     constexpr int h = decltype(hsel)::value;
 #pragma unroll
diff --git a/ladder-vae-pytorch_amd/csrc/conv_wgrad.hip b/ladder-vae-pytorch_amd/csrc/conv_wgrad.hip
--- a/ladder-vae-pytorch_amd/csrc/conv_wgrad.hip
+++ b/ladder-vae-pytorch_amd/csrc/conv_wgrad.hip
@@ -658,6 +658,67 @@
   for (int i = 0; i < 8; ++i) LVAE_REQUIRE(al16_or_null(operand[i]), LVAE_EALIGN, "%s: %s must be 16-byte aligned", who, name[i]);
   const WgradOp oa{a, pa, nullptr, dw_a, db_a, workspace}, ob{b, pb, dy_b, dw_b, db_b, static_cast<char*>(workspace) + piece_a};
   return conv_wgrad_wino_pair_launch(oa, ap, ob, (hipStream_t)stream);
+}
+
+static bool wgrad_shared_route(const lvae_conv_desc* descs, const lvae_bn_apply* const* aps, int32_t n, WgradPlan* p, int32_t* sched) {
+  if (!descs || n < 1 || n > kWgradWinoShared) return false;
+  const lvae_conv_desc* d[kWgradWinoShared];
+  for (int i = 0; i < n; ++i) {
+    d[i] = &descs[i];
+    if (aps && aps[i]) return false;
+    p[i] = WgradPlan{};
+    p[i].variant = LVAE_WGRAD_VARIANT_WINO;
+    if (d[i]->Cout > 64) return false;
+    if (d[i]->precision != LVAE_PREC_F32 || d[i]->x_dtype != LVAE_DT_F32 || d[i]->y_dtype != LVAE_DT_F32) return false;
+    if (d[i]->N != d[0]->N || d[i]->H != d[0]->H || d[i]->W != d[0]->W) return false;
+  }
+  return conv_wgrad_wino_shared_plan(d, n, p, sched);
+}
+
+extern "C" int32_t lvae_conv2d_wgrad_shared_ok(const lvae_conv_desc* descs, const lvae_bn_apply* const* aps, int32_t n) {
+  WgradPlan p[kWgradWinoShared];
+  return wgrad_shared_route(descs, aps, n, p, nullptr) ? 1 : 0;
+}
+
+extern "C" size_t lvae_conv2d_wgrad_shared_workspace(const lvae_conv_desc* descs, int32_t n) {
+  WgradPlan p[kWgradWinoShared];
+  if (!wgrad_shared_route(descs, nullptr, n, p, nullptr)) return 0;
+  size_t tot = 0;
+  for (int i = 0; i < n; ++i) tot += wgrad_piece(p[i]);
+  return tot;
+}
+
+extern "C" int32_t lvae_conv2d_wgrad_shared_schedule(const lvae_conv_desc* descs, const lvae_bn_apply* const* aps, int32_t n, int32_t* sched) {
+  WgradPlan p[kWgradWinoShared];
+  return sched && wgrad_shared_route(descs, aps, n, p, sched) ? 1 : 0;
+}
+
+extern "C" int lvae_conv2d_wgrad_shared_f32(const lvae_conv_desc* descs, const float* const* dy, float* const* dw, float* const* db, int32_t n,
+                                            void* workspace, size_t workspace_bytes, void* stream) {
+  const char* who = "lvae_conv2d_wgrad_shared_f32";
+  LVAE_REQUIRE(descs && dy && dw && db && n >= 1 && n <= kWgradWinoShared && workspace, LVAE_EINVAL, "%s: bad arguments (1 to 3 gradients)", who);
+  for (int i = 0; i < n; ++i) {
+    const int rc = conv_desc_check(&descs[i], who);
+    if (rc) return rc;
+    LVAE_REQUIRE(dy[i] && dw[i], LVAE_EINVAL, "%s: null dy/dw at %d (a gradient whose dy an apply has yet to form is not taken here)", who, i);
+  }
+  WgradPlan p[kWgradWinoShared];
+  LVAE_REQUIRE(wgrad_shared_route(descs, nullptr, n, p, nullptr), LVAE_EINVAL,
+               "%s: not a shared launch (1 to 3 Winograd-domain fp32 weight gradients of one N, H, W with 32 or 64 input and at most 64 output "
+               "channels, fp32 storage; lvae_conv2d_wgrad_shared_ok): use lvae_conv2d_wgrad_f32 per gradient", who);
+  size_t need = 0;
+  for (int i = 0; i < n; ++i) need += wgrad_piece(p[i]);
+  LVAE_REQUIRE(workspace_bytes >= need, LVAE_EWORKSPACE, "%s: workspace %zu < %zu", who, workspace_bytes, need);
+  LVAE_REQUIRE(al16(workspace), LVAE_EALIGN, "%s: workspace must be 16-byte aligned", who);
+  WgradOp ops[kWgradWinoShared];
+  char* ws = static_cast<char*>(workspace);
+  for (int i = 0; i < n; ++i) {
+    LVAE_REQUIRE(al16(dy[i]), LVAE_EALIGN, "%s: dy[%d] must be 16-byte aligned", who, i);
+    for (int j = 0; j < i; ++j) LVAE_REQUIRE(dw[i] != dw[j], LVAE_EINVAL, "%s: entries %d and %d accumulate into one dw", who, j, i);
+    ops[i] = WgradOp{&descs[i], p[i], dy[i], dw[i], db[i], ws};
+    ws += wgrad_piece(p[i]);
+  }
+  return conv_wgrad_wino_shared_launch(ops, n, (hipStream_t)stream);
 }
 
 extern "C" int lvae_conv2d_wgrad_bf16(const lvae_conv_desc* d, const float* dy, float* dw, float* db, void* workspace,
diff --git a/ladder-vae-pytorch_amd/csrc/lvae_host.h b/ladder-vae-pytorch_amd/csrc/lvae_host.h
--- a/ladder-vae-pytorch_amd/csrc/lvae_host.h
+++ b/ladder-vae-pytorch_amd/csrc/lvae_host.h
@@ -106,6 +106,9 @@
 int conv_wgrad_wino_apply_launch(const WgradOp& o, const lvae_bn_apply* ap, hipStream_t s);
 bool conv_wgrad_wino_pair_plan(const lvae_conv_desc* da, const lvae_conv_desc* db, WgradPlan& pa, WgradPlan& pb, int32_t* sched);
 int conv_wgrad_wino_pair_launch(const WgradOp& a, const lvae_bn_apply* ap, const WgradOp& b, hipStream_t s);
+constexpr int kWgradWinoShared = 3;
+bool conv_wgrad_wino_shared_plan(const lvae_conv_desc* const* d, int n, WgradPlan* p, int32_t* sched);
+int conv_wgrad_wino_shared_launch(const WgradOp* o, int n, hipStream_t s);
 
 bool conv1x1_wgrad_plan(const lvae_conv_desc* d, WgradPlan& p);
 int conv1x1_wgrad_launch(const WgradOp& o, hipStream_t s);
diff --git a/ladder-vae-pytorch_amd/kernels.py b/ladder-vae-pytorch_amd/kernels.py
--- a/ladder-vae-pytorch_amd/kernels.py
+++ b/ladder-vae-pytorch_amd/kernels.py
@@ -718,7 +718,7 @@
     call('lvae_conv2d_wgrad_f32', C.byref(d), ptr_dt(dy), ptr(dweight), ptr(dbias), ws.data_ptr(), ws.numel(), stream_ptr())
 
 
-def conv2d_wgrad_grouped(items):
+def _wgrad_item_arrays(items, who):
     n = len(items)
     descs = (ConvDesc * n)()
     dys, dws, dbs = (C.c_void_p * n)(), (C.c_void_p * n)(), (C.c_void_p * n)()
@@ -726,14 +726,60 @@
         _chk_nhwc(x, 'x')
         _chk_nhwc(dy, 'dy')
         if tuple(dweight.stride()) != tuple(weight.stride()):
-            raise _C.LvaeHipError("conv2d_wgrad_grouped: gradient strides %s differ from weight strides %s" %
-                                  (tuple(dweight.stride()), tuple(weight.stride())))
+            raise _C.LvaeHipError("%s: gradient strides %s differ from weight strides %s" %
+                                  (who, tuple(dweight.stride()), tuple(weight.stride())))
         N, H, W, _ = x.shape
         d = _desc(g, weight, x, kw.get('x2'), N, H, W, dy.shape[1], dy.shape[2], g.Cout, g.s_ci, g.s_co,
                   GATHER_TRANSPOSED if g.transposed else GATHER_CONV, None, kw.get('in_scale'), kw.get('in_shift'), kw.get('in_act'))
         d.y_dtype = _dt(dy)
         C.memmove(C.byref(descs, i * C.sizeof(ConvDesc)), C.byref(d), C.sizeof(ConvDesc))
         dys[i], dws[i], dbs[i] = ptr_dt(dy), ptr(dweight), ptr(dbias)
+    return descs, dys, dws, dbs
+
+
+def _wgrad_shared_descs(convs):
+    if precision != PREC_F32 or _ddi is not None or not 1 <= len(convs) <= 3:
+        return None
+    descs = (ConvDesc * len(convs))()
+    for i, (x, weight, g) in enumerate(convs):
+        if x.dim() != 4 or x.dtype != torch.float32 or g.transposed:
+            return None
+        N, H, W, _ = x.shape
+        d = _desc(g, weight, x, None, N, H, W, H, W, g.Cout, g.s_ci, g.s_co, GATHER_CONV)
+        C.memmove(C.byref(descs, i * C.sizeof(ConvDesc)), C.byref(d), C.sizeof(ConvDesc))
+    return descs
+
+
+def conv2d_wgrad_shared_ok(convs, routed=False):
+    descs = _wgrad_shared_descs(convs)
+    if descs is None or not _C.load().lvae_conv2d_wgrad_shared_ok(descs, None, len(convs)):
+        return False
+    if not routed:
+        return True
+    wide = [i for i in range(len(convs)) if descs[i].C1 == 64]
+    return bool(wide) and all(_C.load().lvae_conv2d_wgrad_variant(C.byref(descs[i])) == _C.WGRAD_VARIANT_WINO for i in wide)
+
+
+def conv2d_wgrad_shared_schedule(convs):
+    descs = _wgrad_shared_descs(convs)
+    out = (C.c_int32 * (3 * len(convs)))()
+    if descs is None or not _C.load().lvae_conv2d_wgrad_shared_schedule(descs, None, len(convs), out):
+        return None
+    return tuple(tuple(out[3 * i:3 * i + 3]) for i in range(len(convs)))
+
+
+def conv2d_wgrad_shared(items):
+    n = len(items)
+    descs, dys, dws, dbs = _wgrad_item_arrays(items, 'conv2d_wgrad_shared')
+    need = _C.load().lvae_conv2d_wgrad_shared_workspace(descs, n)
+    ws = workspace(need, items[0][0].device)
+    call('lvae_conv2d_wgrad_shared_f32', descs, C.cast(dys, C.c_void_p), C.cast(dws, C.c_void_p), C.cast(dbs, C.c_void_p), n,
+         ws.data_ptr(), ws.numel(), stream_ptr())
+
+
+def conv2d_wgrad_grouped(items):
+    n = len(items)
+    descs, dys, dws, dbs = _wgrad_item_arrays(items, 'conv2d_wgrad_grouped')
     need = _C.load().lvae_conv2d_wgrad_grouped_workspace(descs, n)
     ws = workspace(need, items[0][0].device)
     call('lvae_conv2d_wgrad_grouped_f32', descs, C.cast(dys, C.c_void_p), C.cast(dws, C.c_void_p), C.cast(dbs, C.c_void_p), n,
diff --git a/ladder-vae-pytorch_amd/lib/stochastic.py b/ladder-vae-pytorch_amd/lib/stochastic.py
--- a/ladder-vae-pytorch_amd/lib/stochastic.py
+++ b/ladder-vae-pytorch_amd/lib/stochastic.py
@@ -32,10 +32,15 @@
             fused = self._fused(p_params, q_params, forced_latent, use_mode, analytical_kl, noise, n_img, rows, stats)
             if fused is not None:
                 return fused
+        share = None
+        if q_params is not None and not tempered and not force_constant_output:
+            ins = ([(p_params, self.conv_in_p)] if self.transform_p_params else []) + [(q_params, self.conv_in_q)]
+            z_like = q_params.detach()[..., :self.c_vars]
+            share = ops.WgradShare.plan(ins + [(z_like, self.conv_out)])
         if self.transform_p_params:
-            p_params = self.conv_in_p(p_params)
+            p_params = ops.conv(p_params, self.conv_in_p, share=share and (share, True))
         if q_params is not None:
-            q_params = self.conv_in_q(q_params)
+            q_params = ops.conv(q_params, self.conv_in_q, share=share and (share, True))
         ref = q_params if q_params is not None else p_params
         N = ref.shape[0] if n_img is None else n_img
         H, W = ref.shape[1], ref.shape[2]
@@ -58,7 +63,7 @@
                 raise RuntimeError("force_constant_output is a sampling-time option; run it under torch.no_grad()")
             z = z[0:1].expand_as(z).contiguous()
             p_params = p_params[0:1].expand(N, -1, -1, -1).contiguous()
-        out = self.conv_out(z)
+        out = ops.conv(z, self.conv_out, share=share and (share, False))
         data = {'z': z, 'p_params': p_params, 'q_params': q_params, 'logprob_p': outs[1], 'logprob_q': None,
                 'kl_elementwise': None, 'kl_samplewise': None, 'kl_spatial': None}
         if q_params is not None:
diff --git a/ladder-vae-pytorch_amd/ops.py b/ladder-vae-pytorch_amd/ops.py
--- a/ladder-vae-pytorch_amd/ops.py
+++ b/ladder-vae-pytorch_amd/ops.py
@@ -87,13 +87,40 @@
             t.record_stream(st)
 
 
+class WgradShare:
+
+    def __init__(self, n_in):
+        self.items, self.wait = [], n_in
+
+    @staticmethod
+    def plan(convs):
+        if not (RB.switches.wgrad_shared and torch.is_grad_enabled() and all(m.weight.requires_grad for _, m in convs)):
+            return None
+        if not K.conv2d_wgrad_shared_ok([(x, m.weight, m.geom()) for x, m in convs], routed=True):
+            return None
+        return WgradShare(len(convs) - 1)
+
+    def add(self, item, is_input):
+        self.items.append(item)
+        self.wait -= int(is_input)
+        if self.wait > 0:
+            return
+        items, self.items = self.items, []
+        if (len(items) >= 2 and _side['stream'] is None and all(it[1].dtype == torch.float32 for it in items) and
+                K.conv2d_wgrad_shared_ok([(it[0], it[2], it[3]) for it in items])):
+            K.conv2d_wgrad_shared(items)
+        else:
+            for x, dy, w, g, dw, db, kw in items:
+                wgrad(x, dy, w, g, dw, db, **kw)
+
+
 class ConvFn(Function):
 
     @staticmethod
-    def forward(ctx, x, x2, mod, out_act, weight, bias):
+    def forward(ctx, x, x2, mod, out_act, weight, bias, share=None):
         g = mod.geom()
         y = K.conv2d(x, weight, g, bias=bias, x2=x2, out_act=out_act)
-        ctx.mod, ctx.out_act, ctx.g = mod, out_act, g
+        ctx.mod, ctx.out_act, ctx.g, ctx.share = mod, out_act, g, share
         ctx.has_x2 = x2 is not None
         ctx.save_for_backward(x, x2, y if out_act else None)
         return y
@@ -107,7 +134,11 @@
             dy = K.act_bwd_from_out(dy, y, ctx.out_act)
         w = mod.weight
         if w.requires_grad:
-            wgrad(x, dy, w, g, grad_buf(w), grad_buf(mod.bias) if mod.bias is not None else None, x2=x2)
+            db = grad_buf(mod.bias) if mod.bias is not None else None
+            if ctx.share is not None and x2 is None:
+                ctx.share[0].add((x, dy, w, g, grad_buf(w), db, {}), ctx.share[1])
+            else:
+                wgrad(x, dy, w, g, grad_buf(w), db, x2=x2)
         dx = dx2 = None
         hw = (x.shape[1], x.shape[2])
         if x2 is None:
@@ -123,11 +154,11 @@
                     dx = K.conv2d_dgrad(dy, w, g, hw, ci_range=(0, C1))
                 if ctx.needs_input_grad[1]:
                     dx2 = K.conv2d_dgrad(dy, w, g, hw, ci_range=(C1, g.Cin))
-        return dx, dx2, None, None, None, None
-
-
-def conv(x, mod, x2=None, out_act=None):
-    return ConvFn.apply(x, x2, mod, out_act, mod.weight, mod.bias)
+        return dx, dx2, None, None, None, None, None
+
+
+def conv(x, mod, x2=None, out_act=None, share=None):
+    return ConvFn.apply(x, x2, mod, out_act, mod.weight, mod.bias, share)
 
 
 def _bn_of_half(h, bn, training, parts, pivot):
diff --git a/ladder-vae-pytorch_amd/resblock.py b/ladder-vae-pytorch_amd/resblock.py
--- a/ladder-vae-pytorch_amd/resblock.py
+++ b/ladder-vae-pytorch_amd/resblock.py
@@ -17,6 +17,7 @@
         self.wgrad_apply_maxw = int(env.get('LVAE_WGRAD_APPLY_MAXW', '16'))
         self.wgrad_pair = on('LVAE_WGRAD_PAIR')
         self.wgrad_pair_maxw = int(env.get('LVAE_WGRAD_PAIR_MAXW', '16'))
+        self.wgrad_shared = on('LVAE_WGRAD_SHARED')
         self.gate_stats = env.get('LVAE_NO_GATE_STATS') is None
         self.defer_apply = on('LVAE_DEFER_APPLY')
         self.defer_apply_large = on('LVAE_DEFER_APPLY_LARGE')
```

Measured after the change: 9480 images/s (median of 6 runs). +1.0%, better.
